# esw0116/DynaVSR

Measured on AMD Instinct MI355X. Metric: inner-loop frames/sec/GPU (EDVR-M x4, 5x3x180x320): forward leg = BASELINE.json configs[1]; the inner MAML step and the per-frame pipeline are `inner_step` / `per_frame_pipeline`, higher is better.
Workload: dtype f32; 1 GPU; EDVR-M x4 forward (PCD deformable alignment + TSA fusion + reconstruction), clips of 1x5x3x180x320 -> 3x720x1280 (BASELINE.json configs[1]); one step = 2 clip(s) per GPU, one per HIP stream (adapt.super_resolve_video); clips_in_flight_per_gpu=2

## Files before the change

### dynavsr_amd/csrc/conv2d_v2.hip

```cpp
#include <algorithm>
#include <cmath>
#include <cstdlib>
#include <type_traits>

#include "common.h"
#include "kernels.h"
#include "small_grid.h"

namespace dvsr {

#ifdef DVSR_CONV_TRACE
#define DVSR_ABLATE(a) ((a).ablate)
#define DVSR_STAMP(i)                                                                              \
  do {                                                                                             \
    if (a.trace && threadIdx.x == 0) a.trace[(size_t)blockIdx.x * 64 + (i)] = __builtin_readcyclecounter(); \
  } while (0)
#else
#define DVSR_ABLATE(a) 0
#define DVSR_STAMP(i) \
  do {                \
  } while (0)
#endif

template <int KS, int S, int CC, int TH, int MT, int BF = 0>
// ... 750 lines not shown
  using Sh = KsShape<MT, NT>;
  auto kern = conv2d_ksplit_kernel<MT, NT>;
  static PerDeviceOnce attr_once;
  set_dyn_lds_once(attr_once, (const void*)kern, Sh::LDS_BYTES);
  hipLaunchKernelGGL(kern, dim3(k.nitems), dim3(256), Sh::LDS_BYTES, st, k);
  return check_launch("conv2d_ksplit_kernel");
}

namespace {
struct ConvShape { int ks, stride, N, Ho, Wo, Cout, Ctot; };
int int_or(const char* v, int dflt) { return v ? atoi(v) : dflt; }

double conv2_pipe_cost(int TH, int MT, int CC, const ConvShape& s) {
  const double wgs = (double)ceil_div(s.Wo, 32) * ceil_div(s.Ho, TH) * s.N * ceil_div(s.Cout, 32 * MT);
  return ceil(wgs / 256.0) * 64.0 * (s.ks * s.ks) * (CC / 2) * (TH / 4) * MT;
}
bool mt1_wins(int cc, const ConvShape& s) { return conv2_pipe_cost(4, 1, cc, s) < 0.97 * conv2_pipe_cost(4, 2, cc, s); }

ConvGeo choose_row_split(const ConvShape& s, ConvAllow allow) {
  ConvGeo g{8, 4, mt1_wins(8, s) ? 1 : 2};
  if ((allow & ALLOW_DMA_HALO) && s.stride == 1 && s.Wo % 4 == 0) g.kernel = ConvKernel::ROW_SPLIT;
  return g;
}

constexpr long long KSPLIT_BELOW_WGS = 700;
bool choose_ksplit(const ConvShape& s, ConvAllow allow, ConvGeo* g) {
  if (!(s.ks == 3 && s.stride == 1 && (allow & ALLOW_KSPLIT) && s.Ctot >= 32 && s.Cout >= 32)) return false;
  const long long wg41 = (long long)ceil_div(s.Wo, 32) * ceil_div(s.Ho, 4) * s.N * ceil_div(s.Cout, 32);
  if (wg41 >= KSPLIT_BELOW_WGS) return false;
  *g = (s.Cout % 64 != 0 && s.Ho % 2 == 0) ? ConvGeo{32, 2, 1} : ConvGeo{32, 1, 2};
  return true;
}

int chunk_channels(int ks) { return ks == 1 ? 32 : (ks == 2 ? 16 : 8); }
ConvGeo choose_direct_tile(const ConvShape& s) {
  const int cc = chunk_channels(s.ks);
  if (s.ks == 3 && s.stride == 2) {
    const double c82 = conv2_pipe_cost(8, 2, cc, s);
    if (c82 <= conv2_pipe_cost(4, 2, cc, s) && c82 <= conv2_pipe_cost(4, 1, cc, s)) return ConvGeo{cc, 8, 2};
  }
  return ConvGeo{cc, 4, mt1_wins(cc, s) ? 1 : 2};
}

struct WinoPick { int th; double cost; };
double wino_workgroups(const ConvShape& s, int oh, int ow) { return (double)ceil_div(s.Wo, ow) * ceil_div(s.Ho, oh) * s.N * ceil_div(s.Cout, 64); }
double wino_rounds_cost(const ConvShape& s, double cus, int oh, int ow, double chunk_cyc, double fixed_cyc) {
  return ceil(wino_workgroups(s, oh, ow) / cus) * ((s.Ctot / 8) * chunk_cyc + fixed_cyc) / 2.07;
}
double direct_cost(const ConvShape& s) {
  const double dcyc = std::min(conv2_pipe_cost(4, 2, 8, s), conv2_pipe_cost(4, 1, 8, s));
  const double drounds = dcyc / (64.0 * 9 * 4 * (mt1_wins(8, s) ? 1 : 2));
  return dcyc * (s.Ctot / 8) / (drounds <= 6.0 ? 0.60 : 0.78) / 2.4;
}
WinoPick wino_f2_cost(const ConvShape& s, double cus, bool tile16) {
  const double w4 = wino_rounds_cost(s, cus, 4, 64, 5100.0, 12500.0), w8 = wino_rounds_cost(s, cus, 8, 32, 5100.0, 12500.0);
  const double w16 = tile16 ? wino_rounds_cost(s, cus, 16, 16, 5100.0, 12500.0) : 1e300;
  return {(w16 < w4 && w16 < w8) ? 16 : (w8 < w4 ? 8 : 4), std::min(std::min(w4, w8), w16)};
}
constexpr double W5_CHUNK_CYC = 4300.0, W5_FIXED_CYC = 17500.0;
WinoPick wino_f4_cost(const ConvShape& s, double cus) {
  const double f8 = wino_rounds_cost(s, cus, 8, 64, W5_CHUNK_CYC, W5_FIXED_CYC), f16 = wino_rounds_cost(s, cus, 16, 32, W5_CHUNK_CYC, W5_FIXED_CYC);
  return {f16 < f8 ? 16 : 8, std::min(f8, f16)};
}
constexpr double SHARED_LATENCY_BOUND = 1.05;
bool f4_occupies_less(const ConvShape& s, double cus, const WinoPick& f2, const WinoPick& f4) {
  const int ow2 = f2.th == 16 ? 16 : (f2.th == 8 ? 32 : 64), ow4 = f4.th == 16 ? 32 : 64;
  const double g2 = wino_workgroups(s, f2.th, ow2), g4 = wino_workgroups(s, f4.th, ow4);
  if (g2 > cus || g4 > cus) return false;
  ConvShape one = s;
  one.N = 1;
  if (2.0 * wino_workgroups(one, f2.th, ow2) <= cus || 2.0 * wino_workgroups(one, f4.th, ow4) > cus) return false;
  return g4 * f4.cost < g2 * f2.cost && f4.cost <= SHARED_LATENCY_BOUND * f2.cost;
}
}

double conv2_f4_occupied_cycles(int N, int Ho, int Wo, int Cout, int Ctot, int th) {
  const ConvShape s{3, 1, N, Ho, Wo, Cout, Ctot};
  return wino_workgroups(s, th, th == 16 ? 32 : 64) * ((Ctot / 8) * W5_CHUNK_CYC + W5_FIXED_CYC);
}

ConvGeo conv2_choose(int ks, int stride, int N, int Ho, int Wo, int Cout, int Ctot, ConvAllow allow) {
  const ConvShape s{ks, stride, N, Ho, Wo, Cout, Ctot};
  if (ks == 7 || ks == 9) return choose_row_split(s, allow);
  ConvGeo g;
  if (choose_ksplit(s, allow, &g)) return g;
  g = choose_direct_tile(s);
  if ((allow & ALLOW_DMA_HALO) && ks == 3 && stride == 1 && Wo % 4 == 0 && Ctot % 8 == 0) g.kernel = ConvKernel::DMA_HALO;
  const int wino_on = int_or(getenv("DVSR_CONV_WINO"), 1);
  if (!(wino_on && g.kernel == ConvKernel::DMA_HALO && (allow & ALLOW_WINO) && Cout >= 32 && Ctot >= 16)) return g;
  const int wino3_on = int_or(getenv("DVSR_CONV_WINO3"), 1), wino5_on = int_or(getenv("DVSR_CONV_WINO5"), 1);
  const double direct = direct_cost(s), cus = (double)device_cus();
  const WinoPick f2 = wino_f2_cost(s, cus, wino3_on != 0);
  if (wino5_on && wino3_on && (allow & ALLOW_WINO_F4) && Wo % 4 == 0 && device_lds_optin() >= (size_t)156 * 1024) {
    const WinoPick f4 = wino_f4_cost(s, cus);
    const bool shared_pick = (allow & ALLOW_SHARED_DEVICE) && f2.cost < direct && f4_occupies_less(s, cus, f2, f4);
    if (wino5_on >= 2 || (allow & ALLOW_ONLY_F4) || ((1.15 * f4.cost < f2.cost || shared_pick) && f4.cost < direct))
      return ConvGeo{8, wino5_on == 3 ? 16 : f4.th, 2, 0, ConvKernel::WINO_F4};
  }
  if ((wino_on == 2 || f2.cost < direct) && device_lds_optin() >= (size_t)155 * 1024)
    return ConvGeo{8, f2.th, 2, 0, wino3_on ? ConvKernel::WINO_F2_BF16 : ConvKernel::WINO_F2};
  return g;
}

static int pack_chunk_floats(int ks, int cc, int bf, PackLayout layout) {
  switch (layout) {
    case PackLayout::WINO_F2: return 16 * 2 * 64 * 4;
    case PackLayout::WINO_F2_BF16: return 2 * 6144;
    case PackLayout::WINO_F4: return 18 * 2 * 3 * 256;
    case PackLayout::DCN_SPLIT: return mdcn_pack_floats();
    default: return (bf == 2 ? 3 : 1) * 2 * ks * ks * (bf ? cc / 16 : cc / 8) * 2 * 32 * 4;
  }
}
size_t conv2_pack_floats(int ks, int Cout, int Ctot, int cc, int bf, PackLayout layout) {
  return (size_t)ceil_div(Cout, 64) * ceil_div(Ctot, cc) * pack_chunk_floats(ks, cc, bf, layout);
}
PackEntry conv2_pack_entry(const float* w, float* P, int ks, int Cout, int Ctot, int cc, int bf, PackLayout layout, int wt, int w_ctot,
                           int w_coff) {
  PackEntry e{};
  e.w = w; e.P = P; e.Cout = Cout; e.Ctot = Ctot; e.KK = ks * ks; e.CC = cc; e.wt = wt; e.w_ctot = w_ctot; e.w_coff = w_coff;
  e.ncb = ceil_div(Cout, 64); e.nchunks = ceil_div(Ctot, cc); e.pch = pack_chunk_floats(ks, cc, bf, layout);
  e.bf = bf; e.layout = layout;
  return e;
}

#ifdef DVSR_CONV_TRACE
static long long* g_trace_buf = nullptr;
static int g_trace_countdown = -1;
extern "C" int dvsr_debug_conv_trace(void* buf, int launch_index) {
  g_trace_buf = (long long*)buf;
  g_trace_countdown = launch_index;
  return 0;
}
#endif

int conv2d_packed_prepare(const dvsr_conv2d_desc& d, const float* wp, const ConvExtra& ex, const ConvGeo& geo, ConvK2* out) {
  DVSR_REQUIRE(d.x0 && wp && d.y, DVSR_ERR_INVALID, "conv2d_packed: null x0/wp/y");
  DVSR_REQUIRE(((d.ks == 1 || d.ks == 2) && d.stride == 1) || (d.ks == 3 && (d.stride == 1 || d.stride == 2)) ||
                   ((d.ks == 7 || d.ks == 9) && d.stride == 1 && geo.kernel == ConvKernel::ROW_SPLIT),
               DVSR_ERR_UNSUPPORTED, "conv2d_packed: ks=%d stride=%d", d.ks, d.stride);
  DVSR_REQUIRE(d.c1 == 0 || (d.c0 % geo.cc == 0 && !ex.in_ps && !ex.in_dil), DVSR_ERR_UNSUPPORTED,
               "conv2d_packed: two inputs need c0 %% %d == 0 and a plain first input (c0=%d)", geo.cc, d.c0);
  ConvK2& k = *out;
  k.x0 = d.x0; k.x1 = d.x1; k.wp = wp; k.bias = d.bias; k.res = d.res; k.y = d.y;
  k.N = d.N; k.c0 = d.c0; k.c1 = d.c1; k.H = d.H; k.W = d.W; k.Cout = d.Cout;
  k.pad = d.pad; k.act = d.act; k.ps = d.pixel_shuffle; k.x1_bdiv = d.x1_bdiv > 0 ? d.x1_bdiv : 1;
  k.x0_bs = d.x0_bstride > 0 ? d.x0_bstride : (long long)d.c0 * d.H * d.W;
  k.x1_bs = d.x1_bstride > 0 ? d.x1_bstride : (long long)d.c1 * d.H * d.W;
  k.Ho = (d.H + 2 * d.pad - d.ks) / d.stride + 1;
  k.Wo = (d.W + 2 * d.pad - d.ks) / d.stride + 1;
  k.nchunks = ceil_div(d.c0 + d.c1, geo.cc);
  k.in_ps = ex.in_ps; k.in_dil = ex.in_dil; k.Hs = ex.Hs; k.Ws = ex.Ws; k.accum = ex.accum;
  k.gmask = ex.gmask; k.gmask_act = ex.gmask_act;
  k.wdiv = ex.wdiv > 0 ? ex.wdiv : 1; k.w_gs = ex.w_gs; k.b_gs = ex.b_gs;
  DVSR_REQUIRE(!d.pre || (geo.kernel == ConvKernel::WINO_F4 && !d.res && d.pixel_shuffle == 0 && ((uintptr_t)d.pre & 15) == 0),
               DVSR_ERR_UNSUPPORTED, "conv2d_packed: a pre-activation addend needs the F(4x4, 3x3) kernel, a 16-byte aligned tensor, "
               "no residual and no PixelShuffle");
  k.pre = d.pre; k.pre_bdiv = d.pre_bdiv > 0 ? d.pre_bdiv : 1; k.pre_bs = (long long)d.Cout * k.Ho * k.Wo;
#ifdef DVSR_CONV_TRACE
  {
    static int ablate = -1;
    if (ablate < 0) {
      const char* v = getenv("DVSR_CONV_ABLATE");
      ablate = v ? atoi(v) : 0;
    }
    k.ablate = ablate;
  }
#endif
  if (k.in_ps) k.x0_bs = (long long)d.c0 * d.H * d.W;
  if (k.in_dil) k.x0_bs = (long long)d.c0 * ex.Hs * ex.Ws;
#ifdef DVSR_CONV_TRACE
  k.trace = (g_trace_countdown == 0) ? g_trace_buf : nullptr;
  if (g_trace_countdown >= 0) --g_trace_countdown;
#endif
  if (geo.kernel == ConvKernel::ROW_SPLIT) {
    DVSR_REQUIRE((d.ks == 7 || d.ks == 9) && d.stride == 1 && d.pad == d.ks / 2 && !ex.in_ps && !ex.in_dil && geo.cc == 8 &&
                     geo.th == 4 && d.W % 4 == 0 && (d.c1 == 0 || d.c0 % 8 == 0) && k.x0_bs % 4 == 0 && k.x1_bs % 4 == 0 &&
                     ((uintptr_t)d.x0 & 15) == 0 && ((uintptr_t)d.x1 & 15) == 0,
                 DVSR_ERR_UNSUPPORTED, "conv2d_packed: the row-split DMA kernel needs 7x7 / 9x9, stride 1, pad ks/2, plain "
                 "16-byte aligned inputs and W %% 4 == 0 (W=%d c0=%d c1=%d)", d.W, d.c0, d.c1);
  } else if (needs_dma_halo_inputs(geo.kernel)) {
    DVSR_REQUIRE(!is_winograd(geo.kernel) || d.c0 + d.c1 >= 16, DVSR_ERR_UNSUPPORTED, "conv2d_packed: the Winograd kernel needs two 8-channel chunks");
    DVSR_REQUIRE(geo.kernel != ConvKernel::WINO_F4 || (!ex.accum && !ex.gmask && d.W % 4 == 0 && (geo.th == 8 || geo.th == 16)), DVSR_ERR_UNSUPPORTED,
                 "conv2d_packed: the F(4x4, 3x3) kernel stores whole tile columns of forward launches (W=%d th=%d)", d.W, geo.th);
    DVSR_REQUIRE(!is_winograd(geo.kernel) || d.pixel_shuffle == 0 || (d.pixel_shuffle == 2 && d.Cout % 4 == 0 && !d.res && !ex.accum && !ex.gmask),
                 DVSR_ERR_UNSUPPORTED, "conv2d_packed: the Winograd kernel stores plain or PixelShuffle(2) tiles (ps=%d)", d.pixel_shuffle);
    DVSR_REQUIRE(d.ks == 3 && d.stride == 1 && d.pad == 1 && !ex.in_ps && !ex.in_dil && geo.cc == 8 && (geo.th == 4 || geo.th == 8 || (geo.th == 16 && on_bf16_split(geo.kernel))) &&
                     d.W % 4 == 0 && d.c0 % 8 == 0 && d.c1 % 8 == 0 && k.x0_bs % 4 == 0 && k.x1_bs % 4 == 0 &&
                     ((uintptr_t)d.x0 & 15) == 0 && ((uintptr_t)d.x1 & 15) == 0,
                 DVSR_ERR_UNSUPPORTED, "conv2d_packed: the DMA-halo kernel needs 3x3/s1/pad 1, plain 16-byte aligned inputs, "
                 "W %% 4 == 0 and channel counts %% 8 == 0 (W=%d c0=%d c1=%d)", d.W, d.c0, d.c1);
  }
  if (d.ks == 3 && geo.cc == 32) {
    DVSR_REQUIRE(d.stride == 1 && (d.c1 == 0 || d.c0 % 32 == 0) && !ex.in_ps && !ex.in_dil && d.pad == 1 &&
                     ((geo.th == 1 && geo.mt == 2) || (geo.th == 2 && geo.mt == 1)),
                 DVSR_ERR_UNSUPPORTED, "conv2d_packed: the K-split kernel needs 3x3/s1/pad 1, plain inputs, c0 %% 32 == 0 "
                 "with two inputs (th=%d mt=%d)", geo.th, geo.mt);
    k.tiles_x = ceil_div(k.Wo, 32); k.tiles_y = ceil_div(k.Ho, geo.th); k.ntiles = k.tiles_x * k.tiles_y * k.N;
    k.ncb = ceil_div(k.Cout, 32 * geo.mt);
    k.tiles_per_xcd = ceil_div(k.ntiles, 8);
    k.nitems = k.tiles_per_xcd * 8 * k.ncb;
  }
  return DVSR_OK;
}

template <int KS, int S, int CC, int TH, int BF>
static int launch_conv2_mt(int mt, const ConvK2& k, hipStream_t st) {
  return mt == 2 ? launch_conv2<KS, S, CC, TH, 2, BF>(k, st) : launch_conv2<KS, S, CC, TH, 1, BF>(k, st);
}

int conv2d_packed_run(const dvsr_conv2d_desc& d, const float* wp, const ConvExtra& ex, const ConvGeo& geo,
                      hipStream_t st) {
  ConvK2 k;
  int rc = conv2d_packed_prepare(d, wp, ex, geo, &k);
  if (rc) return rc;
  if (geo.bf) {
    DVSR_REQUIRE((d.ks == 3 || (d.ks == 2 && geo.bf == 2)) && d.stride == 1 && geo.cc == 16 && (geo.th == 4 || (geo.bf == 2 && geo.th == 8)),
                 DVSR_ERR_UNSUPPORTED,
                 "conv2d_packed: the bf16 kernel exists for 3x3 (split: also 2x2) stride-1 convs with 16-channel chunks");
    const bool th8 = geo.th == 8;
    if (geo.bf == 2 && d.ks == 2)
      return th8 ? launch_conv2_mt<2, 1, 16, 8, 2>(geo.mt, k, st) : launch_conv2_mt<2, 1, 16, 4, 2>(geo.mt, k, st);
    if (geo.bf == 2) return th8 ? launch_conv2_mt<3, 1, 16, 8, 2>(geo.mt, k, st) : launch_conv2_mt<3, 1, 16, 4, 2>(geo.mt, k, st);
    return launch_conv2_mt<3, 1, 16, 4, 1>(geo.mt, k, st);
  }
  switch (geo.kernel) {
    case ConvKernel::WINO_F2: return conv2d_wino_launch(k, geo.th, st);
    case ConvKernel::WINO_F2_BF16: return conv2d_wino3_launch(k, geo.th, st);
    case ConvKernel::WINO_F4: return conv2d_wino5_launch(k, geo.th, st);
    case ConvKernel::ROW_SPLIT:
      if (d.ks == 7) return geo.mt == 2 ? launch_dmarow<7, 4, 2>(k, st) : launch_dmarow<7, 4, 1>(k, st);
      return geo.mt == 2 ? launch_dmarow<9, 4, 2>(k, st) : launch_dmarow<9, 4, 1>(k, st);
    case ConvKernel::DMA_HALO:
      if (geo.th != 4) break;
      return geo.mt == 2 ? launch_dma<4, 2>(k, st) : launch_dma<4, 1>(k, st);
    case ConvKernel::REG:
      if (d.ks == 3 && geo.cc == 32) return geo.mt == 2 ? launch_ksplit<2, 1>(k, st) : launch_ksplit<1, 2>(k, st);
      switch (((d.ks * 10 + d.stride) * 100 + geo.cc) * 100 + geo.th * 10 + geo.mt) {
        case 320882: return launch_conv2<3, 2, 8, 8, 2>(k, st);
        case 320842: return launch_conv2<3, 2, 8, 4, 2>(k, st);
        case 320841: return launch_conv2<3, 2, 8, 4, 1>(k, st);
        case 310842: return launch_conv2<3, 1, 8, 4, 2>(k, st);
        case 310841: return launch_conv2<3, 1, 8, 4, 1>(k, st);
        case 211642: return launch_conv2<2, 1, 16, 4, 2>(k, st);
        case 211641: return launch_conv2<2, 1, 16, 4, 1>(k, st);
        case 113242: return launch_conv2<1, 1, 32, 4, 2>(k, st);
        case 113241: return launch_conv2<1, 1, 32, 4, 1>(k, st);
      }
      break;
  }
  DVSR_REQUIRE(false, DVSR_ERR_INVALID, "conv2d_packed: no kernel for ks=%d cc=%d th=%d mt=%d", d.ks, geo.cc, geo.th,
               geo.mt);
}

}

namespace {
struct OpPack {
  dvsr::ConvGeo geo;
  size_t floats;
};
OpPack op_pack(int ks, int stride, int pad, int N, int Ho, int Wo, int Cout, int Ctot, bool plain, bool aligned = false,
               bool only_f4 = false) {
  using namespace dvsr;
  OpPack o;
  const bool k3 = ks == 3 && stride == 1 && pad == 1, kbig = (ks == 7 || ks == 9) && stride == 1 && pad == ks / 2;
  o.geo = conv2_choose(ks, stride, N, Ho, Wo, Cout, Ctot, (k3 && plain && !only_f4 ? ALLOW_KSPLIT : ALLOW_NONE) | ((k3 || kbig) && aligned ? ALLOW_DMA_HALO : ALLOW_NONE) |
                                                              (k3 && aligned ? ALLOW_WINO | ALLOW_WINO_F4 : ALLOW_NONE) | (only_f4 ? ALLOW_ONLY_F4 : ALLOW_NONE));
  o.floats = conv2_pack_floats(ks, Cout, Ctot, o.geo);
  return o;
}
OpPack op_pack_for(const dvsr_conv2d_desc& d, int Cout, int Ctot) {
  const bool big = d.ks == 7 || d.ks == 9;
  const bool aligned = (((uintptr_t)d.x0 | (uintptr_t)d.x1) & 15) == 0 && (big ? (d.c1 == 0 || d.c0 % 8 == 0) : (d.c0 % 8 == 0 && d.c1 % 8 == 0)) &&
                       d.x0_bstride % 4 == 0 && d.x1_bstride % 4 == 0 && (d.H * d.W) % 4 == 0;
  return op_pack(d.ks, 1, d.pad, d.N, d.H, d.W, Cout, Ctot, d.c1 == 0 || d.c0 % 32 == 0, aligned, d.pre != nullptr);
}
int op_run(const dvsr_conv2d_desc& d, const dvsr::ConvExtra& ex, int Cout, int Ctot, void* ws, size_t bytes, hipStream_t st) {
  using namespace dvsr;
  DVSR_REQUIRE((d.ks == 1 || d.ks == 3 || d.ks == 7 || d.ks == 9) && d.stride == 1 && d.pad == d.ks / 2, DVSR_ERR_UNSUPPORTED,
               "conv2d (packed): ks=%d stride=%d pad=%d (1x1 / 3x3 / 7x7 / 9x9, stride 1, pad ks/2)", d.ks, d.stride, d.pad);
  const OpPack o = op_pack_for(d, Cout, Ctot);
  DVSR_REQUIRE(d.ks <= 3 || o.geo.kernel == ConvKernel::ROW_SPLIT, DVSR_ERR_UNSUPPORTED, "conv2d (packed): this %dx%d convolution is not eligible for the "
               "row-split kernel (dvsr_conv2d_packed_geometry): use dvsr_conv2d_forward / _backward", d.ks, d.ks);
  DVSR_REQUIRE(!d.pre || (o.geo.kernel == ConvKernel::WINO_F4 && !d.res && !d.pixel_shuffle), DVSR_ERR_UNSUPPORTED,
               "conv2d (packed): a pre-activation addend (pre) needs a launch the F(4x4, 3x3) kernel takes -- an aligned 3x3 / "
               "stride 1 / pad 1 convolution, W %% 4 == 0, whole 8-channel chunks, at least 32 outputs and 16 inputs -- without a "
               "residual or a PixelShuffle");
  DVSR_REQUIRE(ws && bytes >= o.floats * sizeof(float), DVSR_ERR_WORKSPACE, "conv2d (packed): workspace %zu < %zu bytes", bytes,
               o.floats * sizeof(float));
  PackTable t;
  t.n = 1;
  t.e[0] = conv2_pack_entry(d.w, (float*)ws, d.ks, Cout, Ctot, o.geo, ex.wt, ex.w_ctot, ex.w_coff);
  int rc = pack_weights_run(t, st);
  if (rc) return rc;
  return conv2d_packed_run(d, (const float*)ws, ex, o.geo, st);
}
}

extern "C" size_t dvsr_conv2d_packed_workspace_bytes(const dvsr_conv2d_desc* d) {
  if (!d || (d->ks != 1 && d->ks != 3 && d->ks != 7 && d->ks != 9)) return 0;
  const int ctot = d->c0 + d->c1;
  const size_t a = op_pack(d->ks, 1, d->ks / 2, d->N, d->H, d->W, d->Cout, ctot, true).floats;
  const size_t b = op_pack(d->ks, 1, d->ks / 2, d->N, d->H, d->W, ctot, d->Cout, true).floats;
  const size_t c = op_pack(d->ks, 1, d->ks / 2, d->N, d->H, d->W, d->Cout, ctot, false).floats;
  size_t w = 0;
  if (d->ks == 3)
    for (const dvsr::PackLayout l : {dvsr::PackLayout::WINO_F2_BF16, dvsr::PackLayout::WINO_F4})
      w = std::max(w, std::max(dvsr::conv2_pack_floats(3, d->Cout, ctot, 8, 0, l), dvsr::conv2_pack_floats(3, ctot, d->Cout, 8, 0, l)));
  return std::max(std::max(a, b), std::max(c, w)) * sizeof(float);
}

extern "C" int dvsr_conv2d_packed_geometry(const dvsr_conv2d_desc* d, int geo[4]) {
  DVSR_REQUIRE(d && geo && (d->ks == 1 || d->ks == 3 || d->ks == 7 || d->ks == 9) && d->stride == 1 && d->pad == d->ks / 2,
               DVSR_ERR_INVALID, "conv2d_packed_geometry: 1x1 / 3x3 / 7x7 / 9x9 stride-1 descriptors only");
  const OpPack o = op_pack_for(*d, d->Cout, d->c0 + d->c1);
  geo[0] = o.geo.cc; geo[1] = o.geo.th; geo[2] = o.geo.mt; geo[3] = static_cast<int>(o.geo.kernel);
  return DVSR_OK;
}

extern "C" int dvsr_conv2d_forward_packed(const dvsr_conv2d_desc* d, void* workspace, size_t workspace_bytes,
                                          dvsr_stream_t stream) {
  DVSR_REQUIRE(d && d->x0 && d->w && d->y, DVSR_ERR_INVALID, "conv2d_forward_packed: null argument");
  DVSR_REQUIRE(d->pixel_shuffle == 0 || (d->pixel_shuffle == 2 && d->Cout % 4 == 0 && !d->res), DVSR_ERR_INVALID,
               "conv2d_forward_packed: pixel_shuffle needs Cout %% 4 == 0 and no residual");
  return op_run(*d, dvsr::ConvExtra(), d->Cout, d->c0 + d->c1, workspace, workspace_bytes, (hipStream_t)stream);
}

extern "C" int dvsr_conv2d_dgrad_packed(const dvsr_conv2d_desc* d, const float* gy, float* gx0, void* workspace,
                                        size_t workspace_bytes, dvsr_stream_t stream) {
  using namespace dvsr;
  DVSR_REQUIRE(d && gy && gx0 && d->w, DVSR_ERR_INVALID, "conv2d_dgrad_packed: null argument");
  DVSR_REQUIRE(d->c1 == 0 && d->pixel_shuffle == 0, DVSR_ERR_UNSUPPORTED, "conv2d_dgrad_packed: single plain input only");
  dvsr_conv2d_desc g = {};
  g.x0 = gy; g.w = d->w; g.y = gx0; g.N = d->N; g.c0 = d->Cout; g.Cout = d->c0; g.H = d->H; g.W = d->W; g.ks = d->ks;
  g.stride = 1; g.pad = d->ks / 2; g.act = ACT_NONE; g.x1_bdiv = 1;
  ConvExtra ex;
  ex.wt = 1; ex.w_ctot = d->c0; ex.w_coff = 0;
  return op_run(g, ex, d->c0, d->Cout, workspace, workspace_bytes, (hipStream_t)stream);
}
```

### dynavsr_amd/csrc/conv2d_wino5.hip

```cpp
#include <type_traits>

#include "common.h"
#include "kernels.h"
#include "small_grid.h"

namespace dvsr {

#ifdef DVSR_CONV_TRACE
#define W5_STAMP(i)                                                                                       \
  do {                                                                                                    \
    if (a.trace && threadIdx.x == 0) a.trace[(size_t)blockIdx.x * 64 + (i)] = __builtin_readcyclecounter(); \
  } while (0)
#else
#define W5_STAMP(i) \
  do {              \
  } while (0)
#endif

typedef float w5f2 __attribute__((ext_vector_type(2)));
typedef __bf16 w5bf8 __attribute__((ext_vector_type(8)));
typedef __bf16 w5bf2 __attribute__((ext_vector_type(2)));
typedef unsigned w5u4 __attribute__((ext_vector_type(4)));

constexpr int W5_PCH = 18 * 2 * 3 * 256;

template <int TC>
struct Wino5Shape {
  static constexpr int CC = 8, NTILE = 32, TRW = NTILE / TC, NT = 768;
  static constexpr int OH = 4 * TRW, OW = 4 * TC;
  static constexpr int IH = OH + 2, RP = OW + 8, GR = RP / 4;
  static constexpr int NG = CC * IH * GR;
  static constexpr int NI = (NG + NT - 1) / NT;
  static constexpr int RAWPAD = NI * NT * 4;
  static constexpr int VIMG = 36 * 3 * 32 * 4;
  static constexpr int XCH = 6 * 16 * 64 * 4;
  static constexpr int LOOP = 2 * RAWPAD + 2 * VIMG;
  static constexpr size_t LDS_BYTES = (size_t)(LOOP > XCH ? LOOP : XCH) * sizeof(float);
};

constexpr int w5_waitcnt(int vm, int lgkm) { return (vm & 15) | (7 << 4) | ((lgkm & 15) << 8) | ((vm >> 4) << 14); }

__device__ __forceinline__ unsigned w5_cvt_pk(float a, float b) {
  return __builtin_bit_cast(unsigned, __builtin_convertvector(w5f2{a, b}, w5bf2));
}
__device__ __forceinline__ void w5_dma16(__amdgpu_buffer_rsrc_t rs, float* lds, unsigned voff, unsigned soff) {
  __builtin_amdgcn_raw_ptr_buffer_load_lds(rs, (__attribute__((address_space(3))) void*)lds, 16, voff, soff, 0, 0);
}
__device__ __forceinline__ __amdgpu_buffer_rsrc_t w5_rsrc(const float* base, int num_records) {
  return __builtin_amdgcn_make_buffer_rsrc(const_cast<float*>(base), 0, num_records, 0x00020000);
}

__global__ void pack_weights_wino5_kernel(PackTable t) {
  const PackEntry& e = t.e[blockIdx.y];
  if (e.layout != PackLayout::WINO_F4) return;
  __bf16* const P16 = reinterpret_cast<__bf16*>(e.P);
  const size_t total = (size_t)e.ncb * e.nchunks * 512;
  constexpr double G[6][3] = {{1.0 / 4, 0, 0},          {-1.0 / 6, -1.0 / 6, -1.0 / 6}, {-1.0 / 6, 1.0 / 6, -1.0 / 6},
                              {1.0 / 24, 1.0 / 12, 1.0 / 6}, {1.0 / 24, -1.0 / 12, 1.0 / 6}, {0, 0, 1}};
  for (size_t i = blockIdx.x * (size_t)blockDim.x + threadIdx.x; i < total; i += (size_t)gridDim.x * blockDim.x) {
    const int c8 = (int)(i & 7), col = (int)((i >> 3) & 63);
    const size_t ck = i >> 9;
    const int k = (int)(ck % e.nchunks), cb = (int)(ck / e.nchunks);
    const int co = cb * 64 + col, ci = k * 8 + c8;
    double g[3][3];
    const bool ok = co < e.Cout && ci < e.Ctot;
    const float* src = !e.wt ? e.w + ((size_t)co * (e.w_ctot ? e.w_ctot : e.Ctot) + (e.w_ctot ? e.w_coff : 0) + ci) * 9
                             : e.w + ((size_t)ci * e.w_ctot + e.w_coff + co) * 9;
#pragma unroll
    for (int tap = 0; tap < 9; ++tap) g[tap / 3][tap % 3] = ok ? (double)src[e.wt ? 8 - tap : tap] : 0.0;
    double c[6][3];
#pragma unroll
    for (int xi = 0; xi < 6; ++xi)
#pragma unroll
      for (int b = 0; b < 3; ++b) c[xi][b] = G[xi][0] * g[0][b] + G[xi][1] * g[1][b] + G[xi][2] * g[2][b];
    const int mh = col >> 5, c32 = col & 31;
    __bf16* dst = P16 + ck * (size_t)(2 * W5_PCH) + (size_t)mh * 1536 + (size_t)c32 * 8 + c8;
#pragma unroll
    for (int xi = 0; xi < 6; ++xi)
#pragma unroll
      for (int nu = 0; nu < 6; ++nu) {
        const float u = (float)(c[xi][0] * G[nu][0] + c[xi][1] * G[nu][1] + c[xi][2] * G[nu][2]);
        const __bf16 h = (__bf16)u;
        const float r1 = u - (float)h;
        const __bf16 m = (__bf16)r1;
        const __bf16 l = (__bf16)(r1 - (float)m);
        __bf16* d = dst + (size_t)(xi * 3 + (nu >> 1)) * 3072;
        if (nu & 1) { d[512] = m; d[768] = h; d[1024] = l; }
        else { d[0] = h; d[256] = m; d[1280] = l; }
      }
  }
}

int pack_weights_wino5_run(const PackTable& t, hipStream_t st) {
  hipLaunchKernelGGL(pack_weights_wino5_kernel, dim3(64, t.n), dim3(256), 0, st, t);
  return check_launch("pack_weights_wino5_kernel");
}

template <int TC, bool RES, bool R16, bool PRE>
__global__ __launch_bounds__(1024) void conv2d_wino5_kernel(ConvK2 a) {
  static_assert(!PRE || (R16 && !RES), "the addend is read by the sixteen-reader epilogue, never beside a residual");
  using Sh = Wino5Shape<TC>;
  constexpr int IH = Sh::IH, RP = Sh::RP, GR = Sh::GR;
  constexpr int CHF = IH * RP;
  constexpr int QF = 768 * 4;
  extern __shared__ __attribute__((aligned(16))) float smem[];
  float* const raw0 = smem;
  unsigned* const vimg0 = reinterpret_cast<unsigned*>(smem + 2 * Sh::RAWPAD);

  const int id = blockIdx.x;
  const int q_ = id >> 3;
  const int cbi = q_ % a.ncb;
  const int j_ = q_ / a.ncb;
  const int tile = (id & 7) * a.tiles_per_xcd + j_;
  if (j_ >= a.tiles_per_xcd || tile >= a.ntiles) return;
  const int tx_ = tile % a.tiles_x;
  const int t2 = tile / a.tiles_x;
  const int ty_ = t2 % a.tiles_y;
  const int n = t2 / a.tiles_y;
  const int oy0 = ty_ * Sh::OH, ox0 = tx_ * Sh::OW;

  const int tid = threadIdx.x, lane = tid & 63;
  const int wave = __builtin_amdgcn_readfirstlane(tid >> 6);
  const int lo = lane & 31, hi = lane >> 5;
  const size_t HW = (size_t)a.H * a.W;
  auto fence = [&]() __attribute__((always_inline)) { __builtin_amdgcn_sched_barrier(0); };
  auto lds_barrier = [&]() __attribute__((always_inline)) {
    asm volatile("s_waitcnt lgkmcnt(0)" ::: "memory");
    __builtin_amdgcn_s_barrier();
    asm volatile("" ::: "memory");
  };
  W5_STAMP(0);
#ifdef DVSR_CONV_TRACE
  if (a.trace && threadIdx.x == 0) a.trace[(size_t)blockIdx.x * 64 + 60] = __builtin_amdgcn_s_memrealtime();
#endif

  auto read16 = [&](int m) __attribute__((always_inline)) {
    int le = lane;
    asm volatile("" : "+v"(le));
    const int rq_r = wave & 3, cp_r = wave >> 2;
    const float* const xr = smem + (rq_r * 64 + le) * 4 + cp_r;
    const int lo_e = le & 31, hi_e = le >> 5;
    const int trow_e = lo_e / TC, tcol_e = lo_e - trow_e * TC;
    const int oy = oy0 + 4 * trow_e, ox = ox0 + 4 * tcol_e;
    const size_t HWo = (size_t)a.Ho * a.Wo;
    const float slope = a.act == ACT_LRELU ? 0.1f : (a.act == ACT_RELU ? 0.f : 1.f);
    const float* bias = wset_ptr(a.bias, a.b_gs, n, a.wdiv);
    const int co0 = cbi * 64 + m * 32 + 8 * rq_r + 4 * hi_e + cp_r;
    f32x4 pr[4];
    if constexpr (PRE) {
      const bool live = oy < a.Ho && ox < a.Wo && co0 < a.Cout;
      const float* pre = a.pre + (size_t)(n / a.pre_bdiv) * a.pre_bs + (size_t)co0 * HWo + (size_t)oy * a.Wo + ox;
#pragma unroll
      for (int i = 0; i < 4; ++i)
        pr[i] = (live && oy + i < a.Ho) ? *reinterpret_cast<const f32x4*>(pre + (size_t)i * a.Wo) : f32x4{0.f, 0.f, 0.f, 0.f};
    }
    float y[4][4];
#pragma unroll
    for (int j = 0; j < 4; ++j) {
      float z[6];
#pragma unroll
      for (int x = 0; x < 6; ++x) z[x] = xr[(x * 16 + j * 4) * 256];
      const float sa = z[1] + z[2], da = z[1] - z[2];
      const float sb = z[3] + z[4], db = z[3] - z[4];
      y[0][j] = z[0] + sa + sb;
      y[1][j] = __builtin_fmaf(2.f, db, da);
      y[2][j] = __builtin_fmaf(4.f, sb, sa);
      y[3][j] = __builtin_fmaf(8.f, db, da) + z[5];
    }
    const bool px_ok = oy < a.Ho && ox < a.Wo;
    const int nrow = a.Ho - oy < 4 ? a.Ho - oy : 4;
    if (px_ok && co0 < a.Cout) {
      const float b0 = bias ? bias[co0] : 0.f;
      const size_t base = ((size_t)n * a.Cout + co0) * HWo + (size_t)oy * a.Wo + ox;
      f32x4 rr[4];
      if constexpr (RES) {
#pragma unroll
        for (int i = 0; i < 4; ++i)
          rr[i] = i < nrow ? *reinterpret_cast<const f32x4*>(a.res + base + (size_t)i * a.Wo) : f32x4{0.f, 0.f, 0.f, 0.f};
      }
#pragma unroll
      for (int i = 0; i < 4; ++i) {
        if (i >= nrow) break;
        f32x4 v;
#pragma unroll
        for (int j = 0; j < 4; ++j) {
          float v0 = y[i][j] + b0;
          if constexpr (PRE) v0 += pr[i][j];
          v[j] = fmaxf(v0, v0 * slope);
        }
        if constexpr (RES) v += rr[i];
        *reinterpret_cast<f32x4*>(a.y + base + (size_t)i * a.Wo) = v;
      }
    }
  };

  if (wave >= 12) {
    const int pw = wave - 12, ptid = tid - 768;
    const float* x0n = a.x0 + (size_t)n * a.x0_bs;
    const float* x1n = a.c1 ? a.x1 + (size_t)(n / a.x1_bdiv) * a.x1_bs : x0n;
    static_assert(IH * GR * 4 == 720, "a channel quad is 720 groups");
    unsigned hoff[3];
#pragma unroll
    for (int jj = 0; jj < 3; ++jj) {
      const int L = jj * 256 + ptid;
      const int cq = L / (IH * GR), rr = L - cq * (IH * GR);
      const int iy = rr / GR, g = rr - iy * GR;
      const int gy = oy0 - 1 + iy, gx = ox0 - 4 + 4 * g;
      const bool live = L < 4 * IH * GR;
      const bool ok = live && (unsigned)gy < (unsigned)a.H && (unsigned)gx < (unsigned)a.W;
      hoff[jj] = ok ? (unsigned)(((size_t)cq * HW + (size_t)gy * a.W + gx) * 4) : 0x80000000u;
      if (live && !ok) {
#pragma unroll
        for (int bb = 0; bb < 4; ++bb) *reinterpret_cast<f32x4*>(raw0 + (bb >> 1) * Sh::RAWPAD + (bb & 1) * QF + L * 4) = f32x4{0.f, 0.f, 0.f, 0.f};
      }
    }
    const unsigned chunk_bytes = (unsigned)(Sh::CC * HW * 4), quad_bytes = (unsigned)(4 * HW * 4);
    auto issue_raw = [&](int k) __attribute__((always_inline)) {
      const bool live = k < a.nchunks;
      const bool second = k * Sh::CC >= a.c0;
      const unsigned soff = live ? (unsigned)(second ? k - a.c0 / Sh::CC : k) * chunk_bytes : 0u;
      const __amdgpu_buffer_rsrc_t rs = w5_rsrc(second ? x1n : x0n, live ? 0x7fffffff : 0);
      float* dst = raw0 + (k & 1) * Sh::RAWPAD + 256 * pw;
#pragma unroll
      for (int jj = 0; jj < 3; ++jj) {
        w5_dma16(rs, dst + jj * 1024, hoff[jj], soff);
        w5_dma16(rs, dst + QF + jj * 1024, hoff[jj], soff + quad_bytes);
      }
    };
    const int ptile = 8 * pw + (lane & 7), ppair = (lane >> 3) & 3;
    const int trow_t = ptile / TC, tcol_t = ptile - trow_t * TC;
    const int pch = 2 * ppair + hi;
    const float* prd = raw0 + (pch >> 2) * QF + (pch & 3) * CHF + 4 * trow_t * RP + 4 * tcol_t;
    unsigned* vw12 = vimg0 + (hi ? 2 : 1) * 6 * 384 + ptile * 4 + ppair;
    unsigned* vw34 = vimg0 + (hi ? 4 : 3) * 6 * 384 + ptile * 4 + ppair;
    unsigned* vw05 = vimg0 + (hi ? 5 : 0) * 6 * 384 + ptile * 4 + ppair;
    auto ld_row = [&](float (&d)[6], int row) __attribute__((always_inline)) {
      const float* p = prd + row * RP;
      const w5f2 l2 = *reinterpret_cast<const w5f2*>(p + 2);
      const f32x4 m4 = *reinterpret_cast<const f32x4*>(p + 4);
      const w5f2 h2 = *reinterpret_cast<const w5f2*>(p + 8);
      d[0] = l2[1]; d[1] = m4[0]; d[2] = m4[1]; d[3] = m4[2]; d[4] = m4[3]; d[5] = h2[0];
    };
    auto colpass = [&](const float (&r)[6], float (&v)[6]) __attribute__((always_inline)) {
      v[0] = __builtin_fmaf(4.f, r[0], __builtin_fmaf(-5.f, r[2], r[4]));
      v[5] = __builtin_fmaf(4.f, r[1], __builtin_fmaf(-5.f, r[3], r[5]));
      const float e1 = __builtin_fmaf(-4.f, r[2], r[4]), o1 = __builtin_fmaf(-4.f, r[1], r[3]);
      v[1] = e1 + o1; v[2] = e1 - o1;
      const float e2 = r[4] - r[2], o2 = r[3] - r[1];
      v[3] = __builtin_fmaf(2.f, o2, e2); v[4] = __builtin_fmaf(-2.f, o2, e2);
    };
    auto finish_pair = [&](const float (&ra)[6], const float (&rb)[6], unsigned* vw) __attribute__((always_inline)) {
      float va[6], vb[6];
      colpass(ra, va);
      colpass(rb, vb);
#pragma unroll
      for (int v = 0; v < 6; ++v) {
        const auto s0 = __builtin_amdgcn_permlane32_swap(__builtin_bit_cast(unsigned, va[v]), __builtin_bit_cast(unsigned, vb[v]), false, false);
        const unsigned u0 = s0[0], u1 = s0[1];
        const float v0 = __builtin_bit_cast(float, u0), v1 = __builtin_bit_cast(float, u1);
        const unsigned h = w5_cvt_pk(v0, v1);
        const float r0 = v0 - __builtin_bit_cast(float, h << 16), r1 = v1 - __builtin_bit_cast(float, h & 0xffff0000u);
        const unsigned m = w5_cvt_pk(r0, r1);
        const float q0 = r0 - __builtin_bit_cast(float, m << 16), q1 = r1 - __builtin_bit_cast(float, m & 0xffff0000u);
        unsigned* d = vw + v * 384;
#ifdef W5_NOVW
        d[0] = h ^ m ^ w5_cvt_pk(q0, q1);
#else
        d[0] = h; d[128] = m; d[256] = w5_cvt_pk(q0, q1);
#endif
      }
    };
    auto produce = [&]() __attribute__((always_inline)) {
      float d0[6], d1[6], d2[6], d3[6], d4[6], d5[6];
      ld_row(d1, 1); ld_row(d2, 2); ld_row(d3, 3); ld_row(d4, 4);
      ld_row(d0, 0); ld_row(d5, 5);
      float ra[6], rb[6];
#pragma unroll
      for (int j = 0; j < 6; ++j) {
        const float e = __builtin_fmaf(-4.f, d2[j], d4[j]), o = __builtin_fmaf(-4.f, d1[j], d3[j]);
        ra[j] = e + o; rb[j] = e - o;
      }
      finish_pair(ra, rb, vw12);
      fence();
#pragma unroll
      for (int j = 0; j < 6; ++j) {
        const float e = d4[j] - d2[j], o = d3[j] - d1[j];
        ra[j] = __builtin_fmaf(2.f, o, e); rb[j] = __builtin_fmaf(-2.f, o, e);
      }
      finish_pair(ra, rb, vw34);
      fence();
#pragma unroll
      for (int j = 0; j < 6; ++j) {
        ra[j] = __builtin_fmaf(4.f, d0[j], __builtin_fmaf(-5.f, d2[j], d4[j]));
        rb[j] = __builtin_fmaf(4.f, d1[j], __builtin_fmaf(-5.f, d3[j], d5[j]));
      }
      finish_pair(ra, rb, vw05);
    };
    issue_raw(0);
    issue_raw(1);
    __builtin_amdgcn_s_waitcnt(w5_waitcnt(6, 0));
    __builtin_amdgcn_s_barrier();
    asm volatile("" ::: "memory");
    produce();
    __builtin_amdgcn_s_waitcnt(w5_waitcnt(0, 0));
    __builtin_amdgcn_s_barrier();
    asm volatile("" ::: "memory");
    int vstep = Sh::VIMG, rstep = Sh::RAWPAD;
    vw12 += vstep; vw34 += vstep; vw05 += vstep; prd += rstep;
    __builtin_amdgcn_s_setprio(3);
    for (int k = 0; k < a.nchunks; ++k) {

#ifndef W5_NODMA
      issue_raw(k + 2);
#endif
#ifndef W5_NOPROD
      if (k + 1 < a.nchunks) produce();
#endif
      __builtin_amdgcn_s_waitcnt(w5_waitcnt(0, 0));
      __builtin_amdgcn_s_barrier();
      asm volatile("" ::: "memory");
      vw12 -= vstep; vw34 -= vstep; vw05 -= vstep; prd -= rstep;
      vstep = -vstep; rstep = -rstep;
    }
    if constexpr (R16) {
      __builtin_amdgcn_s_setprio(0);
      lds_barrier();
      lds_barrier(); read16(0);
      lds_barrier();
      lds_barrier(); read16(1);
    } else {
      lds_barrier(); lds_barrier(); lds_barrier(); lds_barrier();
    }
    return;
  }
  {
    const int cxi = wave % 6, cmh = wave / 6;
    f32x16 acc[6];
#pragma unroll
    for (int v = 0; v < 6; ++v)
#pragma unroll
      for (int r = 0; r < 16; ++r) acc[v][r] = 0.f;
    const float* wp_cb = wset_ptr(a.wp, a.w_gs, n, a.wdiv) + (size_t)cbi * a.nchunks * W5_PCH;
    const __amdgpu_buffer_rsrc_t wrsrc = w5_rsrc(wp_cb, -1);
    const unsigned avoff = (unsigned)(lane * 16);
    const int asb = (cxi * 3 * 2 + cmh) * 3072;
    f32x4 AF[3];
    auto gldA = [&](auto g_, int k) __attribute__((always_inline)) {
      constexpr int G = decltype(g_)::value;
#ifdef W5_NOA
      if (k > 0 || G > 2) return;
#endif
      const int soff = k * (W5_PCH * 4) + asb + (G / 3) * 6144 + (G % 3) * 1024;
      AF[G % 3] = __builtin_bit_cast(f32x4, __builtin_amdgcn_raw_buffer_load_b128(wrsrc, (int)avoff, soff, 0));
    };
    auto blend = [&](f32x4& x, const f32x4& l, bool keep) __attribute__((always_inline)) {
#pragma unroll
      for (int r = 0; r < 4; ++r) x[r] = keep ? x[r] : l[r];
    };
    const unsigned* vrd = vimg0 + cxi * 6 * 384 + lo * 4;
    const unsigned* vrd_lh = vrd + (hi ? 0 : 256);
    const unsigned* vrd_hl = vrd + (hi ? 256 : 0);
    w5u4 BF[2];
    auto ldB = [&](auto f_) __attribute__((always_inline)) {
      constexpr int F = decltype(f_)::value, NU = F / 3, W = F % 3;
      if constexpr (W == 0) BF[F & 1] = *reinterpret_cast<const w5u4*>(vrd + NU * 384);
      else if constexpr (W == 1) BF[F & 1] = *reinterpret_cast<const w5u4*>(vrd + NU * 384 + 128);
      else if constexpr (NU & 1) BF[F & 1] = *reinterpret_cast<const w5u4*>(vrd_hl + NU * 384);
      else BF[F & 1] = *reinterpret_cast<const w5u4*>(vrd_lh + NU * 384);
    };
    auto mma = [&](f32x16& c, const f32x4& av, const w5u4& bv) __attribute__((always_inline)) {
#ifdef W5_NOMMA
      c[0] += av[0] * __builtin_bit_cast(float, bv[0]);
      return;
#endif
      c = __builtin_amdgcn_mfma_f32_32x32x16_bf16(__builtin_bit_cast(w5bf8, av), __builtin_bit_cast(w5bf8, bv), c, 0, 0, 0);
    };
    static_for<0, 3>([&](auto g_) __attribute__((always_inline)) { gldA(g_, 0); });
    __builtin_amdgcn_s_barrier();
    asm volatile("" ::: "memory");
    __builtin_amdgcn_s_barrier();
    asm volatile("" ::: "memory");
    int vstep = Sh::VIMG;
    for (int k = 0; k < a.nchunks; ++k) {
      ldB(std::integral_constant<int, 0>{}); ldB(std::integral_constant<int, 1>{});
      const int knext = k + 1 < a.nchunks ? k + 1 : k;
      static_for<0, 18>([&](auto f_) __attribute__((always_inline)) {
        constexpr int F = decltype(f_)::value, NU = F / 3, I = F % 3;
        constexpr int XS = NU & 1;
        mma(acc[NU], AF[XS], BF[F & 1]);
#ifdef W5_NOBR
        if constexpr (false)
#else
        if constexpr (F + 2 < 18)
#endif
          ldB(std::integral_constant<int, (F + 2 < 18 ? F + 2 : 0)>{});
        if constexpr (I == 1) {
          blend(AF[XS], AF[2], (NU & 1) ? hi != 0 : hi == 0);
          if constexpr ((NU & 1) && NU < 5) gldA(std::integral_constant<int, 3 * ((NU < 5 ? NU : 1) / 2) + 5>{}, k);
          if constexpr (NU == 5) gldA(std::integral_constant<int, 2>{}, knext);
        }
        if constexpr (I == 2) {
          if constexpr (NU < 4) gldA(std::integral_constant<int, 3 * ((NU < 4 ? NU : 0) / 2) + 3 + (NU & 1)>{}, k);
          else gldA(std::integral_constant<int, (NU & 1)>{}, knext);
        }
        fence();
      });
      lds_barrier();
      if (k < 16) W5_STAMP(3 + k);
      vrd += vstep; vrd_lh += vstep; vrd_hl += vstep;
      vstep = -vstep;
    }
  W5_STAMP(40);

  int lane_e = lane;
  asm volatile("" : "+v"(lane_e));
  f32x16 Z[4];
#pragma unroll
  for (int r = 0; r < 16; ++r) {
    const float sa = acc[1][r] + acc[2][r], da = acc[1][r] - acc[2][r];
    const float sb = acc[3][r] + acc[4][r], db = acc[3][r] - acc[4][r];
    Z[0][r] = acc[0][r] + sa + sb;
    Z[1][r] = __builtin_fmaf(2.f, db, da);
    Z[2][r] = __builtin_fmaf(4.f, sb, sa);
    Z[3][r] = __builtin_fmaf(8.f, db, da) + acc[5][r];
  }
  float* const xw = smem + (cxi * 16 * 64 + lane_e) * 4;
  const int rq_r = wave & 3, cp_r = wave >> 2;
  const float* const xr = smem + (rq_r * 64 + lane_e) * 4 + cp_r * 2;
  const int lo_e = lane_e & 31, hi_e = lane_e >> 5;
  const int trow_e = lo_e / TC, tcol_e = lo_e - trow_e * TC;
  const int oy = oy0 + 4 * trow_e, ox = ox0 + 4 * tcol_e;
  const size_t HWo = (size_t)a.Ho * a.Wo;
  const float slope = a.act == ACT_LRELU ? 0.1f : (a.act == ACT_RELU ? 0.f : 1.f);
  const float* bias = wset_ptr(a.bias, a.b_gs, n, a.wdiv);
  W5_STAMP(50);
  lds_barrier();
  W5_STAMP(51);
#pragma unroll 1
  for (int m = 0; m < 2; ++m) {
    if (cmh == m) {
#pragma unroll
      for (int j = 0; j < 4; ++j)
#pragma unroll
        for (int rq = 0; rq < 4; ++rq)
          *reinterpret_cast<f32x4*>(xw + (j * 4 + rq) * 256) = f32x4{Z[j][4 * rq], Z[j][4 * rq + 1], Z[j][4 * rq + 2], Z[j][4 * rq + 3]};
    }
    W5_STAMP(52 + 4 * m);
    lds_barrier();
    W5_STAMP(53 + 4 * m);
    if constexpr (R16) read16(m);
    else if (wave < 8) {
      const int co0 = cbi * 64 + m * 32 + 8 * rq_r + 4 * hi_e + 2 * cp_r;
      float y[2][4][4];
#pragma unroll
      for (int j = 0; j < 4; ++j) {
        w5f2 z[6];
#pragma unroll
        for (int x = 0; x < 6; ++x) z[x] = *reinterpret_cast<const w5f2*>(xr + (x * 16 + j * 4) * 256);
#pragma unroll
        for (int c = 0; c < 2; ++c) {
          const float sa = z[1][c] + z[2][c], da = z[1][c] - z[2][c];
          const float sb = z[3][c] + z[4][c], db = z[3][c] - z[4][c];
          y[c][0][j] = z[0][c] + sa + sb;
          y[c][1][j] = __builtin_fmaf(2.f, db, da);
          y[c][2][j] = __builtin_fmaf(4.f, sb, sa);
          y[c][3][j] = __builtin_fmaf(8.f, db, da) + z[5][c];
        }
      }
      const bool px_ok = oy < a.Ho && ox < a.Wo;
      const int nrow = a.Ho - oy < 4 ? a.Ho - oy : 4;
      if (px_ok && co0 < a.Cout) {
        const bool two = co0 + 1 < a.Cout;
        const float b0 = bias ? bias[co0] : 0.f, b1 = (bias && two) ? bias[co0 + 1] : 0.f;
#pragma unroll
        for (int i = 0; i < 4; ++i)
#pragma unroll
          for (int j = 0; j < 4; ++j) {
            const float v0 = y[0][i][j] + b0, v1 = y[1][i][j] + b1;
            y[0][i][j] = fmaxf(v0, v0 * slope);
            y[1][i][j] = fmaxf(v1, v1 * slope);
          }
        if (a.ps == 0) {
#pragma unroll
          for (int c = 0; c < 2; ++c) {
            if (c == 1 && !two) break;
            const size_t base = ((size_t)n * a.Cout + co0 + c) * HWo + (size_t)oy * a.Wo + ox;
            if constexpr (RES) {
              f32x4 rr[4];
#pragma unroll
              for (int i = 0; i < 4; ++i)
                rr[i] = i < nrow ? *reinterpret_cast<const f32x4*>(a.res + base + (size_t)i * a.Wo) : f32x4{0.f, 0.f, 0.f, 0.f};
#pragma unroll
              for (int i = 0; i < 4; ++i) {
                if (i >= nrow) break;
                const f32x4 v = f32x4{y[c][i][0], y[c][i][1], y[c][i][2], y[c][i][3]} + rr[i];
                *reinterpret_cast<f32x4*>(a.y + base + (size_t)i * a.Wo) = v;
              }
            } else {
#pragma unroll
              for (int i = 0; i < 4; ++i) {
                if (i >= nrow) break;
                *reinterpret_cast<f32x4*>(a.y + base + (size_t)i * a.Wo) = f32x4{y[c][i][0], y[c][i][1], y[c][i][2], y[c][i][3]};
              }
            }
          }
        } else {
          const int cq = co0 >> 2, dy = (co0 >> 1) & 1;
          float* dst = a.y + (((size_t)n * (a.Cout >> 2) + cq) * (2 * a.Ho) + (2 * oy + dy)) * (size_t)(2 * a.Wo) + 2 * ox;
#pragma unroll
          for (int i = 0; i < 4; ++i) {
            if (i >= nrow) break;
            float* d = dst + (size_t)(2 * i) * (2 * a.Wo);
            *reinterpret_cast<f32x4*>(d) = f32x4{y[0][i][0], y[1][i][0], y[0][i][1], y[1][i][1]};
            *reinterpret_cast<f32x4*>(d + 4) = f32x4{y[0][i][2], y[1][i][2], y[0][i][3], y[1][i][3]};
          }
        }
      }
    }
    W5_STAMP(54 + 4 * m);
    if (m == 0) lds_barrier();
    W5_STAMP(55 + 4 * m);
  }
#ifdef DVSR_CONV_TRACE
  W5_STAMP(41);
  __builtin_amdgcn_s_waitcnt(0);
  W5_STAMP(42);
  if (a.trace && threadIdx.x == 0) {
    a.trace[(size_t)blockIdx.x * 64 + 61] = __builtin_amdgcn_s_memrealtime();
    a.trace[(size_t)blockIdx.x * 64 + 63] = __builtin_amdgcn_s_getreg((4) | (0 << 6) | (31 << 11));
    a.trace[(size_t)blockIdx.x * 64 + 62] = __builtin_amdgcn_s_getreg((20) | (0 << 6) | (31 << 11));
  }
#endif
  }
}

template <int TC>
static int launch_wino5(ConvK2 k, hipStream_t st) {
  using Sh = Wino5Shape<TC>;
  auto kern = k.pre ? conv2d_wino5_kernel<TC, false, true, true>
                    : (k.res ? conv2d_wino5_kernel<TC, true, true, false> : conv2d_wino5_kernel<TC, false, false, false>);
  static PerDeviceOnce attr_once, attr_once_r, attr_once_p;
  set_dyn_lds_once(attr_once, (const void*)conv2d_wino5_kernel<TC, false, false, false>, Sh::LDS_BYTES);
  set_dyn_lds_once(attr_once_r, (const void*)conv2d_wino5_kernel<TC, true, true, false>, Sh::LDS_BYTES);
  set_dyn_lds_once(attr_once_p, (const void*)conv2d_wino5_kernel<TC, false, true, true>, Sh::LDS_BYTES);
  k.tiles_x = ceil_div(k.Wo, Sh::OW); k.tiles_y = ceil_div(k.Ho, Sh::OH); k.ntiles = k.tiles_x * k.tiles_y * k.N;
  k.ncb = ceil_div(k.Cout, 64);
  k.tiles_per_xcd = ceil_div(k.ntiles, 8);
  k.nitems = k.tiles_per_xcd * 8 * k.ncb;
  hipLaunchKernelGGL(kern, dim3(k.nitems), dim3(1024), Sh::LDS_BYTES, st, k);
  return check_launch("conv2d_wino5_kernel");
}

int conv2d_wino5_launch(const ConvK2& k, int th, hipStream_t st) {
  return th == 16 ? launch_wino5<8>(k, st) : launch_wino5<16>(k, st);
}

}
```

### dynavsr_amd/csrc/engine.hip

```cpp
#include <algorithm>
#include <cstdlib>
#include <string>
#include <vector>

#include "common.h"
#include "kernels.h"
#include "small_grid.h"

namespace dvsr {

enum { SP_ARENA = 0, SP_INPUT = 1, SP_OUTPUT = 2, SP_NONE = 3 };
struct T {
  int space = SP_NONE;
  size_t off = 0, numel = 0;
  bool valid() const { return space != SP_NONE; }
};

enum OpType { OP_CONV, OP_DCN, OP_UP, OP_POOL, OP_GATE, OP_BLEND, OP_ADD, OP_PAD, OP_MEANSUB, OP_ADDMEAN };

struct Op {
  OpType type;
  const char* name = "";
  T x0, x1, res, y, y2;
  int pw = -1, pb = -1;
  int N = 0, c0 = 0, c1 = 0, H = 0, W = 0, Cout = 0, ks = 3, stride = 1, act = 0, ps = 0;
  int x1_bdiv = 1, dg = 8;
  int pad = -1;
  int pmode = 0, T = 1;
  int wmap = 0;
  size_t w2_off = 0;
  int no_dgrad = 0;
  int pad_out = 0;
  struct T ypad;
  int fused_into = -1;
  int dual = -1;
  long long x0_bs = 0, x1_bs = 0;
  int S = 1;
  float mul = 1.f;
  size_t planes = 0;
  int gB = 0, gN = 0, gC = 0;
  size_t gHW = 0;
  struct PackSlot { ConvGeo geo = {8, 8, 2}; size_t off = 0, floats = 0; };
  PackSlot dgrad[2], dcn_pack;
  enum LaunchRole { WHOLE, MAIN_PART, REF_PART };
  struct Launch { PackSlot pack; int c_off = 0, c = 0; LaunchRole role = WHOLE; };
  struct LaunchList {
    int n = 0; Launch l[2];
    const Launch* begin() const { return l; }
    const Launch* end() const { return l + n; }
    const Launch& primary() const { return l[n - 1]; }
  } launches[2];
  struct T pre;
};
enum FwdMode { FWD_GRAD = 0, FWD_NOGRAD = 1 };

enum { R_ACT = 0, R_GRAD = 1, R_X = 2, R_GX = 3, R_GOUT = 4, R_TMP = 5, R_NONE = 6 };
struct Ref {
  int space = R_NONE;
  size_t off = 0;
};
enum BType { B_MEMSET, B_COPYADD, B_ACT, B_WGRAD, B_DGRAD, B_REDUCE, B_DCN, B_UP, B_POOL, B_GATE, B_BLEND,
             B_PADFOLD, B_ADDMEAN, B_WUNMAP };
struct BOp {
  BType type;
  int fwd = -1;
  Ref a, b, c, d, e, f;
  size_t n = 0;
  int accum = 0, which = 0, cnt = 1, B = 0;
  int mask_op = -1;
  size_t ws_off = 0, ws_bytes = 0;
  long long bs = 0;
  size_t per = 0;
};

static inline int conv_pad(const Op& o) { return o.pad < 0 ? o.ks / 2 : o.pad; }
static inline int conv_out(const Op& o, int in) { return (in + 2 * conv_pad(o) - o.ks) / o.stride + 1; }

}

struct dvsr_edvr_plan {
  dvsr_edvr_config cfg;
  int B, H, W;
  int n_params = 0;
  size_t arena_floats = 0;
  std::vector<dvsr::Op> ops;
  std::vector<std::pair<std::string, dvsr::T>> named;
  std::vector<std::pair<size_t, size_t>> allocs;
  std::vector<dvsr::BOp> bops;
  size_t dpack_floats = 0;
  bool use_v1 = false;
  size_t tmp_floats = 0;
  size_t scratch_bytes = 0;
  size_t wscratch_bytes = 0;
  mutable hipStream_t side = nullptr;
  mutable hipEvent_t ev_fork = nullptr, ev_join = nullptr;
  int side_streams = 1;
  int fork_every = 3;
  const char* bwd_unsupported = nullptr;
  int wgroups = 1;
  int wsets = 1;
  bool split_any_pad = false;
};

namespace dvsr {

static T arena_alloc(dvsr_edvr_plan& p, const char* name, size_t numel) {
  T t;
  t.space = SP_ARENA;
  t.off = p.arena_floats;
  t.numel = numel;
  p.allocs.emplace_back(t.off, numel);
  p.arena_floats += (numel + 63) & ~(size_t)63;
  if (name && *name) p.named.emplace_back(name, t);
  return t;
}

static WgradDesc wgrad_shape(const dvsr_edvr_plan& p, const Op& o, int which) {
  WgradDesc d;
  d.x_bs = which ? o.x1_bs : o.x0_bs; d.x_bdiv = which ? o.x1_bdiv : 1; d.gy_ps = o.ps;
  d.N = o.N; d.Cin = which ? o.c1 : o.c0; d.H = o.H; d.W = o.W; d.Cout = o.Cout;
  d.Ctot = o.c0 + o.c1; d.c_off = which ? o.c0 : 0;
  d.ks = o.ks; d.stride = o.stride; d.pad = conv_pad(o);
  d.groups = p.wgroups; d.dW_gs = (long long)o.Cout * (o.c0 + o.c1) * o.ks * o.ks; d.db_gs = o.Cout;
  d.mode = (p.cfg.bf16_mfma == 1 && !o.wmap) ? 1 : (wgrad_split3_default() ? 2 : 0);
  return d;
}

static Op::LaunchList plan_hoist(const Op& o, const dvsr_edvr_plan& p, ConvAllow fwd_ok, const Op::Launch& whole) {
  Op::LaunchList pair;
  const char* hv = getenv("DVSR_PCD_HOIST");
  if ((hv && hv[0] == '0') || p.use_v1 || p.wsets != 1 || whole.pack.geo.kernel != ConvKernel::WINO_F4 || o.x1_bdiv <= 1 || o.c1 <= 0 ||
      o.N % o.x1_bdiv != 0 || o.res.valid() || o.ps)
    return pair;
  const int Ho = conv_out(o, o.H), Wo = conv_out(o, o.W), bd = o.x1_bdiv;
  const ConvAllow shared = fwd_ok | ALLOW_WINO_F4 | ALLOW_SHARED_DEVICE;
  const ConvAllow only_f4 = without(fwd_ok, ALLOW_KSPLIT) | ALLOW_WINO_F4 | ALLOW_ONLY_F4;
  auto choose = [&](int n, int c, ConvAllow allow) { return conv2_choose(o.ks, o.stride, n, Ho, Wo, o.Cout, c, allow); };
  auto f4 = [](const ConvGeo& g) { return g.kernel == ConvKernel::WINO_F4; };
  const ConvGeo gm = choose(o.N, o.c0, shared), gr = choose(o.N / bd, o.c1, only_f4);
  const ConvGeo u1 = choose(bd, o.c0 + o.c1, shared), m1 = choose(bd, o.c0, shared), r1 = choose(1, o.c1, only_f4);
  if (f4(gm) && f4(gr) && f4(u1) && f4(m1) && f4(r1) &&
      conv2_f4_occupied_cycles(bd, Ho, Wo, o.Cout, o.c0, m1.th) + conv2_f4_occupied_cycles(1, Ho, Wo, o.Cout, o.c1, r1.th) <
          conv2_f4_occupied_cycles(bd, Ho, Wo, o.Cout, o.c0 + o.c1, u1.th)) {
    const size_t mf = conv2_pack_floats(o.ks, o.Cout, o.c0, gm), rf = conv2_pack_floats(o.ks, o.Cout, o.c1, gr);
    if (mf + rf <= whole.pack.floats)
      pair = {2, {{{gr, whole.pack.off + mf, rf}, o.c0, o.c1, Op::REF_PART}, {{gm, whole.pack.off, mf}, 0, o.c0, Op::MAIN_PART}}};
  }
  return pair;
}

static void plan_conv_launches(Op& o, dvsr_edvr_plan& p) {
  const int ks = o.ks, N = o.N, c0 = o.c0, c1 = o.c1, Cout = o.Cout, Ho = conv_out(o, o.H), Wo = conv_out(o, o.W);
  const char* s2 = getenv("DVSR_EST_SPLIT2");
  const int split2 = s2 ? atoi(s2) : 1;
  const bool bf = p.cfg.bf16_mfma && (ks == 3 || (ks == 2 && p.split_any_pad && p.cfg.bf16_mfma == 2 && split2 && c0 % 16 == 0)) &&
                  o.stride == 1 && (o.pad < 0 || p.split_any_pad) && (c1 == 0 || c0 % 16 == 0);
  static const int split_th8_from = getenv("DVSR_SPLIT_TH8_FROM") ? atoi(getenv("DVSR_SPLIT_TH8_FROM")) : 200;
  auto as_bf = [&](ConvGeo g, int ho, int wo, int cout, bool dgrad = false) {
    if (!bf || (ks == 2 && split2 == 2 && dgrad)) return g;
    if (ks == 2 && (long long)ceil_div(wo, 32) * ceil_div(ho, 4) * N * ceil_div(cout, 64) < 256) return g;
    g.cc = 16; g.th = 4; g.bf = p.cfg.bf16_mfma == 2 ? 2 : 1;
    if (g.bf == 2 && (long long)ceil_div(wo, 32) * ceil_div(ho, 8) * N * ceil_div(cout, 32 * g.mt) >= split_th8_from)
      g.th = 8;
    return g;
  };
  const bool plain = o.pad < 0 && !o.wmap && !p.cfg.bf16_mfma;
  const ConvAllow ks_ok = (plain && (c1 == 0 || c0 % 32 == 0) ? ALLOW_KSPLIT : ALLOW_NONE) |
                          (plain && c0 % 8 == 0 && c1 % 8 == 0 ? ALLOW_DMA_HALO | ALLOW_WINO : ALLOW_NONE);
  const ConvAllow fwd_ok = (o.ps == 0 || (o.ps == 2 && !o.res.valid())) ? ks_ok : without(ks_ok, ALLOW_WINO);
  auto whole = [&](const ConvGeo& g) {
    const size_t floats = conv2_pack_floats(ks, Cout, c0 + c1, g);
    return Op::Launch{{g, arena_alloc(p, "", floats * p.wsets).off, floats}, 0, c0 + c1, Op::WHOLE};
  };
  o.launches[FWD_GRAD] = {1, {whole(as_bf(conv2_choose(ks, o.stride, N, Ho, Wo, Cout, c0 + c1, fwd_ok), Ho, Wo, Cout))}};
  Op::LaunchList& nograd = o.launches[FWD_NOGRAD] = o.launches[FWD_GRAD];
  if ((fwd_ok & ALLOW_WINO) && !nograd.l[0].pack.geo.bf) {
    const ConvGeo g5 = conv2_choose(ks, o.stride, N, Ho, Wo, Cout, c0 + c1, fwd_ok | ALLOW_WINO_F4 | ALLOW_SHARED_DEVICE);
    if (g5.kernel == ConvKernel::WINO_F4) nograd.l[0] = whole(g5);
  }
  const Op::LaunchList pair = plan_hoist(o, p, fwd_ok, nograd.l[0]);
  if (pair.n) {
    o.pre = arena_alloc(p, "", (size_t)(N / o.x1_bdiv) * Cout * Ho * Wo);
    nograd = pair;
  }
  for (int which = 0; which < 2; ++which) {
    const int ci = which ? c1 : c0;
    if (!ci) continue;
    Op::PackSlot& dg = o.dgrad[which];
    dg.geo = as_bf(conv2_choose(ks, 1, N, o.H, o.W, ci, Cout, (!o.ps && o.stride == 1) ? ks_ok : ALLOW_NONE), o.H, o.W, ci, true);
    dg.floats = conv2_pack_floats(ks, ci, Cout, dg.geo);
    dg.off = p.dpack_floats;
    p.dpack_floats += dg.floats * p.wsets;
  }
}

struct Builder {
  dvsr_edvr_plan& p;
  int pcur = 0;
  explicit Builder(dvsr_edvr_plan& plan) : p(plan) {}

  T alloc(const char* name, size_t numel) { return arena_alloc(p, name, numel); }
  static T view(const T& base, size_t off, size_t numel) {
    T t = base;
    t.off += off;
    t.numel = numel;
    return t;
  }
  struct CP { int w, b; };
  CP take() { CP c{pcur, pcur + 1}; pcur += 2; return c; }

  T conv(const char* name, CP cp, T x0, int c0, T x1, int c1, int N, int H, int W, int Cout, int ks,
         int stride, int act, T res = T(), int ps = 0, int x1_bdiv = 1, long long x0_bs = 0,
         long long x1_bs = 0, T y_override = T(), int pad = -1, int wmap = 0) {
    Op o;
    o.type = OP_CONV; o.name = name; o.pw = cp.w; o.pb = cp.b; o.pad = pad; o.wmap = wmap;
    o.x0 = x0; o.x1 = x1; o.res = res;
    o.N = N; o.c0 = c0; o.c1 = c1; o.H = H; o.W = W; o.Cout = Cout; o.ks = ks; o.stride = stride;
    o.act = act; o.ps = ps; o.x1_bdiv = x1_bdiv; o.x0_bs = x0_bs; o.x1_bs = x1_bs;
    o.y = y_override.valid() ? y_override : alloc(name, (size_t)N * Cout * conv_out(o, H) * conv_out(o, W));
    if (wmap) o.w2_off = alloc("", (size_t)std::max(p.wgroups, p.wsets) * Cout * (c0 + c1) * ks * ks).off;
    plan_conv_launches(o, p);
    p.ops.push_back(o);
    return o.y;
  }
  T dcn(const char* name, int pw, int pb, T x, T om, int N, int C, int H, int W, int dg, int act) {
    Op o;
    o.type = OP_DCN; o.name = name; o.pw = pw; o.pb = pb; o.x0 = x; o.x1 = om;
    o.N = N; o.c0 = C; o.H = H; o.W = W; o.Cout = C; o.dg = dg; o.act = act;
    o.y = alloc(name, (size_t)N * C * H * W);
    if (C % (dg * 8) == 0) {
      o.dcn_pack.floats = conv2_pack_floats(3, C, C, 8, 0, PackLayout::DCN_SPLIT);
      o.dcn_pack.off = alloc("", o.dcn_pack.floats * p.wsets).off;
    }
    p.ops.push_back(o);
    return o.y;
  }
  T up(const char* name, T x, size_t planes, int H, int W, int S, float mul) {
    Op o;
    o.type = OP_UP; o.name = name; o.x0 = x; o.planes = planes; o.H = H; o.W = W; o.S = S; o.mul = mul;
    o.y = alloc(name, planes * H * W * S * S);
    p.ops.push_back(o);
    return o.y;
  }
  T padop(const char* name, T x, int mode, int N, int C, int H, int W, int Tn) {
    Op o;
    o.type = OP_PAD; o.name = name; o.x0 = x; o.pmode = mode; o.N = N; o.c0 = C; o.H = H; o.W = W; o.T = Tn;
    o.y = alloc(name, pad_out_numel(mode, (size_t)N, C, H, W));
    p.ops.push_back(o);
    return o.y;
  }
  void pool(const char* name, T x, size_t planes, int H, int W, T& ymax, T& yavg) {
    Op o;
    o.type = OP_POOL; o.name = name; o.x0 = x; o.planes = planes; o.H = H; o.W = W;
    const size_t n = planes * (size_t)((H - 1) / 2 + 1) * ((W - 1) / 2 + 1);
    o.y = ymax = alloc((std::string(name) + "_max").c_str(), n);
    o.y2 = yavg = alloc((std::string(name) + "_avg").c_str(), n);
    p.ops.push_back(o);
  }
};

enum PlanPart { PART_WHOLE = 0, PART_EXTRACT = 1, PART_FUSE = 2 };

struct SlotLayout { size_t off[3], numel[3], raw, floats; };
static SlotLayout slot_layout(int C, int H, int W) {
  auto up = [](size_t n) { return (n + 63) & ~(size_t)63; };
  SlotLayout s;
  s.numel[0] = (size_t)C * H * W; s.numel[1] = (size_t)C * (H / 2) * (W / 2); s.numel[2] = (size_t)C * (H / 4) * (W / 4);
  s.off[0] = 0; s.off[1] = up(s.numel[0]); s.off[2] = s.off[1] + up(s.numel[1]);
  s.raw = s.off[2] + up(s.numel[2]);
  s.floats = s.raw + up((size_t)3 * H * W);
  return s;
}

static int build_plan(dvsr_edvr_plan& p, PlanPart part = PART_WHOLE) {
  const dvsr_edvr_config& c = p.cfg;
  const int B = p.B, Nf = c.nframes, C = c.nf, H = p.H, W = p.W, BN = B * Nf, dg = c.groups;
  const int H2 = H / 2, W2 = W / 2, H4 = H / 4, W4 = W / 4;
  const size_t HW = (size_t)H * W, HW2 = (size_t)H2 * W2, HW4 = (size_t)H4 * W4;
  Builder b(p);
  const int L = ACT_LRELU, R = ACT_RELU, NO = ACT_NONE;
  T none;
  const int EN = part == PART_EXTRACT ? 1 : BN;
  T xin; xin.space = SP_INPUT; xin.off = 0; xin.numel = (size_t)EN * 3 * HW;

  T f1, f2, f3;
  if (part == PART_FUSE) {
    f1 = b.alloc("L1_fea", (size_t)BN * C * HW);
    f2 = b.alloc("L2_fea", (size_t)BN * C * HW2);
    f3 = b.alloc("L3_fea", (size_t)BN * C * HW4);
    b.pcur += 2 * (1 + 2 * c.front_RBs + 4);
  } else {
    const SlotLayout sl = slot_layout(C, H, W);
    auto dst = [&](int l, bool final_of_level) {
      T t;
      if (part == PART_EXTRACT && final_of_level) { t.space = SP_OUTPUT; t.off = sl.off[l]; t.numel = sl.numel[l]; }
      return t;
    };
    f1 = b.conv("conv_first", b.take(), xin, 3, none, 0, EN, H, W, C, 3, 1, L, none, 0, 1, 0, 0, dst(0, c.front_RBs == 0));
    for (int i = 0; i < c.front_RBs; ++i) {
      auto p1 = b.take(); auto p2 = b.take();
      T t = b.conv("fe_rb_a", p1, f1, C, none, 0, EN, H, W, C, 3, 1, R);
      f1 = b.conv("fe_rb_b", p2, t, C, none, 0, EN, H, W, C, 3, 1, NO, f1, 0, 1, 0, 0, dst(0, i == c.front_RBs - 1));
    }
    p.named.emplace_back("L1_fea", f1);
    f2 = b.conv("fea_L2_conv1", b.take(), f1, C, none, 0, EN, H, W, C, 3, 2, L);
    f2 = b.conv("L2_fea", b.take(), f2, C, none, 0, EN, H2, W2, C, 3, 1, L, none, 0, 1, 0, 0, dst(1, true));
    f3 = b.conv("fea_L3_conv1", b.take(), f2, C, none, 0, EN, H2, W2, C, 3, 2, L);
    f3 = b.conv("L3_fea", b.take(), f3, C, none, 0, EN, H4, W4, C, 3, 1, L, none, 0, 1, 0, 0, dst(2, true));
  }
  if (part == PART_EXTRACT) {
    p.n_params = b.pcur;
    return DVSR_OK;
  }

  struct DP { int w, b; Builder::CP com; };
  auto take_dcn = [&]() { DP d; d.w = b.pcur; d.b = b.pcur + 1; b.pcur += 2; d.com = b.take(); return d; };
  auto L3o1 = b.take(); auto L3o2 = b.take(); DP L3d = take_dcn();
  auto L2o1 = b.take(); auto L2o2 = b.take(); auto L2o3 = b.take(); DP L2d = take_dcn(); auto L2f = b.take();
  auto L1o1 = b.take(); auto L1o2 = b.take(); auto L1o3 = b.take(); DP L1d = take_dcn(); auto L1f = b.take();
  auto cso1 = b.take(); auto cso2 = b.take(); DP csd = take_dcn();
  const int ctr = c.center;
  T ref1 = Builder::view(f1, (size_t)ctr * C * HW, 0), ref2 = Builder::view(f2, (size_t)ctr * C * HW2, 0),
    ref3 = Builder::view(f3, (size_t)ctr * C * HW4, 0);
  const long long rs1 = (long long)Nf * C * HW, rs2 = (long long)Nf * C * HW2, rs3 = (long long)Nf * C * HW4;
  T o3 = b.conv("L3_offset_conv1", L3o1, f3, C, ref3, C, BN, H4, W4, C, 3, 1, L, none, 0, Nf, 0, rs3);
  o3 = b.conv("L3_offset", L3o2, o3, C, none, 0, BN, H4, W4, C, 3, 1, L);
  T om3 = b.conv("L3_om", L3d.com, o3, C, none, 0, BN, H4, W4, dg * 27, 3, 1, NO);
  T fe3 = b.dcn("L3_aligned", L3d.w, L3d.b, f3, om3, BN, C, H4, W4, dg, L);
  T o2 = b.conv("L2_offset_conv1", L2o1, f2, C, ref2, C, BN, H2, W2, C, 3, 1, L, none, 0, Nf, 0, rs2);
  T u3 = b.up("L3_offset_up", o3, (size_t)BN * C, H4, W4, 2, 2.f);
  o2 = b.conv("L2_offset_conv2", L2o2, o2, C, u3, C, BN, H2, W2, C, 3, 1, L);
  o2 = b.conv("L2_offset", L2o3, o2, C, none, 0, BN, H2, W2, C, 3, 1, L);
  T om2 = b.conv("L2_om", L2d.com, o2, C, none, 0, BN, H2, W2, dg * 27, 3, 1, NO);
  T d2 = b.dcn("L2_dcn", L2d.w, L2d.b, f2, om2, BN, C, H2, W2, dg, NO);
  T uf3 = b.up("L3_aligned_up", fe3, (size_t)BN * C, H4, W4, 2, 1.f);
  T fe2 = b.conv("L2_aligned", L2f, d2, C, uf3, C, BN, H2, W2, C, 3, 1, L);
  T o1 = b.conv("L1_offset_conv1", L1o1, f1, C, ref1, C, BN, H, W, C, 3, 1, L, none, 0, Nf, 0, rs1);
  T u2 = b.up("L2_offset_up", o2, (size_t)BN * C, H2, W2, 2, 2.f);
  o1 = b.conv("L1_offset_conv2", L1o2, o1, C, u2, C, BN, H, W, C, 3, 1, L);
  o1 = b.conv("L1_offset", L1o3, o1, C, none, 0, BN, H, W, C, 3, 1, L);
  T om1 = b.conv("L1_om", L1d.com, o1, C, none, 0, BN, H, W, dg * 27, 3, 1, NO);
  T d1 = b.dcn("L1_dcn", L1d.w, L1d.b, f1, om1, BN, C, H, W, dg, NO);
  T uf2 = b.up("L2_aligned_up", fe2, (size_t)BN * C, H2, W2, 2, 1.f);
  T fe1 = b.conv("L1_aligned", L1f, d1, C, uf2, C, BN, H, W, C, 3, 1, NO);
  T oc = b.conv("cas_offset_conv1", cso1, fe1, C, ref1, C, BN, H, W, C, 3, 1, L, none, 0, Nf, 0, rs1);
  oc = b.conv("cas_offset", cso2, oc, C, none, 0, BN, H, W, C, 3, 1, L);
  T omc = b.conv("cas_om", csd.com, oc, C, none, 0, BN, H, W, dg * 27, 3, 1, NO);
  T aligned = b.dcn("aligned", csd.w, csd.b, fe1, omc, BN, C, H, W, dg, L);

  auto tA1 = b.take(); auto tA2 = b.take(); auto ffu = b.take(); auto s1 = b.take(); auto s2 = b.take();
  auto s3 = b.take(); auto s4 = b.take(); auto s5 = b.take(); auto sL1 = b.take(); auto sL2 = b.take();
  auto sL3 = b.take(); auto sa1 = b.take(); auto sa2 = b.take();
  T emb_ref = b.conv("tsa_emb_ref", tA2, Builder::view(aligned, (size_t)ctr * C * HW, 0), C, none, 0, B, H,
                     W, C, 3, 1, NO, none, 0, 1, (long long)Nf * C * HW);
  T emb = b.conv("tsa_emb", tA1, aligned, C, none, 0, BN, H, W, C, 3, 1, NO);
  T cor = b.alloc("tsa_cor", (size_t)BN * HW);
  T gated = b.alloc("tsa_gated", (size_t)BN * C * HW);
  {
    Op o; o.type = OP_GATE; o.name = "tsa_gate"; o.x0 = emb; o.x1 = emb_ref; o.res = aligned;
    o.y = cor; o.y2 = gated; o.gB = B; o.gN = Nf; o.gC = C; o.gHW = HW;
    p.ops.push_back(o);
  }
  T fea = b.conv("tsa_fea", ffu, gated, Nf * C, none, 0, B, H, W, C, 1, 1, L);
  T att = b.conv("tsa_att1", s1, gated, Nf * C, none, 0, B, H, W, C, 1, 1, L);
  {
    static const bool dual_on = [] { const char* v = getenv("DVSR_TSA_DUAL"); return !(v && v[0] == '0'); }();
    const int ia = (int)p.ops.size() - 2, ib = ia + 1;
    if (dual_on && C == 64 && !p.cfg.bf16_mfma) { p.ops[ia].dual = ib; p.ops[ib].fused_into = ia; }
  }
  T pmx, pav;
  b.pool("tsa_pool1", att, (size_t)B * C, H, W, pmx, pav);
  att = b.conv("tsa_att2", s2, pmx, C, pav, C, B, H2, W2, C, 1, 1, L);
  T attL = b.conv("tsa_attL1", sL1, att, C, none, 0, B, H2, W2, C, 1, 1, L);
  T qmx, qav;
  b.pool("tsa_pool2", attL, (size_t)B * C, H2, W2, qmx, qav);
  attL = b.conv("tsa_attL2", sL2, qmx, C, qav, C, B, H4, W4, C, 3, 1, L);
  attL = b.conv("tsa_attL3", sL3, attL, C, none, 0, B, H4, W4, C, 3, 1, L);
  T attLu = b.up("tsa_attL_up", attL, (size_t)B * C, H4, W4, 2, 1.f);
  T a3 = b.conv("tsa_att3", s3, att, C, none, 0, B, H2, W2, C, 3, 1, L);
  T att3 = b.alloc("tsa_att3_sum", (size_t)B * C * HW2);
  {
    Op o; o.type = OP_ADD; o.name = "tsa_att3_add"; o.x0 = a3; o.x1 = attLu; o.y = att3;
    p.ops.push_back(o);
  }
  T a4 = b.conv("tsa_att4", s4, att3, C, none, 0, B, H2, W2, C, 1, 1, L);
  T a4u = b.up("tsa_att4_up", a4, (size_t)B * C, H2, W2, 2, 1.f);
  T a5 = b.conv("tsa_att", s5, a4u, C, none, 0, B, H, W, C, 3, 1, NO);
  T ad = b.conv("tsa_add1", sa1, a5, C, none, 0, B, H, W, C, 1, 1, L);
  ad = b.conv("tsa_add2", sa2, ad, C, none, 0, B, H, W, C, 1, 1, NO);
  T out = b.alloc("tsa_out", (size_t)B * C * HW);
  {
    Op o; o.type = OP_BLEND; o.name = "tsa_blend"; o.x0 = fea; o.x1 = a5; o.res = ad; o.y = out;
    p.ops.push_back(o);
  }

  for (int i = 0; i < c.back_RBs; ++i) {
    auto p1 = b.take(); auto p2 = b.take();
    T t = b.conv("rc_rb_a", p1, out, C, none, 0, B, H, W, C, 3, 1, R);
    out = b.conv("rc_rb_b", p2, t, C, none, 0, B, H, W, C, 3, 1, NO, out);
  }
  p.named.emplace_back("recon", out);
  int h = H, w = W;
  if (c.scale == 4) {
    out = b.conv("upconv1", b.take(), out, C, none, 0, B, h, w, C * 4, 3, 1, L, none, 2);
    h *= 2; w *= 2;
    out = b.conv("upconv2", b.take(), out, C, none, 0, B, h, w, 256, 3, 1, L, none, 2);
  } else {
    out = b.conv("upconv2", b.take(), out, C, none, 0, B, h, w, 256, 3, 1, L, none, 2);
  }
  h *= 2; w *= 2;
  out = b.conv("HRconv", b.take(), out, 64, none, 0, B, h, w, 64, 3, 1, L);
  T base = b.alloc("base", (size_t)B * 3 * h * w);
  for (int bi = 0; bi < B; ++bi) {
    Op o; o.type = OP_UP; o.name = "base_up";
    o.x0 = Builder::view(xin, part == PART_FUSE ? 0 : ((size_t)bi * Nf + ctr) * 3 * HW, 3 * HW);
    o.planes = 3; o.H = H; o.W = W; o.S = c.scale; o.mul = 1.f;
    o.y = Builder::view(base, (size_t)bi * 3 * h * w, (size_t)3 * h * w);
    p.ops.push_back(o);
  }
  T yout; yout.space = SP_OUTPUT; yout.off = 0; yout.numel = (size_t)B * 3 * h * w;
  b.conv("conv_last", b.take(), out, 64, none, 0, B, h, w, 3, 3, 1, NO, base, 0, 1, 0, 0, yout);
  p.n_params = b.pcur;
  return DVSR_OK;
}


struct BackBuilder {
  dvsr_edvr_plan& p;
  std::vector<char> written;
  struct Pending { Ref src; size_t n; int fwd; };
  std::vector<Pending> pending;
  bool gx_zeroed = false;
  explicit BackBuilder(dvsr_edvr_plan& plan) : p(plan), written(plan.allocs.size(), 0), pending(plan.allocs.size()) {}

  int alloc_index(size_t off) const {
    int lo = 0, hi = (int)p.allocs.size() - 1, ans = -1;
    while (lo <= hi) {
      const int mid = (lo + hi) / 2;
      if (p.allocs[mid].first <= off) { ans = mid; lo = mid + 1; } else hi = mid - 1;
    }
    return ans;
  }
  static Ref act(const T& t) {
    Ref r;
    r.space = t.space == SP_ARENA ? R_ACT : (t.space == SP_INPUT ? R_X : R_NONE);
    r.off = t.off;
    return r;
  }
  static Ref grad(const T& t) {
    Ref r;
    r.space = t.space == SP_ARENA ? R_GRAD : (t.space == SP_INPUT ? R_GX : (t.space == SP_OUTPUT ? R_GOUT : R_NONE));
    r.off = t.off;
    return r;
  }
  void materialize(int ai) {
    if (ai < 0 || written[ai] != 2) return;
    BOp o;
    o.type = B_COPYADD; o.fwd = pending[ai].fwd; o.a.space = R_GRAD; o.a.off = p.allocs[ai].first; o.b = pending[ai].src;
    o.n = pending[ai].n; o.accum = 0;
    p.bops.push_back(o);
    written[ai] = 1;
  }
  void materialize(const T& t) { if (t.space == SP_ARENA) materialize(alloc_index(t.off)); }
  bool take_pending_as_residual(const T& t, Ref* src) {
    if (t.space != SP_ARENA) return false;
    const int ai = alloc_index(t.off);
    if (written[ai] != 2 || t.off != p.allocs[ai].first || t.numel != p.allocs[ai].second || pending[ai].n != t.numel)
      return false;
    *src = pending[ai].src;
    written[ai] = 1;
    return true;
  }
  int contribute(const T& t, bool full, int fwd) {
    if (t.space == SP_INPUT) return 1;
    const int ai = alloc_index(t.off);
    const bool whole = full && t.off == p.allocs[ai].first && t.numel == p.allocs[ai].second;
    materialize(ai);
    if (written[ai]) return 1;
    written[ai] = 1;
    if (whole) return 0;
    BOp m;
    m.type = B_MEMSET; m.fwd = fwd; m.a.space = R_GRAD; m.a.off = p.allocs[ai].first; m.n = p.allocs[ai].second;
    p.bops.push_back(m);
    return 1;
  }
  void copyadd(const T& dst, const Ref& src, size_t n, int fwd) {
    if (dst.space == SP_ARENA) {
      const int ai = alloc_index(dst.off);
      static const bool defer = [] { const char* v = getenv("DVSR_FUSE_RES_BWD"); return !(v && v[0] == '0'); }();
      if (defer && !written[ai] && dst.off == p.allocs[ai].first && dst.numel == p.allocs[ai].second && n == dst.numel) {
        written[ai] = 2;
        pending[ai] = Pending{src, n, fwd};
        return;
      }
    }
    BOp o;
    o.type = B_COPYADD; o.fwd = fwd; o.a = grad(dst); o.b = src; o.n = n;
    o.accum = contribute(dst, true, fwd);
    p.bops.push_back(o);
  }
};

static int sole_producer_with_act(const dvsr_edvr_plan& p, const T& t, int consumer) {
  if (t.space != SP_ARENA) return -1;
  int prod = -1;
  for (int j = 0; j < consumer; ++j) {
    const Op& q = p.ops[j];
    if (q.type == OP_CONV && q.act != ACT_NONE && q.y.space == SP_ARENA && q.y.off == t.off && q.y.numel == t.numel &&
        !q.ps)
      prod = j;
  }
  if (prod < 0) return -1;
  const Op& q = p.ops[prod];
  int readers = 0;
  for (size_t j = 0; j < p.ops.size(); ++j) {
    const Op& r = p.ops[j];
    for (const T* in : {&r.x0, &r.x1, &r.res})
      if (in->space == SP_ARENA && in->off < q.y.off + q.y.numel && in->off + in->numel > q.y.off) ++readers;
  }
  return readers == 1 ? prod : -1;
}

static void build_backward(dvsr_edvr_plan& p) {
  BackBuilder bb(p);
  size_t tmp = 0, scratch = 0, wscratch = 0;
  std::vector<char> act_fused(p.ops.size(), 0);
  const bool fuse_act = !p.use_v1 && [] { const char* v = getenv("DVSR_FUSE_ACT_BWD"); return !(v && v[0] == '0'); }();
  for (int i = (int)p.ops.size() - 1; i >= 0; --i) {
    const Op& o = p.ops[i];
    const Ref gy = BackBuilder::grad(o.y);
    bb.materialize(o.y);
    bb.materialize(o.y2);
    if (o.type == OP_GATE) bb.materialize(o.res);
    switch (o.type) {
      case OP_CONV: {
        if (o.res.valid() && o.act != ACT_NONE) p.bwd_unsupported = "a convolution with both a residual input and an activation";
        if (o.res.valid()) bb.copyadd(o.res, gy, o.y.numel, i);
        if (o.act != ACT_NONE && !act_fused[i]) {
          BOp a; a.type = B_ACT; a.fwd = i; a.a = gy; a.b = BackBuilder::act(o.y); a.n = o.y.numel;
          p.bops.push_back(a);
        }
        for (int which = 0; which < 2; ++which) {
          if (which == 1 && !o.c1) break;
          BOp w; w.type = B_WGRAD; w.fwd = i; w.which = which; w.a = BackBuilder::act(which ? o.x1 : o.x0); w.b = gy;
          p.bops.push_back(w);
          BOp& wr = p.bops.back();
          wr.ws_bytes = (conv2d_wgrad_workspace_bytes(wgrad_shape(p, o, which)) + 255) & ~(size_t)255;
          wr.ws_off = wscratch;
          wscratch += wr.ws_bytes;
          if (o.wmap) {
            BOp u; u.type = B_WUNMAP; u.fwd = i;
            p.bops.push_back(u);
          }
        }
        for (int which = 0; which < 2; ++which) {
          if ((which == 1 && !o.c1) || o.no_dgrad) break;
          const T& xin = which ? o.x1 : o.x0;
          const int ci = which ? o.c1 : o.c0;
          const bool strided = which ? (o.x1_bdiv > 1 || o.x1_bs != 0) : (o.x0_bs != 0);
          BOp d; d.type = B_DGRAD; d.fwd = i; d.which = which; d.b = gy;
          if (!strided) {
            T full = xin; full.numel = (size_t)o.N * ci * o.H * o.W;
            if (!p.use_v1 && bb.take_pending_as_residual(full, &d.e)) d.accum = 0;
            else d.accum = bb.contribute(full, true, i);
            d.a = BackBuilder::grad(xin);
            if (!d.accum && !o.c1 && fuse_act && d.e.space == R_NONE) {
              const int prod = sole_producer_with_act(p, full, i);
              if (prod >= 0) { d.mask_op = prod; act_fused[prod] = 1; }
            }
            p.bops.push_back(d);
          } else {
            d.accum = 0; d.a.space = R_TMP; d.a.off = 0;
            p.bops.push_back(d);
            const int bdiv = which ? o.x1_bdiv : 1;
            const size_t per = (size_t)ci * o.H * o.W;
// ... 162 lines not shown
      const bool mpad = b.mask_op >= 0 && p.ops[b.mask_op].pad_out;
      return pad_bwd(bs.at(b.b), gx, o->pmode, o->N, o->c0, o->H, o->W, o->T, b.accum, st,
                     b.mask_op >= 0 ? bs.arena + (mpad ? o->y.off : p.ops[b.mask_op].y.off) : nullptr,
                     b.mask_op >= 0 ? p.ops[b.mask_op].act : 0, mpad ? 1 : 0);
    }
    case B_ADDMEAN:
      return addmean_bwd(bs.at(b.b), bs.at(b.a), o->N / o->T, o->c0, o->T, (size_t)o->H * o->W, st);
    case B_DGRAD: {
      if (!bs.at(b.a)) return DVSR_OK;
      dvsr_conv2d_desc g;
      ConvExtra ex;
      dgrad_desc(p, b, P, bs, &g, &ex);
      if (p.use_v1) return conv2d_run(g, ex, st);
      return conv2d_packed_run(g, bs.dpack + o->dgrad[b.which].off, ex, o->dgrad[b.which].geo, st);
    }
    case B_REDUCE: {
      float* dst = bs.at(b.a);
      if (!dst) return DVSR_OK;
      return reduce_frames(dst, b.bs, bs.at(b.b), b.B, b.cnt, b.per, b.accum, st);
    }
    case B_DCN: {
      const size_t P_ = (size_t)o->H * o->W;
      const long long bstride = (long long)o->dg * 27 * P_;
      const float* om = bs.arena + o->x1.off;
      float* gom = bs.at(b.c);
      return mdcn_backward_run(bs.arena + o->x0.off, om, bstride, om + (size_t)o->dg * 18 * P_, bstride, 1, P[o->pw],
                               bs.at(b.b), bs.at(b.a), gom, bstride, gom + (size_t)o->dg * 18 * P_, bstride,
                               GP[o->pw], GP[o->pb], o->N, o->c0, o->H, o->W, o->Cout, 1, 1, 1, o->dg, scratch,
                               scratch_bytes, st, p.wgroups, (long long)o->Cout * o->c0 * 9, o->Cout,
                               p.wsets > 1 ? (long long)o->Cout * o->c0 * 9 : 0);
    }
    case B_UP: {
      float* gx = bs.at(b.a);
      if (!gx) return DVSR_OK;
      return upsample_bilinear_bwd(bs.at(b.b), gx, o->planes, o->H, o->W, o->S, o->mul, b.accum, st);
    }
    case B_POOL:
      return pool3s2_bwd(bs.arena + o->x0.off, bs.at(b.b), bs.at(b.c), bs.at(b.a), o->planes, o->H, o->W, b.accum, st);
    case B_GATE:
      return tsa_gate_bwd(bs.arena + o->x0.off, bs.arena + o->x1.off, bs.arena + o->res.off, bs.arena + o->y.off,
                          bs.at(b.b), bs.at(b.a), bs.at(b.c), bs.at(b.d), o->gB, o->gN, o->gC, o->gHW, st,
                          bs.garena + o->y.off);
    case B_BLEND:
      return tsa_blend_bwd(bs.arena + o->x0.off, bs.arena + o->x1.off, bs.at(b.b), bs.at(b.a), bs.at(b.c),
                           o->y.numel, b.accum, st);
    case B_WGRAD: break;
  }
  return DVSR_ERR_INVALID;
}

struct Bases {
  float* arena; const float* x; float* out;
  FwdMode mode;
  float* at(const T& t) const {
    if (t.space == SP_ARENA) return arena + t.off;
    if (t.space == SP_INPUT) return const_cast<float*>(x) + t.off;
    if (t.space == SP_OUTPUT) return out + t.off;
    return nullptr;
  }
};

static int pack_all(const dvsr_edvr_plan& p, const float* const* P, float* arena_base, float* fwd_base,
                    float* bwd_base, hipStream_t st, FwdMode mode = FWD_GRAD) {
  PackTable t;
  t.n = 0;
  auto flush = [&]() { int rc = pack_weights_run(t, st); t.n = 0; return rc; };
  const int S = p.wsets;
  for (const Op& o : p.ops) {
    if (o.type == OP_DCN && fwd_base && o.dcn_pack.floats) {
      for (int ws = 0; ws < S; ++ws) {
        t.e[t.n++] = conv2_pack_entry(P[o.pw] + (size_t)ws * o.Cout * o.c0 * 9, fwd_base + o.dcn_pack.off + (size_t)ws * o.dcn_pack.floats,
                                      3, o.Cout, o.c0, 8, 0, mdcn_pack_layout(o.W));
        if (t.n == 48) { int rc = flush(); if (rc) return rc; }
      }
    }
    if (o.type != OP_CONV) continue;
    const int ctot = o.c0 + o.c1, KK = o.ks * o.ks;
    const size_t wnum = (size_t)o.Cout * ctot * KK;
    const float* wsrc = P[o.pw];
    if (o.wmap) {
      wsrc = arena_base + o.w2_off;
      if (fwd_base) {
        int rc = w4_to_s2d(P[o.pw], arena_base + o.w2_off, S * o.Cout, ctot / 4, 0, st);
        if (rc) return rc;
      }
    }
    for (int ws = 0; ws < S; ++ws) {
      if (fwd_base) {
        for (const Op::Launch& l : o.launches[mode]) {
          const bool sliced = l.c != ctot;
          t.e[t.n++] = conv2_pack_entry(wsrc + ws * wnum, fwd_base + l.pack.off + (size_t)ws * l.pack.floats, o.ks, o.Cout, l.c, l.pack.geo,
                                        0, sliced ? ctot : 0, sliced ? l.c_off : 0);
          if (t.n == 48) { int rc = flush(); if (rc) return rc; }
        }
      }
      if (bwd_base) {
        for (int which = 0; which < 2; ++which) {
          const int ci = which ? o.c1 : o.c0;
          if (!ci) continue;
          const Op::PackSlot& dg = o.dgrad[which];
          t.e[t.n++] = conv2_pack_entry(wsrc + ws * wnum, bwd_base + dg.off + (size_t)ws * dg.floats, o.ks, ci, o.Cout, dg.geo, 1, ctot,
                                        which ? o.c0 : 0);
          if (t.n == 48) { int rc = flush(); if (rc) return rc; }
        }
      }
    }
  }
  return flush();
}

static dvsr_conv2d_desc launch_desc(dvsr_conv2d_desc d, const Op& o, Op::LaunchRole role, float* pre) {
  if (role == Op::WHOLE) return d;
  if (role == Op::REF_PART) { d.x0 = d.x1; d.c0 = o.c1; d.x0_bstride = o.x1_bs; d.N = o.N / o.x1_bdiv; d.act = ACT_NONE; d.y = pre; }
  else { d.bias = nullptr; d.pre = pre; d.pre_bdiv = o.x1_bdiv; }
  d.x1 = nullptr; d.c1 = 0; d.x1_bdiv = 1; d.x1_bstride = 0;
  return d;
}

static int run_forward_op(const dvsr_edvr_plan& p, const Op& o, const float* const* P, const Bases& bs, hipStream_t st) {
  switch (o.type) {
    case OP_CONV: {
      dvsr_conv2d_desc d = {};
      d.x0 = bs.at(o.x0); d.x1 = bs.at(o.x1); d.w = P[o.pw]; d.bias = P[o.pb]; d.res = bs.at(o.res);
      d.y = bs.at(o.y);
      d.N = o.N; d.c0 = o.c0; d.c1 = o.c1; d.H = o.H; d.W = o.W; d.Cout = o.Cout; d.ks = o.ks;
      d.stride = o.stride; d.pad = conv_pad(o); d.act = o.act; d.pixel_shuffle = o.ps;
      if (o.pad_out) { d.y = bs.at(o.ypad); d.pixel_shuffle = o.pad_out; }
      if (!p.use_v1 && (o.dual >= 0 || o.fused_into >= 0)) {
        const Op& oa = o.dual >= 0 ? o : p.ops[o.fused_into];
        const Op& ob = p.ops[oa.dual];
        const long long HW = (long long)oa.H * oa.W;
        auto plain1x1 = [](const Op& q) {
          return q.type == OP_CONV && q.ks == 1 && q.stride == 1 && q.c1 == 0 && q.Cout == 64 && !q.res.valid() && !q.ps && !q.wmap && !q.pad_out;
        };
        const bool pair_ok = plain1x1(oa) && plain1x1(ob) && oa.act == ob.act && oa.c0 == ob.c0 && oa.N == ob.N && oa.H == ob.H &&
                             oa.W == ob.W && oa.x0.space == ob.x0.space && oa.x0.off == ob.x0.off;
        if (pair_ok && conv1x1_dual_ok(bs.at(oa.x0), P[oa.pw], P[ob.pw], bs.at(oa.y), bs.at(ob.y), oa.c0, HW)) {
          if (o.fused_into >= 0) return DVSR_OK;
          return conv1x1_dual_run(bs.at(oa.x0), P[oa.pw], P[oa.pb], P[ob.pw], P[ob.pb], bs.at(oa.y), bs.at(ob.y), oa.N, oa.c0,
                                  (int)HW, oa.act, st, p.wsets > 1 ? oa.N / p.wsets : 1,
                                  p.wsets > 1 ? (long long)oa.Cout * oa.c0 : 0, p.wsets > 1 ? oa.Cout : 0);
        }
      }
      if (o.wmap) d.w = bs.arena + o.w2_off;
      d.x1_bdiv = o.x1_bdiv; d.x0_bstride = o.x0_bs; d.x1_bstride = o.x1_bs;
      if (p.use_v1) return conv2d_run(d, ConvExtra(), st);
      if (o.Cout <= 4 && o.ks == 3 && o.stride == 1 && !o.c1 && !o.ps && !o.x0_bs && o.pad < 0)
        return conv3x3_small_cout_run(d.x0, d.w, d.bias, d.res, d.y, o.N, o.c0, o.H, o.W, o.Cout, o.act, st,
                                      p.wsets > 1 ? o.N / p.wsets : 1, p.wsets > 1 ? (long long)o.Cout * o.c0 * 9 : 0,
                                      p.wsets > 1 ? o.Cout : 0);
      for (const Op::Launch& l : o.launches[bs.mode]) {
        ConvExtra ex;
        set_wsets(p, o.N, l.pack.floats, o.Cout, &ex);
        int rc = conv2d_packed_run(launch_desc(d, o, l.role, bs.at(o.pre)), bs.arena + l.pack.off, ex, l.pack.geo, st);
        if (rc != DVSR_OK) return rc;
      }
      return DVSR_OK;
    }
    case OP_DCN: {
      const float* om = bs.at(o.x1);
      const long long bstride = (long long)o.dg * 27 * o.H * o.W;
      if (!p.use_v1 && o.dcn_pack.floats)
        return mdcn_forward_packed_run(bs.at(o.x0), om, bstride, om + (size_t)o.dg * 18 * o.H * o.W, bstride, 1,
                                       bs.arena + o.dcn_pack.off, P[o.pb], bs.at(o.y), o.N, o.c0, o.H, o.W, o.Cout,
                                       o.dg, o.act, st, p.wsets > 1 ? o.N / p.wsets : 1,
                                       p.wsets > 1 ? (long long)o.dcn_pack.floats : 0, p.wsets > 1 ? o.Cout : 0, mdcn_pack_layout(o.W));
      return mdcn_forward_run(bs.at(o.x0), om, bstride, om + (size_t)o.dg * 18 * o.H * o.W, bstride, 1,
                              P[o.pw], P[o.pb], bs.at(o.y), o.N, o.c0, o.H, o.W, o.Cout, 3, 3, 1, 1,
                              1, 1, o.dg, o.act, st);
    }
    case OP_UP:
      return upsample_bilinear_fwd(bs.at(o.x0), bs.at(o.y), o.planes, o.H, o.W, o.S, o.mul, st);
    case OP_POOL:
      return pool3s2_fwd(bs.at(o.x0), bs.at(o.y), bs.at(o.y2), o.planes, o.H, o.W, st);
    case OP_GATE:
      return tsa_gate_fwd(bs.at(o.x0), bs.at(o.x1), bs.at(o.res), bs.at(o.y), bs.at(o.y2), o.gB, o.gN,
                          o.gC, o.gHW, st);
    case OP_BLEND:
      return tsa_blend_fwd(bs.at(o.x0), bs.at(o.x1), bs.at(o.res), bs.at(o.y), o.y.numel, st);
    case OP_PAD:
      if (o.fused_into >= 0) return DVSR_OK;
      return pad_fwd(bs.at(o.x0), bs.at(o.y), o.pmode, o.N, o.c0, o.H, o.W, o.T, st);
    case OP_MEANSUB:
      return meansub_fwd(bs.at(o.x0), bs.at(o.y), bs.at(o.y2), bs.at(o.res), o.N / o.T, o.c0, o.T, o.H, o.W, st);
    case OP_ADDMEAN:
      return addmean_fwd(bs.at(o.x0), bs.at(o.x1), bs.at(o.y), o.N / o.T, o.c0, o.T, (size_t)o.H * o.W, st);
    case OP_ADD:
      return add_out(bs.at(o.y), bs.at(o.x0), bs.at(o.x1), o.y.numel, st);
  }
  return DVSR_ERR_INVALID;
}

}

using namespace dvsr;

extern "C" int dvsr_edvr_plan_create(const dvsr_edvr_config* cfg, int B, int H, int W,
                                     dvsr_edvr_plan** out) {
  return dvsr_edvr_plan_create_grouped(cfg, B, H, W, 1, out);
}

extern "C" int dvsr_edvr_plan_create_grouped(const dvsr_edvr_config* cfg, int B, int H, int W, int grad_groups,
                                             dvsr_edvr_plan** out) {
  return dvsr_edvr_plan_create_ex(cfg, B, H, W, grad_groups, 1, out);
}

extern "C" int dvsr_edvr_plan_create_ex(const dvsr_edvr_config* cfg, int B, int H, int W, int grad_groups,
                                        int weight_sets, dvsr_edvr_plan** out) {
  DVSR_REQUIRE(cfg && out, DVSR_ERR_INVALID, "edvr_plan_create: null argument");
  DVSR_REQUIRE(weight_sets == 1 || weight_sets == grad_groups, DVSR_ERR_INVALID,
               "edvr_plan_create: weight_sets=%d must be 1 or grad_groups=%d", weight_sets, grad_groups);
  DVSR_REQUIRE(B > 0 && H > 0 && W > 0 && H % 4 == 0 && W % 4 == 0, DVSR_ERR_INVALID,
               "edvr_plan_create: B=%d H=%d W=%d (H, W must be positive multiples of 4)", B, H, W);
  DVSR_REQUIRE(grad_groups >= 1 && B % grad_groups == 0, DVSR_ERR_INVALID,
               "edvr_plan_create: grad_groups=%d must divide the batch B=%d", grad_groups, B);
  DVSR_REQUIRE(cfg->nf > 0 && cfg->nf % cfg->groups == 0 && cfg->nframes > 0 && cfg->front_RBs >= 0 &&
                   cfg->back_RBs >= 0, DVSR_ERR_INVALID, "edvr_plan_create: bad network config");
  DVSR_REQUIRE(cfg->scale == 4 || cfg->scale == 2, DVSR_ERR_UNSUPPORTED,
               "edvr_plan_create: scale=%d (2 or 4)", cfg->scale);
  DVSR_REQUIRE(cfg->center >= 0 && cfg->center < cfg->nframes, DVSR_ERR_INVALID,
               "edvr_plan_create: center=%d out of range", cfg->center);
  const int cpg = cfg->nf / cfg->groups;
  DVSR_REQUIRE(cpg == 4 || cpg == 8 || cpg == 16, DVSR_ERR_UNSUPPORTED,
               "edvr_plan_create: nf/groups=%d (supported: 4, 8, 16)", cpg);
  dvsr_edvr_plan* p = new dvsr_edvr_plan();
  p->cfg = *cfg; p->B = B; p->H = H; p->W = W; p->wgroups = grad_groups; p->wsets = weight_sets;
  { const char* v = getenv("DVSR_CONV_V1"); p->use_v1 = v && v[0] == '1'; }
  if (weight_sets > 1 && (p->use_v1 || cpg % 8 != 0)) {
    delete p;
    DVSR_REQUIRE(false, DVSR_ERR_UNSUPPORTED, "edvr_plan_create: per-sample weight sets need the packed kernels (no "
                 "DVSR_CONV_V1) and nf/groups a multiple of 8");
  }
  { const char* v = getenv("DVSR_BWD_STREAMS"); p->side_streams = (v && v[0] == '0') ? 0 : 1; }
  int rc = build_plan(*p);
  if (rc != DVSR_OK) { delete p; return rc; }
  build_backward(*p);
  *out = p;
  return DVSR_OK;
}

extern "C" void dvsr_edvr_plan_destroy(dvsr_edvr_plan* p) {
  if (!p) return;
  if (p->side) (void)hipStreamSynchronize(p->side);
  if (p->ev_fork) {
    (void)hipEventDestroy(p->ev_fork);
    (void)hipEventDestroy(p->ev_join);
  }
  delete p;
}

extern "C" int dvsr_edvr_num_params(const dvsr_edvr_plan* p) { return p ? p->n_params : -1; }

extern "C" int dvsr_edvr_num_launches(const dvsr_edvr_plan* p) { return p ? (int)p->ops.size() : -1; }

extern "C" size_t dvsr_edvr_workspace_bytes(const dvsr_edvr_plan* p, int need_grad) {
  if (!p) return 0;
  size_t b = p->arena_floats * sizeof(float);
  if (need_grad)
    b += (p->arena_floats + p->tmp_floats + p->dpack_floats) * sizeof(float) + p->scratch_bytes + p->wscratch_bytes;
  return b;
}

extern "C" int dvsr_edvr_backward(const dvsr_edvr_plan* p, const float* const* params, const float* x,
                                  const float* grad_out, float* const* grad_params, float* grad_x, void* ws,
                                  size_t ws_bytes, dvsr_stream_t stream) {
  DVSR_REQUIRE(p && params && x && grad_out && grad_params && ws, DVSR_ERR_INVALID, "edvr_backward: null argument");
  DVSR_REQUIRE(!p->bwd_unsupported, DVSR_ERR_UNSUPPORTED, "edvr_backward: the tape holds %s", p->bwd_unsupported);
  DVSR_REQUIRE(ws_bytes >= dvsr_edvr_workspace_bytes(p, 1), DVSR_ERR_WORKSPACE,
               "edvr_backward: workspace %zu < %zu bytes (allocate with need_grad=1 BEFORE the forward)", ws_bytes,
               dvsr_edvr_workspace_bytes(p, 1));
  hipStream_t st = (hipStream_t)stream;
  BBases bs;
  bs.arena = (float*)ws; bs.garena = bs.arena + p->arena_floats; bs.x = x; bs.gx = grad_x; bs.gout = grad_out;
  bs.tmp = bs.garena + p->arena_floats;
  bs.dpack = bs.tmp + p->tmp_floats;
  void* scratch = bs.dpack + p->dpack_floats;
  if (!p->use_v1) {
    int rc = pack_all(*p, params, bs.arena, nullptr, bs.dpack, st);
    if (rc != DVSR_OK) return rc;
  }
  if (grad_x) {
    const size_t n = (size_t)p->B * p->cfg.nframes * 3 * p->H * p->W;
    DVSR_REQUIRE(hipMemsetAsync(grad_x, 0, n * sizeof(float), st) == hipSuccess, DVSR_ERR_HIP,
                 "edvr_backward: memset of grad_x failed");
  }
  bool use_side = p->side_streams != 0;
  if (use_side && !p->ev_fork) {
    if (hipEventCreateWithFlags(&p->ev_fork, hipEventDisableTiming) != hipSuccess ||
        hipEventCreateWithFlags(&p->ev_join, hipEventDisableTiming) != hipSuccess) {
      (void)hipGetLastError();
      p->ev_fork = nullptr;
      use_side = false;
    }
  }
  if (use_side) {
    p->side = side_stream_for(st);
    if (!p->side) use_side = false;
  }
  void* wscratch = (char*)scratch + p->scratch_bytes;
  DVSR_REQUIRE(hipMemsetAsync(wscratch, 0, p->wscratch_bytes, st) == hipSuccess, DVSR_ERR_HIP,
               "edvr_backward: memset of the wgrad scratch failed");
  bool forked = false;
  int last_fork_fwd = -1;
  std::vector<WgradReduceEntry> reduces;
  std::vector<const BOp*> unmaps;
  reduces.reserve(p->bops.size());
  static const int fork_env = [] { const char* v = getenv("DVSR_BWD_FORK_EVERY"); return v ? atoi(v) : 0; }();
  const int fork_every = fork_env > 0 ? fork_env : p->fork_every;
  std::vector<WgradLaunch> waiting;
  int waiting_layers = 0;
  auto flush_waiting = [&]() -> int {
    if (waiting.empty()) return DVSR_OK;
    hipStream_t ws = st;
    if (use_side) {
      DVSR_REQUIRE(hipEventRecord(p->ev_fork, st) == hipSuccess && hipStreamWaitEvent(p->side, p->ev_fork, 0) == hipSuccess,
                   DVSR_ERR_HIP, "edvr_backward: fork to the wgrad stream failed");
      ws = p->side;
      forked = true;
    }
    for (const WgradLaunch& l : waiting) {
      int rc = conv2d_wgrad_launch(l, ws);
      if (rc != DVSR_OK) return rc;
    }
    waiting.clear();
    waiting_layers = 0;
    return DVSR_OK;
  };
  for (const BOp& b : p->bops) {
    int rc = DVSR_OK;
    if (b.type == B_WGRAD) {
      reduces.emplace_back();
      WgradLaunch l;
      rc = prep_wgrad(*p, b, grad_params, bs, (char*)wscratch + b.ws_off, b.ws_bytes, st, &reduces.back(), &l);
      if (rc != DVSR_OK) return rc;
      if (b.fwd != last_fork_fwd) {
        if (waiting_layers >= fork_every) rc = flush_waiting();
        last_fork_fwd = b.fwd;
        ++waiting_layers;
      }
      waiting.push_back(l);
      if (rc == DVSR_OK && (!use_side || !l.geo.row_split)) rc = flush_waiting();
    } else if (b.type == B_WUNMAP) {
      unmaps.push_back(&b);
    } else {
      rc = run_backward_op(*p, b, params, grad_params, bs, scratch, p->scratch_bytes, st);
    }
    if (rc != DVSR_OK) return rc;
  }
  {
    int rc = flush_waiting();
    if (rc != DVSR_OK) return rc;
    hipStream_t ws = use_side && forked ? p->side : st;
    rc = wgrad_reduce_batch(reduces.data(), (int)reduces.size(), ws);
    if (rc != DVSR_OK) return rc;
    for (const BOp* b : unmaps) {
      rc = run_backward_op(*p, *b, params, grad_params, bs, nullptr, 0, ws);
      if (rc != DVSR_OK) return rc;
    }
  }
  if (forked)
    DVSR_REQUIRE(hipEventRecord(p->ev_join, p->side) == hipSuccess &&
                     hipStreamWaitEvent(st, p->ev_join, 0) == hipSuccess,
                 DVSR_ERR_HIP, "edvr_backward: join of the wgrad stream failed");
  return DVSR_OK;
}

extern "C" int dvsr_edvr_num_backward_launches(const dvsr_edvr_plan* p) { return p ? (int)p->bops.size() : -1; }

static FwdMode forward_mode(const dvsr_edvr_plan* p, size_t ws_bytes) {
  return ws_bytes < dvsr_edvr_workspace_bytes(p, 1) ? FWD_NOGRAD : FWD_GRAD;
}

static int run_forward_tape(const dvsr_edvr_plan& p, const float* const* params, const Bases& bs, bool packs_valid, hipStream_t st) {
  if (!p.use_v1 && !packs_valid) {
    int rc = pack_all(p, params, bs.arena, bs.arena, nullptr, st, bs.mode);
    if (rc != DVSR_OK) return rc;
  }
  for (const Op& o : p.ops) {
    int rc = run_forward_op(p, o, params, bs, st);
    if (rc != DVSR_OK) return rc;
  }
  return DVSR_OK;
}

static int edvr_forward_impl(const dvsr_edvr_plan* p, const float* const* params, const float* x, float* out, void* ws,
                             size_t ws_bytes, dvsr_stream_t stream, bool packs_valid);

extern "C" int dvsr_edvr_forward(const dvsr_edvr_plan* p, const float* const* params, const float* x,
                                 float* out, void* ws, size_t ws_bytes, dvsr_stream_t stream) {
  return edvr_forward_impl(p, params, x, out, ws, ws_bytes, stream, false);
}

extern "C" int dvsr_edvr_forward_packed(const dvsr_edvr_plan* p, const float* const* params, const float* x,
                                        float* out, void* ws, size_t ws_bytes, dvsr_stream_t stream) {
  return edvr_forward_impl(p, params, x, out, ws, ws_bytes, stream, true);
}

static int edvr_forward_impl(const dvsr_edvr_plan* p, const float* const* params, const float* x, float* out, void* ws,
                             size_t ws_bytes, dvsr_stream_t stream, bool packs_valid) {
  DVSR_REQUIRE(p && params && x && out && ws, DVSR_ERR_INVALID, "edvr_forward: null argument");
  DVSR_REQUIRE(ws_bytes >= p->arena_floats * sizeof(float), DVSR_ERR_WORKSPACE,
               "edvr_forward: workspace %zu < %zu bytes", ws_bytes, p->arena_floats * sizeof(float));
  return run_forward_tape(*p, params, Bases{(float*)ws, x, out, forward_mode(p, ws_bytes)}, packs_valid, (hipStream_t)stream);
}

static void op_work(const Op& o, const char** kind, double* flops, double* bytes) {
  *flops = 0; *bytes = 0; *kind = "other";
  switch (o.type) {
    case OP_CONV: {
      const int Ho = conv_out(o, o.H), Wo = conv_out(o, o.W);
      const double ctot = o.c0 + o.c1, px = (double)o.N * Ho * Wo;
      *flops = 2.0 * px * o.Cout * ctot * o.ks * o.ks;
      *bytes = 4.0 * ((double)o.N * o.c0 * o.H * o.W + (double)(o.N / o.x1_bdiv) * o.c1 * o.H * o.W +
                      px * o.Cout * (o.res.valid() ? 2 : 1) + (double)o.Cout * ctot * o.ks * o.ks);
      *kind = o.ks == 1 ? "conv1x1" : (o.ks == 2 ? "conv2x2" : (o.stride == 2 ? "conv3x3s2" : "conv3x3s1"));
      break;
    }
    case OP_DCN: {
      const double px = (double)o.N * o.H * o.W;
      *flops = 2.0 * px * o.Cout * o.c0 * 9 + px * o.c0 * 9 * 8.0;
      *bytes = 4.0 * (px * o.c0 + px * o.dg * 27 + px * o.Cout + (double)o.Cout * o.c0 * 9);
      *kind = "mdcn";
      break;
    }
    case OP_UP: *bytes = 4.0 * o.planes * o.H * o.W * (1.0 + o.S * o.S); *kind = "upsample"; break;
    case OP_POOL: *bytes = 4.0 * o.planes * o.H * o.W * 1.5; *kind = "pool"; break;
    case OP_GATE: *bytes = 4.0 * ((double)o.gB * o.gN * o.gC * o.gHW * 3 + (double)o.gB * o.gC * o.gHW +
                                 (double)o.gB * o.gN * o.gHW); *kind = "tsa_gate"; break;
    case OP_BLEND: *bytes = 4.0 * o.y.numel * 4; *kind = "tsa_blend"; break;
    case OP_ADD: *bytes = 4.0 * o.y.numel * 3; *kind = "add"; break;
    case OP_PAD: *bytes = 4.0 * ((double)o.N * o.c0 * o.H * o.W + (double)o.y.numel); *kind = "pad"; break;
    case OP_MEANSUB: *bytes = 4.0 * o.y.numel * 3; *kind = "meansub"; break;
    case OP_ADDMEAN: *bytes = 4.0 * o.y.numel * 2; *kind = "addmean"; break;
  }
}

extern "C" int dvsr_edvr_op_info(const dvsr_edvr_plan* p, int index, char* kind, int kind_cap,
                                 char* name, int name_cap, double* flops, double* bytes) {
  DVSR_REQUIRE(p && kind && name && flops && bytes && index >= 0 && index < (int)p->ops.size(),
               DVSR_ERR_INVALID, "edvr_op_info: bad argument");
  const char* k;
  op_work(p->ops[index], &k, flops, bytes);
  snprintf(kind, kind_cap, "%s", k);
  if (p->ops[index].type == OP_CONV)
  {
    const ConvGeo& g = p->ops[index].launches[FWD_NOGRAD].primary().pack.geo;
    snprintf(name, name_cap, "%s[%d/%d/%d%s]", p->ops[index].name, g.cc, g.th, g.mt, kernel_tag(g.kernel));
  }
  else
    snprintf(name, name_cap, "%s", p->ops[index].name);
  return DVSR_OK;
}

extern "C" int dvsr_edvr_op_launch_count(const dvsr_edvr_plan* p, int index, int nograd) {
  if (!p || index < 0 || index >= (int)p->ops.size()) return -1;
  const Op& o = p->ops[index];
  return o.type == OP_CONV ? o.launches[nograd ? FWD_NOGRAD : FWD_GRAD].n : 1;
}

static int plan_work(const dvsr_edvr_plan* p, double* out9, FwdMode mode) {
  DVSR_REQUIRE(p && out9, DVSR_ERR_INVALID, "edvr_plan_work: null argument");
  double fa = 0, fe = 0, ba = 0, be = 0, fby = 0, f32p[2] = {0, 0}, bfp[2] = {0, 0};
  auto conv_part = [](const Op& o, int ci) {
    return 2.0 * (double)o.N * conv_out(o, o.H) * conv_out(o, o.W) * o.Cout * ci * o.ks * o.ks;
  };
  auto issue = [&](const ConvGeo& g, double f, double* ex, int pass) {
    const double shaped = f * multiplies_per_output_ratio(g.kernel);
    *ex += shaped;
    if (on_bf16_split(g.kernel) || g.bf == 2) bfp[pass] += 6.0 * shaped;
    else if (g.bf == 1) bfp[pass] += shaped;
    else f32p[pass] += shaped;
  };
  for (const Op& o : p->ops) {
    {
      const char* k; double fl, by;
      op_work(o, &k, &fl, &by);
      fby += by;
    }
    if (o.type == OP_CONV) {
      const double f = conv_part(o, o.c0 + o.c1);
      fa += f;
      for (const Op::Launch& l : o.launches[mode])
        issue(l.pack.geo, conv_part(o, l.c) / (l.role == Op::REF_PART ? o.x1_bdiv : 1), &fe, 0);
    } else if (o.type == OP_DCN) {
      const double f = 2.0 * (double)o.N * o.H * o.W * o.Cout * o.c0 * 9;
      fa += f; fe += f; f32p[0] += f;
    }
  }
  for (const BOp& b : p->bops) {
    if (b.fwd < 0) continue;
    const Op& o = p->ops[b.fwd];
    if (b.type == B_WGRAD) {
      const double f = conv_part(o, b.which ? o.c1 : o.c0);
      ba += f; be += f;
      const WgradKernel k = conv2d_wgrad_choose(wgrad_shape(*p, o, b.which)).kernel;
      if (on_bf16_split(k)) bfp[1] += 6.0 * f; else if (on_bf16_pipe(k)) bfp[1] += f; else f32p[1] += f;
    } else if (b.type == B_DGRAD) {
      const double f = conv_part(o, b.which ? o.c1 : o.c0);
      ba += f; issue(o.dgrad[b.which].geo, f, &be, 1);
    } else if (b.type == B_DCN) {
      const double f = 2.0 * 2.0 * (double)o.N * o.H * o.W * o.Cout * o.c0 * 9;
      ba += f; be += f; f32p[1] += f;
    }
  }
  out9[0] = fa; out9[1] = fe; out9[2] = ba; out9[3] = be;
  out9[4] = fby;
  out9[5] = f32p[0]; out9[6] = bfp[0]; out9[7] = f32p[1]; out9[8] = bfp[1];
  return DVSR_OK;
}
extern "C" int dvsr_edvr_plan_work(const dvsr_edvr_plan* p, double* out9) { return plan_work(p, out9, FWD_GRAD); }
extern "C" int dvsr_edvr_plan_work_nograd(const dvsr_edvr_plan* p, double* out9) { return plan_work(p, out9, FWD_NOGRAD); }

extern "C" int dvsr_edvr_forward_timed(const dvsr_edvr_plan* p, const float* const* params,
                                       const float* x, float* out, void* ws, size_t ws_bytes,
                                       dvsr_stream_t stream, float* op_ms) {
  DVSR_REQUIRE(p && params && x && out && ws && op_ms, DVSR_ERR_INVALID, "edvr_forward_timed: null argument");
  DVSR_REQUIRE(ws_bytes >= p->arena_floats * sizeof(float), DVSR_ERR_WORKSPACE,
               "edvr_forward_timed: workspace too small");
  hipStream_t st = (hipStream_t)stream;
  const size_t n = p->ops.size();
  std::vector<hipEvent_t> ev(n + 1);
  for (auto& e : ev) DVSR_REQUIRE(hipEventCreate(&e) == hipSuccess, DVSR_ERR_HIP, "hipEventCreate failed");
  const Bases bs{(float*)ws, x, out, forward_mode(p, ws_bytes)};
  int rc = p->use_v1 ? DVSR_OK : pack_all(*p, params, bs.arena, bs.arena, nullptr, st, bs.mode);
  hipEventRecord(ev[0], st);
  for (size_t i = 0; i < n && rc == DVSR_OK; ++i) {
    rc = run_forward_op(*p, p->ops[i], params, bs, st);
    hipEventRecord(ev[i + 1], st);
  }
  if (rc == DVSR_OK && hipStreamSynchronize(st) != hipSuccess) {
    set_error("edvr_forward_timed: stream synchronize failed");
    rc = DVSR_ERR_HIP;
  }
  if (rc == DVSR_OK)
    for (size_t i = 0; i < n; ++i) hipEventElapsedTime(&op_ms[i], ev[i], ev[i + 1]);
  for (auto& e : ev) hipEventDestroy(e);
  return rc;
}

extern "C" int dvsr_edvr_op_output(const dvsr_edvr_plan* p, int index, int which, int* in_arena, long long* offset_floats,
                                   long long* numel) {
  DVSR_REQUIRE(p && in_arena && offset_floats && numel && index >= 0 && index < (int)p->ops.size() && (which == 0 || which == 1),
               DVSR_ERR_INVALID, "edvr_op_output: bad argument");
  const T& t = which ? p->ops[index].y2 : p->ops[index].y;
  DVSR_REQUIRE(t.valid(), DVSR_ERR_INVALID, "edvr_op_output: launch %d has no output %d", index, which);
  *in_arena = t.space == SP_ARENA;
  *offset_floats = (long long)t.off;
  *numel = (long long)t.numel;
  return DVSR_OK;
}

extern "C" int dvsr_edvr_tensor_info(const dvsr_edvr_plan* p, const char* name, long long* offset_floats,
                                     long long* numel) {
  DVSR_REQUIRE(p && name && offset_floats && numel, DVSR_ERR_INVALID, "edvr_tensor_info: null argument");
  for (const auto& kv : p->named)
    if (kv.first == name && kv.second.space == SP_ARENA) {
      *offset_floats = (long long)kv.second.off;
      *numel = (long long)kv.second.numel;
      return DVSR_OK;
    }
  set_error("edvr_tensor_info: no tensor named '%s'", name);
  return DVSR_ERR_INVALID;
}


struct dvsr_edvr_stream {
  dvsr_edvr_plan extract, fuse;
  int slots = 0;
  dvsr::SlotLayout sl;
  size_t fea_off[3] = {0, 0, 0};
};

extern "C" int dvsr_edvr_stream_create(const dvsr_edvr_config* cfg, int H, int W, int slots, dvsr_edvr_stream** out) {
  DVSR_REQUIRE(cfg && out, DVSR_ERR_INVALID, "edvr_stream_create: null argument");
  DVSR_REQUIRE(H > 0 && W > 0 && H % 4 == 0 && W % 4 == 0, DVSR_ERR_INVALID,
               "edvr_stream_create: H=%d W=%d (H, W must be positive multiples of 4)", H, W);
  DVSR_REQUIRE(cfg->nf > 0 && cfg->groups > 0 && cfg->nf % cfg->groups == 0 && cfg->nframes > 0 && cfg->front_RBs >= 0 &&
                   cfg->back_RBs >= 0, DVSR_ERR_INVALID, "edvr_stream_create: bad network config");
  DVSR_REQUIRE(cfg->nframes <= DVSR_STREAM_MAX_FRAMES, DVSR_ERR_UNSUPPORTED, "edvr_stream_create: nframes=%d (at most %d)",
               cfg->nframes, DVSR_STREAM_MAX_FRAMES);
  DVSR_REQUIRE(slots >= cfg->nframes, DVSR_ERR_INVALID, "edvr_stream_create: slots=%d < nframes=%d", slots, cfg->nframes);
  DVSR_REQUIRE(cfg->scale == 4 || cfg->scale == 2, DVSR_ERR_UNSUPPORTED, "edvr_stream_create: scale=%d (2 or 4)", cfg->scale);
  DVSR_REQUIRE(cfg->center >= 0 && cfg->center < cfg->nframes, DVSR_ERR_INVALID, "edvr_stream_create: center=%d out of range",
               cfg->center);
  const int cpg = cfg->nf / cfg->groups;
  DVSR_REQUIRE(cpg == 4 || cpg == 8 || cpg == 16, DVSR_ERR_UNSUPPORTED, "edvr_stream_create: nf/groups=%d (supported: 4, 8, 16)", cpg);
  dvsr_edvr_stream* s = new dvsr_edvr_stream();
  const char* v1 = getenv("DVSR_CONV_V1");
  int k = 0;
  for (dvsr_edvr_plan* p : {&s->extract, &s->fuse}) {
    p->cfg = *cfg; p->B = 1; p->H = H; p->W = W;
    p->use_v1 = v1 && v1[0] == '1';
    int rc = build_plan(*p, k++ == 0 ? PART_EXTRACT : PART_FUSE);
    if (rc != DVSR_OK) { delete s; return rc; }
  }
  s->slots = slots;
  s->sl = slot_layout(cfg->nf, H, W);
  static const char* const names[3] = {"L1_fea", "L2_fea", "L3_fea"};
  for (int l = 0; l < 3; ++l)
    for (const auto& kv : s->fuse.named)
      if (kv.first == names[l]) s->fea_off[l] = kv.second.off;
  *out = s;
  return DVSR_OK;
}

extern "C" void dvsr_edvr_stream_destroy(dvsr_edvr_stream* s) { delete s; }

extern "C" int dvsr_edvr_stream_num_params(const dvsr_edvr_stream* s) { return s ? s->fuse.n_params : -1; }

extern "C" int dvsr_edvr_stream_num_launches(const dvsr_edvr_stream* s, int which) {
  if (!s) return -1;
  return which ? (int)s->fuse.ops.size() + 1 : (int)s->extract.ops.size();
}

extern "C" size_t dvsr_edvr_stream_cache_bytes(const dvsr_edvr_stream* s) {
  return s ? (size_t)s->slots * s->sl.floats * sizeof(float) : 0;
}

extern "C" size_t dvsr_edvr_stream_workspace_bytes(const dvsr_edvr_stream* s) {
  return s ? (s->fuse.arena_floats + s->extract.arena_floats) * sizeof(float) : 0;
}

static int stream_check(const dvsr_edvr_stream* s, const void* params, const void* cache, size_t cache_bytes, const void* ws,
                        size_t ws_bytes, const char* what) {
  DVSR_REQUIRE(s && params && cache && ws, DVSR_ERR_INVALID, "%s: null argument", what);
  DVSR_REQUIRE(cache_bytes >= dvsr_edvr_stream_cache_bytes(s), DVSR_ERR_INVALID, "%s: cache %zu < %zu bytes", what, cache_bytes,
               dvsr_edvr_stream_cache_bytes(s));
  DVSR_REQUIRE(ws_bytes >= dvsr_edvr_stream_workspace_bytes(s), DVSR_ERR_INVALID, "%s: workspace %zu < %zu bytes", what, ws_bytes,
               dvsr_edvr_stream_workspace_bytes(s));
  DVSR_REQUIRE((uintptr_t)cache % 16 == 0 && (uintptr_t)ws % 16 == 0, DVSR_ERR_INVALID, "%s: cache / workspace not 16-byte aligned", what);
  return DVSR_OK;
}

static int stream_extract_tape(const dvsr_edvr_stream* s, const float* const* params, const float* frame, float* dst, void* ws,
                               int packed, hipStream_t st) {
  return run_forward_tape(s->extract, params, Bases{(float*)ws + s->fuse.arena_floats, frame, dst, FWD_NOGRAD}, packed != 0, st);
}

extern "C" int dvsr_edvr_stream_extract(const dvsr_edvr_stream* s, const float* const* params, const float* frame, int slot,
                                        void* cache, size_t cache_bytes, void* ws, size_t ws_bytes, int packed,
                                        dvsr_stream_t stream) {
  int rc = stream_check(s, params, cache, cache_bytes, ws, ws_bytes, "edvr_stream_extract");
  if (rc != DVSR_OK) return rc;
  DVSR_REQUIRE(frame, DVSR_ERR_INVALID, "edvr_stream_extract: null argument");
  DVSR_REQUIRE(slot >= 0 && slot < s->slots, DVSR_ERR_INVALID, "edvr_stream_extract: slot %d outside [0, %d)", slot, s->slots);
  const dvsr_edvr_plan& p = s->extract;
  hipStream_t st = (hipStream_t)stream;
  float* dst = (float*)cache + (size_t)slot * s->sl.floats;
  rc = stream_extract_tape(s, params, frame, dst, ws, packed, st);
  if (rc != DVSR_OK) return rc;
  hipError_t e = hipMemcpyAsync(dst + s->sl.raw, frame, (size_t)3 * p.H * p.W * sizeof(float), hipMemcpyDeviceToDevice, st);
  DVSR_REQUIRE(e == hipSuccess, DVSR_ERR_HIP, "edvr_stream_extract: copy of the frame: %s", hipGetErrorString(e));
  return DVSR_OK;
}

template <class Ingest>
static int stream_extract_frame(const char* what, const dvsr_edvr_stream* s, const float* const* params, int slot, void* cache,
                                size_t cache_bytes, void* ws, size_t ws_bytes, int packed, dvsr_stream_t stream, Ingest ingest) {
  int rc = stream_check(s, params, cache, cache_bytes, ws, ws_bytes, what);
  if (rc != DVSR_OK) return rc;
  DVSR_REQUIRE(slot >= 0 && slot < s->slots, DVSR_ERR_INVALID, "%s: slot %d outside [0, %d)", what, slot, s->slots);
  const dvsr_edvr_plan& p = s->extract;
  hipStream_t st = (hipStream_t)stream;
  float* dst = (float*)cache + (size_t)slot * s->sl.floats;
  float* raw = dst + s->sl.raw;
  rc = ingest(what, raw, p.H, p.W, st);
  if (rc != DVSR_OK) return rc;
  return stream_extract_tape(s, params, raw, dst, ws, packed, st);
}

template <class Desc>
static auto yuv_ingest_step(const Desc* fd, int pad_mode) {
  return [=](const char* what, float* raw, int H, int W, hipStream_t st) {
    Yuv420 f;
    int rc = yuv420_from(what, fd, &f);
    if (rc == DVSR_OK) rc = frame_ingest_yuv_check(what, f, raw, H, W, pad_mode);
    return rc != DVSR_OK ? rc : frame_ingest_yuv_launch(f, raw, H, W, pad_mode, st);
  };
}

extern "C" int dvsr_edvr_stream_extract_frame(const dvsr_edvr_stream* s, const float* const* params, const void* frame,
                                              const dvsr_frame_desc* fd, int pad_mode, int slot, void* cache,
                                              size_t cache_bytes, void* ws, size_t ws_bytes, int packed, dvsr_stream_t stream) {
  return stream_extract_frame("edvr_stream_extract_frame", s, params, slot, cache, cache_bytes, ws, ws_bytes, packed, stream,
                              [=](const char* what, float* raw, int H, int W, hipStream_t st) {
                                int rc = frame_ingest_check(what, frame, fd, raw, H, W, pad_mode);
                                return rc != DVSR_OK ? rc : frame_ingest_launch(frame, *fd, raw, H, W, pad_mode, st);
                              });
}

extern "C" int dvsr_edvr_stream_extract_frame_yuv(const dvsr_edvr_stream* s, const float* const* params, const dvsr_yuv_desc* fd,
                                                  int pad_mode, int slot, void* cache, size_t cache_bytes, void* ws,
                                                  size_t ws_bytes, int packed, dvsr_stream_t stream) {
  return stream_extract_frame("edvr_stream_extract_frame_yuv", s, params, slot, cache, cache_bytes, ws, ws_bytes, packed, stream,
                              yuv_ingest_step(fd, pad_mode));
}

extern "C" int dvsr_edvr_stream_extract_frame_yuv16(const dvsr_edvr_stream* s, const float* const* params,
                                                    const dvsr_yuv16_desc* fd, int pad_mode, int slot, void* cache,
                                                    size_t cache_bytes, void* ws, size_t ws_bytes, int packed,
                                                    dvsr_stream_t stream) {
  return stream_extract_frame("edvr_stream_extract_frame_yuv16", s, params, slot, cache, cache_bytes, ws, ws_bytes, packed, stream,
                              yuv_ingest_step(fd, pad_mode));
}

extern "C" int dvsr_edvr_stream_fuse(const dvsr_edvr_stream* s, const float* const* params, const int* slots, const void* cache,
                                     size_t cache_bytes, float* out, void* ws, size_t ws_bytes, int packed,
                                     dvsr_stream_t stream) {
  int rc = stream_check(s, params, cache, cache_bytes, ws, ws_bytes, "edvr_stream_fuse");
  if (rc != DVSR_OK) return rc;
  DVSR_REQUIRE(slots && out, DVSR_ERR_INVALID, "edvr_stream_fuse: null argument");
  const dvsr_edvr_plan& p = s->fuse;
  const int Nf = p.cfg.nframes;
  for (int f = 0; f < Nf; ++f)
    DVSR_REQUIRE(slots[f] >= 0 && slots[f] < s->slots, DVSR_ERR_INVALID, "edvr_stream_fuse: slots[%d] = %d outside [0, %d)", f,
                 slots[f], s->slots);
  hipStream_t st = (hipStream_t)stream;
  const float* cf = (const float*)cache;
  const Bases bs{(float*)ws, cf + (size_t)slots[p.cfg.center] * s->sl.floats + s->sl.raw, out, FWD_NOGRAD};
  float* const dst[3] = {bs.arena + s->fea_off[0], bs.arena + s->fea_off[1], bs.arena + s->fea_off[2]};
  rc = stream_gather_run(cf, s->sl.floats, s->sl.off, dst, s->sl.numel, Nf, slots, st);
  if (rc != DVSR_OK) return rc;
  return run_forward_tape(p, params, bs, packed != 0, st);
}


struct dvsr_estimator_plan {
  dvsr_edvr_plan core;
  dvsr_estimator_config ecfg;
};

namespace dvsr {

static int build_estimator(dvsr_estimator_plan& ep) {
  dvsr_edvr_plan& p = ep.core;
  const dvsr_estimator_config& c = ep.ecfg;
  const int video = c.kind == DVSR_ESTIMATOR_MFDN;
  const int B = p.B, Tn = video ? c.nframes : 1, BT = B * Tn, nf = c.nf, ic = c.in_nc;
  int H = p.H, W = p.W;
  Builder b(p);
  const int L = ACT_LRELU, NO = ACT_NONE;
  T none;
  T xin; xin.space = SP_INPUT; xin.off = 0; xin.numel = (size_t)BT * ic * H * W;
  T xm = b.alloc("xm", xin.numel);
  T mean = b.alloc("mean", (size_t)BT * ic);
  {
    Op o; o.type = OP_MEANSUB; o.name = "meansub"; o.x0 = xin; o.y = xm; o.y2 = mean;
    o.res = b.alloc("", (size_t)BT * ic * meansub_slices());
    o.N = BT; o.c0 = ic; o.H = H; o.W = W; o.T = Tn;
    p.ops.push_back(o);
  }
  static const bool fuse_pad = [] { const char* v = getenv("DVSR_EST_FUSE_PAD"); return !(v && v[0] == '0'); }();
  auto fuse = [&](int mode) {
    const int pi = (int)p.ops.size() - 1;
    if (!fuse_pad || pi < 1 || (mode != PAD_REFLECT && mode != PAD_REFLECT_S2D)) return;
    Op& pad = p.ops[pi];
    Op& prod = p.ops[pi - 1];
    if (prod.type != OP_CONV || prod.y.space != SP_ARENA || prod.y.off != pad.x0.off || prod.ps || prod.res.valid()) return;
    prod.pad_out = mode == PAD_REFLECT ? PS_PAD_REFLECT : PS_PAD_REFLECT_S2D;
    prod.ypad = pad.y;
    pad.fused_into = pi - 1;
  };
  auto conv3 = [&](const char* pn, const char* cn, T x, int cin, int cout, int mode, bool first) {
    T xp = b.padop(pn, x, mode, BT, cin, H, W, Tn);
    fuse(mode);
    if (first) p.ops.back().no_dgrad = 1;
    const int cin_eff = mode == PAD_REPL_T3 ? 3 * cin : cin;
    T y = b.conv(cn, b.take(), xp, cin_eff, none, 0, BT, H + 2, W + 2, cout, 3, 1, L, none, 0, 1, 0, 0, T(), 0);
    if (first) p.ops.back().no_dgrad = 1;
    return y;
  };
  auto conv4s2 = [&](const char* pn, const char* cn, T x, int cin, int cout) {
    T xp = b.padop(pn, x, PAD_REFLECT_S2D, BT, cin, H, W, Tn);
    fuse(PAD_REFLECT_S2D);
    T y = b.conv(cn, b.take(), xp, 4 * cin, none, 0, BT, (H + 2) / 2, (W + 2) / 2, cout, 2, 1, L, none, 0, 1, 0, 0,
                 T(), 0, 1);
    H /= 2; W /= 2;
    return y;
  };
  T y;
  if (video) {
    y = conv3("pad0", "conv0", xm, ic, nf, PAD_REPL_T3, true);
    y = conv3("pad1", "conv1", y, nf, nf, PAD_REFLECT, false);
    y = conv4s2("pad2", "conv2", y, nf, 2 * nf);
    if (c.scale == 4) y = conv4s2("pad3", "conv3", y, 2 * nf, nf);
    else y = conv3("pad3", "conv3", y, 2 * nf, nf, PAD_REFLECT, false);
    y = conv3("pad4", "conv4", y, nf, nf, PAD_REFLECT, false);
    y = conv3("pad5", "conv5", y, nf, nf, PAD_REPL_T3, false);
  } else {
    y = conv3("pad0", "conv0", xm, ic, nf, PAD_REFLECT, true);
    y = conv3("pad1", "conv1", y, nf, nf, PAD_REFLECT, false);
    y = conv3("pad2", "conv2", y, nf, nf, PAD_REFLECT, false);
    y = conv4s2("pad3", "conv3", y, nf, 2 * nf);
    y = conv3("pad4", "conv4", y, 2 * nf, 2 * nf, PAD_REFLECT, false);
    y = conv3("pad5", "conv5", y, 2 * nf, nf, PAD_REFLECT, false);
  }
  y = b.conv("conv6", b.take(), y, nf, none, 0, BT, H, W, ic, 1, 1, NO, none, 0, 1, 0, 0, T(), 0);
  {
    Op o; o.type = OP_ADDMEAN; o.name = "addmean"; o.x0 = y; o.x1 = mean;
    o.y.space = SP_OUTPUT; o.y.off = 0; o.y.numel = (size_t)BT * ic * H * W;
    o.N = BT; o.c0 = ic; o.H = H; o.W = W; o.T = Tn;
    p.ops.push_back(o);
  }
  p.n_params = b.pcur;
  return DVSR_OK;
}

}

extern "C" int dvsr_estimator_plan_create(const dvsr_estimator_config* cfg, int B, int H, int W,
                                          dvsr_estimator_plan** out) {
  return dvsr_estimator_plan_create_grouped(cfg, B, H, W, 1, out);
}

extern "C" int dvsr_estimator_plan_create_grouped(const dvsr_estimator_config* cfg, int B, int H, int W, int grad_groups,
                                                  dvsr_estimator_plan** out) {
  return dvsr_estimator_plan_create_ex(cfg, B, H, W, grad_groups, 1, out);
}

extern "C" int dvsr_estimator_plan_create_ex(const dvsr_estimator_config* cfg, int B, int H, int W, int grad_groups,
                                             int weight_sets, dvsr_estimator_plan** out) {
  DVSR_REQUIRE(cfg && out, DVSR_ERR_INVALID, "estimator_plan_create: null argument");
  DVSR_REQUIRE(weight_sets == 1 || weight_sets == grad_groups, DVSR_ERR_INVALID,
               "estimator_plan_create: weight_sets=%d must be 1 or grad_groups=%d", weight_sets, grad_groups);
  DVSR_REQUIRE(grad_groups >= 1 && B > 0 && B % grad_groups == 0, DVSR_ERR_INVALID,
               "estimator_plan_create: grad_groups=%d must divide the batch B=%d", grad_groups, B);
  DVSR_REQUIRE(cfg->kind == DVSR_ESTIMATOR_MFDN || cfg->kind == DVSR_ESTIMATOR_SFDN, DVSR_ERR_INVALID,
               "estimator_plan_create: kind=%d", cfg->kind);
  DVSR_REQUIRE(cfg->nf > 0 && cfg->in_nc > 0, DVSR_ERR_INVALID, "estimator_plan_create: nf=%d in_nc=%d", cfg->nf,
               cfg->in_nc);
  if (cfg->kind == DVSR_ESTIMATOR_MFDN) {
    DVSR_REQUIRE(cfg->scale == 2 || cfg->scale == 4, DVSR_ERR_UNSUPPORTED,
                 "estimator_plan_create: MFDN scale=%d (2 or 4, LRimg_estimator.py:72)", cfg->scale);
    DVSR_REQUIRE(cfg->nframes > 0, DVSR_ERR_INVALID, "estimator_plan_create: nframes=%d", cfg->nframes);
  } else {
    DVSR_REQUIRE(cfg->scale == 2, DVSR_ERR_UNSUPPORTED, "estimator_plan_create: SFDN is x2 only (got %d)", cfg->scale);
  }
  const int s = cfg->scale;
  DVSR_REQUIRE(B > 0 && H >= 2 * s && W >= 2 * s && H % s == 0 && W % s == 0, DVSR_ERR_INVALID,
               "estimator_plan_create: B=%d H=%d W=%d (H, W must be multiples of the scale %d)", B, H, W, s);
  dvsr_estimator_plan* ep = new dvsr_estimator_plan();
  ep->ecfg = *cfg;
  dvsr_edvr_plan& p = ep->core;
  p.cfg = dvsr_edvr_config{cfg->nf, cfg->nframes, 1, 0, 0, cfg->scale, 0, 0};
  {
    const char* v = getenv("DVSR_EST_SPLIT");
    if (!v || atoi(v)) { p.cfg.bf16_mfma = 2; p.split_any_pad = true; }
  }
  p.B = B; p.H = H; p.W = W; p.wgroups = grad_groups; p.wsets = weight_sets;
  { const char* v = getenv("DVSR_BWD_STREAMS"); p.side_streams = (v && v[0] == '0') ? 0 : 1; }
  p.fork_every = 1;
  int rc = build_estimator(*ep);
  if (rc != DVSR_OK) { delete ep; return rc; }
  build_backward(p);
  *out = ep;
  return DVSR_OK;
}

extern "C" void dvsr_estimator_plan_destroy(dvsr_estimator_plan* ep) {
  if (!ep) return;
  dvsr_edvr_plan& p = ep->core;
  if (p.side) (void)hipStreamSynchronize(p.side);
  if (p.ev_fork) {
    (void)hipEventDestroy(p.ev_fork);
    (void)hipEventDestroy(p.ev_join);
  }
  delete ep;
}

extern "C" int dvsr_estimator_num_params(const dvsr_estimator_plan* ep) { return ep ? ep->core.n_params : -1; }

extern "C" int dvsr_estimator_num_launches(const dvsr_estimator_plan* ep, int backward) {
  if (!ep) return -1;
  return backward ? (int)ep->core.bops.size() : (int)ep->core.ops.size();
}

extern "C" int dvsr_estimator_plan_work(const dvsr_estimator_plan* ep, double* out9) {
  DVSR_REQUIRE(ep, DVSR_ERR_INVALID, "estimator_plan_work: null plan");
  return dvsr_edvr_plan_work(&ep->core, out9);
}

extern "C" size_t dvsr_estimator_workspace_bytes(const dvsr_estimator_plan* ep, int need_grad) {
  return ep ? dvsr_edvr_workspace_bytes(&ep->core, need_grad) : 0;
}

extern "C" int dvsr_estimator_forward(const dvsr_estimator_plan* ep, const float* const* params, const float* x,
                                      float* out, void* ws, size_t ws_bytes, dvsr_stream_t stream) {
  DVSR_REQUIRE(ep, DVSR_ERR_INVALID, "estimator_forward: null plan");
  return dvsr_edvr_forward(&ep->core, params, x, out, ws, ws_bytes, stream);
}

extern "C" int dvsr_estimator_backward(const dvsr_estimator_plan* ep, const float* const* params, const float* x,
                                       const float* grad_out, float* const* grad_params, void* ws, size_t ws_bytes,
                                       dvsr_stream_t stream) {
  DVSR_REQUIRE(ep, DVSR_ERR_INVALID, "estimator_backward: null plan");
  return dvsr_edvr_backward(&ep->core, params, x, grad_out, grad_params, nullptr, ws, ws_bytes, stream);
}
```

### dynavsr_amd/csrc/kernels.h

```cpp
#pragma once
#include "../../include/dynavsr_hip.h"
#include "common.h"

namespace dvsr {

struct ConvExtra {
  int wt = 0;
  int w_ctot = 0, w_coff = 0;
  int in_ps = 0;
  int in_dil = 0, Hs = 0, Ws = 0;
  int accum = 0;
  const float* gmask = nullptr;
  int gmask_act = 0;
  int wdiv = 1; long long w_gs = 0; int b_gs = 0;
};
int conv2d_run(const dvsr_conv2d_desc& d, const ConvExtra& ex, hipStream_t st);

int mdcn_forward_run(const float* x, const float* off, long long off_bs, const float* msk,
                     long long msk_bs, int mask_logit, const float* w, const float* b, float* out,
                     int N, int C, int H, int W, int Cout, int kh, int kw, int stride, int pad,
                     int dil, int groups, int dg, int act, hipStream_t st);

enum class ConvKernel : int {
  REG = 0,
  DMA_HALO = 1,
  ROW_SPLIT = 2,
  WINO_F2 = 3,
  WINO_F2_BF16 = 4,
  WINO_F4 = 5,
};
enum class PackLayout : int {
  INTERLEAVED = 0,
  DMA_ORDER = 1,
  ROW_SPLIT = 2,
  WINO_F2 = 3,
  WINO_F2_BF16 = 4,
  WINO_F4 = 5,
  DCN_SPLIT = 6,
};
constexpr PackLayout pack_layout(ConvKernel k) { return static_cast<PackLayout>(static_cast<int>(k)); }
constexpr bool is_winograd(ConvKernel k) { return k == ConvKernel::WINO_F2 || k == ConvKernel::WINO_F2_BF16 || k == ConvKernel::WINO_F4; }
constexpr bool on_bf16_split(ConvKernel k) { return k == ConvKernel::WINO_F2_BF16 || k == ConvKernel::WINO_F4; }
constexpr bool needs_dma_halo_inputs(ConvKernel k) { return k == ConvKernel::DMA_HALO || is_winograd(k); }
constexpr double multiplies_per_output_ratio(ConvKernel k) { return k == ConvKernel::WINO_F4 ? 0.25 : (is_winograd(k) ? 16.0 / 36.0 : 1.0); }
constexpr const char* kernel_tag(ConvKernel k) {
  return k == ConvKernel::WINO_F4 ? "w5" : (k == ConvKernel::WINO_F2_BF16 ? "w3" : (k == ConvKernel::WINO_F2 ? "w" : (k == ConvKernel::REG ? "" : "d")));
}
constexpr bool has_own_pack_kernel(PackLayout l) { return static_cast<int>(l) >= static_cast<int>(PackLayout::WINO_F2); }

struct PackEntry {
  const float* w; float* P;
  int Cout, Ctot, KK, CC, wt, w_ctot, w_coff, ncb, nchunks, pch;
  int bf = 0;
  PackLayout layout = PackLayout::INTERLEAVED;
};
struct PackTable {
  int n;
  PackEntry e[48];
};
int pack_weights_run(const PackTable& t, hipStream_t st);
struct ConvGeo { int cc, th, mt; int bf = 0; ConvKernel kernel = ConvKernel::REG; };
enum ConvAllow : int {
  ALLOW_NONE = 0,
  ALLOW_KSPLIT = 1,
  ALLOW_DMA_HALO = 2,
  ALLOW_WINO = 4,
  ALLOW_WINO_F4 = 8,
  ALLOW_SHARED_DEVICE = 16,
  ALLOW_ONLY_F4 = 32,
};
constexpr ConvAllow operator|(ConvAllow a, ConvAllow b) { return static_cast<ConvAllow>(static_cast<int>(a) | static_cast<int>(b)); }
constexpr ConvAllow without(ConvAllow a, ConvAllow b) { return static_cast<ConvAllow>(static_cast<int>(a) & ~static_cast<int>(b)); }
ConvGeo conv2_choose(int ks, int stride, int N, int Ho, int Wo, int Cout, int Ctot, ConvAllow allow = ALLOW_KSPLIT);
size_t conv2_pack_floats(int ks, int Cout, int Ctot, int cc, int bf, PackLayout layout);
PackEntry conv2_pack_entry(const float* w, float* P, int ks, int Cout, int Ctot, int cc, int bf, PackLayout layout, int wt = 0,
                           int w_ctot = 0, int w_coff = 0);
inline size_t conv2_pack_floats(int ks, int Cout, int Ctot, const ConvGeo& g) {
  return conv2_pack_floats(ks, Cout, Ctot, g.cc, g.bf, pack_layout(g.kernel));
}
inline PackEntry conv2_pack_entry(const float* w, float* P, int ks, int Cout, int Ctot, const ConvGeo& g, int wt = 0, int w_ctot = 0,
                                  int w_coff = 0) {
  return conv2_pack_entry(w, P, ks, Cout, Ctot, g.cc, g.bf, pack_layout(g.kernel), wt, w_ctot, w_coff);
}
double conv2_f4_occupied_cycles(int N, int Ho, int Wo, int Cout, int Ctot, int th);
int pack_weights_wino_run(const PackTable& t, hipStream_t st);
int pack_weights_wino3_run(const PackTable& t, hipStream_t st);
int pack_weights_wino5_run(const PackTable& t, hipStream_t st);
int conv2d_packed_run(const dvsr_conv2d_desc& d, const float* wp, const ConvExtra& ex, const ConvGeo& geo,
                      hipStream_t st);

bool conv1x1_dual_ok(const float* x, const float* w0, const float* w1, const float* y0, const float* y1, int Cin, long long HW);
int conv1x1_dual_run(const float* x, const float* w0, const float* b0, const float* w1, const float* b1, float* y0, float* y1,
                     int N, int Cin, int HW, int act, hipStream_t st, int wdiv = 1, long long w_gs = 0, int b_gs = 0);
int conv3x3_small_cout_run(const float* x, const float* w, const float* bias, const float* res, float* y, int N,
                           int C, int H, int W, int Cout, int act, hipStream_t st, int wdiv = 1, long long w_gs = 0,
                           int b_gs = 0);

struct WgradReduceEntry {
  float* partial; float* dbp; float* dW; float* db;
  int nslot, KK, OP, CP, Cout, Cin, Ctot, c_off;
  int ngroups = 1;
  long long dW_gs = 0, db_gs = 0;
};
constexpr int WGRAD_REDUCE_BATCH = 44;
struct WgradReduceTable {
  int n;
  WgradReduceEntry e[WGRAD_REDUCE_BATCH];
};
int wgrad_reduce_batch(const WgradReduceEntry* entries, int n, hipStream_t st, int blocks = 96);
struct WgradDesc {
  const float* x = nullptr; long long x_bs = 0; int x_bdiv = 1;
  const float* gy = nullptr; int gy_ps = 0;
  float* dW = nullptr; float* db = nullptr;
  int N = 0, Cin = 0, H = 0, W = 0, Cout = 0, Ctot = 0, c_off = 0, ks = 0, stride = 1, pad = -1;
  int groups = 1; long long dW_gs = 0, db_gs = 0;
  int mode = 0;
};
enum class WgradKernel : int {
  SIMPLE = 0,
  PIPE = 1,
  BF16 = 2,
  SPLIT_SCALAR = 3,
  SPLIT_VECTOR = 4,
  SPLIT_WAVE8 = 5,
};
constexpr bool on_bf16_pipe(WgradKernel k) { return k >= WgradKernel::BF16; }
constexpr bool on_bf16_split(WgradKernel k) { return k >= WgradKernel::SPLIT_SCALAR; }
struct WgradGeo {
  WgradKernel kernel = WgradKernel::PIPE;
  int row_split = 0;
  int vx = 0;
  int nsplit = 1, nslot = 1;
  dim3 grid; int block = 256;
};
WgradGeo conv2d_wgrad_choose(const WgradDesc& d);
bool wgrad_split3_default();
size_t conv2d_wgrad_workspace_bytes(const WgradDesc& d);
int conv2d_wgrad_run(const WgradDesc& d, void* ws, size_t ws_bytes, hipStream_t st, int scratch_is_zero = 0,
                     WgradReduceEntry* defer = nullptr);
size_t mdcn_backward_workspace_bytes(int N, int C, int H, int W, int Cout, int stride, int pad, int dil, int groups = 1);
int mdcn_backward_run(const float* x, const float* off, long long off_bs, const float* msk, long long msk_bs,
                      int mask_logit, const float* w, const float* gout, float* gx, float* goff,
                      long long goff_bs, float* gmsk, long long gmsk_bs, float* gw, float* gb, int N, int C,
                      int H, int W, int Cout, int stride, int pad, int dil, int dg, void* ws,
                      size_t ws_bytes, hipStream_t st, int groups = 1, long long gw_gs = 0, long long gb_gs = 0,
                      long long w_gs = 0);

int mdcn_forward_packed_run(const float* x, const float* off, long long off_bs, const float* msk,
                            long long msk_bs, int mask_logit, const float* wp, const float* b, float* out,
                            int N, int C, int H, int W, int Cout, int dg, int act, hipStream_t st, int wdiv = 1,
                            long long w_gs = 0, int b_gs = 0, PackLayout layout = PackLayout::INTERLEAVED);
int mdcn_fwd_variant();
int mdcn_pack_floats();
PackLayout mdcn_pack_layout(int W);
int pack_weights_dcn3_run(const PackTable& t, hipStream_t st);

struct DcnK2 {
  const float* x; const float* off; const float* msk; const float* wp; const float* bias; float* out;
  long long off_bstride, msk_bstride;
  int mask_logit;
  int N, C, H, W, Cout, dg, act;
  int tiles_x, tiles_y, ntiles, ncb, nchunks;
  int wdiv = 1; long long w_gs = 0; int b_gs = 0;
#ifdef DVSR_CONV_TRACE
  long long* trace;
#endif
};
// ... 87 lines not shown
```

### dynavsr_amd/csrc/small_grid.h

```cpp
#pragma once
#include <hip/amd_detail/amd_hip_unsafe_atomics.h>

#include <type_traits>

#include "common.h"
#include "kernels.h"

namespace dvsr {

struct ConvK2 {
  const float* x0; const float* x1; const float* wp; const float* bias; const float* res; float* y;
  int N, c0, c1, H, W, Cout, Ho, Wo, pad, act, ps, x1_bdiv;
  long long x0_bs, x1_bs;
  int tiles_x, tiles_y, ntiles, ncb, nchunks, nitems, tiles_per_xcd;
  int in_ps, in_dil, Hs, Ws, accum;
  const float* gmask; int gmask_act;
  int wdiv = 1; long long w_gs = 0; int b_gs = 0;
  const float* pre = nullptr; int pre_bdiv = 1; long long pre_bs = 0;
#ifdef DVSR_CONV_TRACE
  int ablate;
  long long* trace;
#endif
};

struct WgradK {
  const float* x; const float* gy; float* partial; float* dbp;
  long long x_bs;
  int x_bdiv;
  int N, Cin, H, W, Cout, Ho, Wo, pad, gy_ps;
  int tiles_x, tiles_y, ntiles, nsplit, nob, ncb, nslot;
  int ngroups = 1, gtiles = 0;
  int vx = 0;
#ifdef DVSR_CONV_TRACE
  int noflush = 0;
  long long* trace = nullptr;
#endif
};

struct WgSpan { int tile0, tile_end, slot; };
__device__ __forceinline__ WgSpan wg_span(const WgradK& a, int split) {
  int g = 0, s = split;
  if (a.ngroups > 1) { g = split / a.nsplit; s = split - g * a.nsplit; }
  return WgSpan{g * a.gtiles + s, (g + 1) * a.gtiles, g * a.nslot + s % a.nslot};
}

int conv2d_packed_prepare(const dvsr_conv2d_desc& d, const float* wp, const ConvExtra& ex, const ConvGeo& geo, ConvK2* k);
struct WgradLaunch { WgradK k; WgradGeo geo; int ks; };
int conv2d_wgrad_prepare(const WgradDesc& d, void* ws, size_t ws_bytes, hipStream_t st, int scratch_is_zero, WgradReduceEntry* entry,
                         WgradLaunch* out);
int conv2d_wgrad_launch(const WgradLaunch& l, hipStream_t st);
int conv2d_wino_launch(const ConvK2& k, int th, hipStream_t st);
int conv2d_wino3_launch(const ConvK2& k, int th, hipStream_t st);
int conv2d_wino4_launch(const ConvK2& k, int th, hipStream_t st);
int conv2d_wino5_launch(const ConvK2& k, int th, hipStream_t st);
int conv2d_wgrad_bf16_launch(const WgradLaunch& l, hipStream_t st);
int conv2d_wgrad_split3_launch(const WgradLaunch& l, hipStream_t st);

template <int MT, int NT>
struct KsShape {
  static constexpr int KK = 9, CC = 32, KQ4 = 4, TW = 32;
  static constexpr int IH = NT + 2, IW = TW + 2, PLANE = IH * IW;
  static constexpr int E = (PLANE + 127) / 128;
  static constexpr int IN_FLOATS = KQ4 * PLANE * 8;
  static constexpr int HALF = KK * KQ4 * 2 * 32 * 4;
  static constexpr int RED_FLOATS = 4 * MT * NT * 16 * 64;
  static constexpr int LDS_FLOATS = 2 * IN_FLOATS > RED_FLOATS ? 2 * IN_FLOATS : RED_FLOATS;
  static constexpr size_t LDS_BYTES = (size_t)LDS_FLOATS * sizeof(float);
};

template <int MT, int NT>
__device__ __forceinline__ void conv2d_ksplit_item(const ConvK2& a, const int id, float* const smem) {
  using Sh = KsShape<MT, NT>;
  constexpr int KK = Sh::KK, CC = Sh::CC, IH = Sh::IH, IW = Sh::IW, PLANE = Sh::PLANE;

  const int q_ = id >> 3;
  const int cbi = q_ % a.ncb;
  const int j_ = q_ / a.ncb;
  const int tile = (id & 7) * a.tiles_per_xcd + j_;
  if (j_ >= a.tiles_per_xcd || tile >= a.ntiles) return;
  const int tx_ = tile % a.tiles_x;
  const int t2 = tile / a.tiles_x;
  const int ty_ = t2 % a.tiles_y;
  const int n = t2 / a.tiles_y;
  const int oy0 = ty_ * NT, ox0 = tx_ * Sh::TW;
  const int iy0 = oy0 - a.pad, ix0 = ox0 - a.pad;

  const int tid = threadIdx.x, lane = tid & 63;
  const int wave = __builtin_amdgcn_readfirstlane(tid >> 6);
  const int lo = lane & 31, hi = lane >> 5;
  const int Ctot = a.c0 + a.c1;
  const size_t HW = (size_t)a.H * a.W;
  const float* x0n = a.x0 + (size_t)n * a.x0_bs;
  const float* x1n = a.c1 ? a.x1 + (size_t)(n / a.x1_bdiv) * a.x1_bs : x0n;

  constexpr int E = Sh::E;
  const int chalf = wave >> 1;
  unsigned eoffb[E];
  int elds[E];
  bool e_in[E], e_ok[E];
#pragma unroll
  for (int m = 0; m < E; ++m) {
    const int e_ = (tid & 127) + 128 * m;
    const int eiy = e_ / IW, eix = e_ - eiy * IW;
    const int gy_ = iy0 + eiy, gx_ = ix0 + eix;
    e_in[m] = e_ < PLANE;
    e_ok[m] = e_in[m] && (unsigned)gy_ < (unsigned)a.H && (unsigned)gx_ < (unsigned)a.W;
    eoffb[m] = e_ok[m] ? (unsigned)(gy_ * a.W + gx_) * 4u : 0u;
    elds[m] = (eiy * 2) * IW + eix;
  }

  float rin[16][E];
  auto issue_halo = [&](int k) {
    const int cbase = k * CC;
    const bool second = cbase >= a.c0;
    const float* b = second ? x1n : x0n;
    const int nci = second ? a.c1 : a.c0;
    const int ci = (second ? cbase - a.c0 : cbase) + 16 * chalf;
    const char* p = reinterpret_cast<const char*>(b + (size_t)(ci < nci ? ci : nci - 1) * HW);
#pragma unroll
    for (int c = 0; c < 16; ++c) {
#pragma unroll
      for (int m = 0; m < E; ++m) rin[c][m] = *reinterpret_cast<const float*>(p + eoffb[m]);
      p += (ci + c + 1 < nci) ? HW * 4 : 0;
    }
  };
  auto write_halo = [&](int buf) {
    float* s_in = smem + buf * Sh::IN_FLOATS;
#pragma unroll
    for (int m = 0; m < E; ++m) {
      if (!e_in[m]) continue;
#pragma unroll
      for (int qq = 0; qq < 2; ++qq)
#pragma unroll
        for (int h2 = 0; h2 < 2; ++h2) {
          const bool ok = e_ok[m];
          const f32x4 v = {ok ? rin[8 * qq + h2][m] : 0.f, ok ? rin[8 * qq + 2 + h2][m] : 0.f,
                           ok ? rin[8 * qq + 4 + h2][m] : 0.f, ok ? rin[8 * qq + 6 + h2][m] : 0.f};
          *reinterpret_cast<f32x4*>(s_in + ((size_t)((2 * chalf + qq) * IH * 2 * IW) + elds[m] + h2 * IW) * 4) = v;
        }
    }
  };

  const float* wp_cb = wset_ptr(a.wp, a.w_gs, n, a.wdiv) + ((size_t)((cbi * MT) >> 1) * a.nchunks * 2 + ((cbi * MT) & 1)) * Sh::HALF +
                       (size_t)(wave * 64 + lane) * 4;
  f32x4 Ag[3][MT];
  auto load_a = [&](int k, int tap, int slot) {
    const float* b = wp_cb + (size_t)k * (2 * Sh::HALF) + tap * (Sh::KQ4 * 64 * 4);
#pragma unroll
    for (int mt = 0; mt < MT; ++mt) Ag[slot][mt] = *reinterpret_cast<const f32x4*>(b + mt * Sh::HALF);
  };

  f32x16 acc[MT][NT];
#pragma unroll
  for (int i = 0; i < MT; ++i)
#pragma unroll
    for (int j = 0; j < NT; ++j)
#pragma unroll
      for (int r = 0; r < 16; ++r) acc[i][j][r] = 0.f;

  constexpr int AD = 2;
  load_a(0, 0, 0);
  load_a(0, 1, 1);
  issue_halo(0);
  write_halo(0);
  __syncthreads();

  auto chunk = [&](int k, auto has_next_tag) {
    constexpr bool HAS_NEXT = decltype(has_next_tag)::value;
    const float* s_in = smem + (k & 1) * Sh::IN_FLOATS + (size_t)(wave * IH * 2 * IW) * 4;
    if (HAS_NEXT) {
      issue_halo(k + 1);
// ... 396 lines not shown
```

### dynavsr_amd/engine.py

```python
import ctypes
import threading

import torch

from . import _lib as L

_plans = {}
_GEOMETRY_ENV = ("DVSR_CONV_WINO", "DVSR_CONV_WINO3", "DVSR_CONV_WINO5", "DVSR_CONV_V1", "DVSR_EST_SPLIT", "DVSR_EST_SPLIT2", "DVSR_FUSE_ACT_BWD",
                 "DVSR_BWD_STREAMS", "DVSR_PCD_HOIST")
_PROCESS_ENV = ("DVSR_CONV_LDS", "DVSR_CONV_LAST_MFMA", "DVSR_SPLIT_TH8_FROM", "DVSR_WGRAD_SPLIT3",
                "DVSR_WGRAD_WIDE", "DVSR_WGRAD_S3V", "DVSR_WGRAD_S3_KYS_BELOW", "DVSR_WGRAD_S3_WGS", "DVSR_WGRAD_S3W", "DVSR_DCN_FWD", "DVSR_DCN_BWD",
                "DVSR_EST_FUSE_PAD", "DVSR_FUSE_RES_BWD", "DVSR_BWD_FORK_EVERY", "DVSR_BWD_PROBE", "DVSR_TSA_DUAL", "DVSR_TSA_V",
                "DVSR_DEGRADE_GENERIC", "DVSR_UP2")
_process_env_seen = None


def _check_process_env():
    import os
    import warnings
    global _process_env_seen
    now = tuple(os.environ.get(k) for k in _PROCESS_ENV)
    if _process_env_seen is None:
        _process_env_seen = now
        return
    for k, a, b in zip(_PROCESS_ENV, _process_env_seen, now):
        if a != b:
            warnings.warn("dynavsr_amd: %s=%r now, but the native library read %r when the first plan of this process was built "
                          "and keeps that value (switches of this kind are read once per process: set them before the first "
                          "plan, one process per value)" % (k, b, a), RuntimeWarning, stacklevel=3)
    _process_env_seen = now


_WORK_KEYS = ("fwd_algorithmic", "fwd_executed", "bwd_algorithmic", "bwd_executed", "fwd_bytes",
              "fwd_f32_pipe", "fwd_bf16_pipe", "bwd_f32_pipe", "bwd_bf16_pipe")


def _env_key():
    import os
    return tuple(os.environ.get(k) for k in _GEOMETRY_ENV)


class Plan:

    def __init__(self, cfg, b, h, w, grad_groups=1, weight_sets=1):
        self.key = (cfg, b, h, w, grad_groups, weight_sets)
        cfg = tuple(cfg) + (0,) * (8 - len(cfg))
        self.cfg = dict(zip(("nf", "nframes", "groups", "front_RBs", "back_RBs", "scale", "center", "bf16_mfma"), cfg))
        self.b, self.h, self.w, self.grad_groups, self.weight_sets = b, h, w, grad_groups, weight_sets
        self._h = ctypes.c_void_p()
        L.check(L.lib().dvsr_edvr_plan_create_ex(L.EdvrConfig(*cfg), b, h, w, grad_groups, weight_sets,
                                                 ctypes.byref(self._h)), "dvsr_edvr_plan_create_ex")
        self.n_params = L.lib().dvsr_edvr_num_params(self._h)
        self.n_launches = L.lib().dvsr_edvr_num_launches(self._h)
        self.n_backward_launches = L.lib().dvsr_edvr_num_backward_launches(self._h)

    def workspace_bytes(self, need_grad):
        return int(L.lib().dvsr_edvr_workspace_bytes(self._h, int(need_grad)))

    def forward(self, params, x, out, ws, packed=False):
        arr = (ctypes.c_void_p * len(params))(*[L.ptr(p) for p in params])
        fn = L.lib().dvsr_edvr_forward_packed if packed else L.lib().dvsr_edvr_forward
        L.check(fn(self._h, arr, L.ptr(x), L.ptr(out), ws.data_ptr(), ws.numel() * ws.element_size(), L.stream()),
                "dvsr_edvr_forward_packed" if packed else "dvsr_edvr_forward")

    def backward(self, params, x, gout, gparams, gx, ws):
        arr = (ctypes.c_void_p * len(params))(*[L.ptr(p) for p in params])
        garr = (ctypes.c_void_p * len(gparams))(*[L.ptr(g) for g in gparams])
        L.check(L.lib().dvsr_edvr_backward(self._h, arr, L.ptr(x), L.ptr(gout), garr, L.ptr(gx),
                                           ws.data_ptr(), ws.numel() * ws.element_size(), L.stream()),
                "dvsr_edvr_backward")

    def forward_timed(self, params, x, out, ws):
        arr = (ctypes.c_void_p * len(params))(*[L.ptr(p) for p in params])
        ms = (ctypes.c_float * self.n_launches)()
        L.check(L.lib().dvsr_edvr_forward_timed(self._h, arr, L.ptr(x), L.ptr(out), ws.data_ptr(),
                                                ws.numel() * ws.element_size(), L.stream(), ms),
                "dvsr_edvr_forward_timed")
        return list(ms)

    def work(self, nograd=False):
        out = (ctypes.c_double * 9)()
        fn = L.lib().dvsr_edvr_plan_work_nograd if nograd else L.lib().dvsr_edvr_plan_work
        L.check(fn(self._h, ctypes.byref(out)), "dvsr_edvr_plan_work")
        return dict(zip(_WORK_KEYS, out))

    def op_output(self, ws, index, which=0):
        ia, off, n = ctypes.c_int(), ctypes.c_longlong(), ctypes.c_longlong()
        L.check(L.lib().dvsr_edvr_op_output(self._h, index, which, ctypes.byref(ia), ctypes.byref(off), ctypes.byref(n)),
                "dvsr_edvr_op_output")
        if not ia.value:
            return None
        return ws.view(torch.float32)[off.value:off.value + n.value]

    def op_info(self):
        out = []
        kind, name = ctypes.create_string_buffer(32), ctypes.create_string_buffer(64)
        fl, by = ctypes.c_double(), ctypes.c_double()
        for i in range(self.n_launches):
            L.check(L.lib().dvsr_edvr_op_info(self._h, i, kind, 32, name, 64, ctypes.byref(fl),
                                              ctypes.byref(by)), "dvsr_edvr_op_info")
            out.append((kind.value.decode(), name.value.decode(), fl.value, by.value))
        return out

    def tensor(self, ws, name, shape=None):
        off, n = ctypes.c_longlong(), ctypes.c_longlong()
        L.check(L.lib().dvsr_edvr_tensor_info(self._h, name.encode(), ctypes.byref(off),
                                              ctypes.byref(n)), "dvsr_edvr_tensor_info")
        t = ws.view(torch.float32)[off.value:off.value + n.value]
        return t.view(shape) if shape is not None else t

    def __del__(self):
        try:
            if self._h:
                L.lib().dvsr_edvr_plan_destroy(self._h)
        except Exception:
            pass


def get_plan(cfg, b, h, w, device=None, grad_groups=1, weight_sets=1):
    dev = torch.cuda.current_device() if device is None else torch.device(device).index
    key = (tuple(cfg), b, h, w, dev, torch.cuda.current_stream(dev).cuda_stream, grad_groups, weight_sets, _env_key())
    p = _plans.get(key)
    if p is None:
        _check_process_env()
        p = _plans[key] = Plan(tuple(cfg), b, h, w, grad_groups, weight_sets)
    return p


def _stash(ctx, plan, ws, x, params):
    ctx.plan, ctx.ws, ctx.x, ctx.params = plan, ws, x, params
    ctx.versions = [p._version for p in params]


def _check_stash(ctx, what):
    if ctx.ws is None:
        raise RuntimeError("%s: backward called a second time -- the activation arena was released after the "
                           "first one (the tape is first-order and single-use, like once_differentiable in "
                           "deform_conv.py:123)" % what)
    for i, (p, v) in enumerate(zip(ctx.params, ctx.versions)):
        if p._version != v:
            raise RuntimeError("%s: parameter %d was modified in place between forward and backward (version %d -> "
                               "%d); the gradient would be taken at the wrong weights" % (what, i, v, p._version))


def _prep(t):
    if t.dtype != torch.float32:
        t = t.float()
    return t.contiguous()


_grad_mode = threading.local()


class _TapeFunction(torch.autograd.Function):

    @classmethod
    def apply(cls, *args, **kwargs):
        _grad_mode.enabled = torch.is_grad_enabled()
        return super().apply(*args, **kwargs)


def _need_grad(ctx):
# ... 370 lines not shown
```

Measured before the change: 264.3 frames/s.

## Make the Winograd F4 conv kernel persistent with an atomic work queue and prefetch

```diff
diff --git a/dynavsr_amd/csrc/conv2d_v2.hip b/dynavsr_amd/csrc/conv2d_v2.hip
--- a/dynavsr_amd/csrc/conv2d_v2.hip
+++ b/dynavsr_amd/csrc/conv2d_v2.hip
@@ -926,6 +926,7 @@
   k.in_ps = ex.in_ps; k.in_dil = ex.in_dil; k.Hs = ex.Hs; k.Ws = ex.Ws; k.accum = ex.accum;
   k.gmask = ex.gmask; k.gmask_act = ex.gmask_act;
   k.wdiv = ex.wdiv > 0 ? ex.wdiv : 1; k.w_gs = ex.w_gs; k.b_gs = ex.b_gs;
+  k.queue = geo.kernel == ConvKernel::WINO_F4 ? ex.queue : nullptr;
   DVSR_REQUIRE(!d.pre || (geo.kernel == ConvKernel::WINO_F4 && !d.res && d.pixel_shuffle == 0 && ((uintptr_t)d.pre & 15) == 0),
                DVSR_ERR_UNSUPPORTED, "conv2d_packed: a pre-activation addend needs the F(4x4, 3x3) kernel, a 16-byte aligned tensor, "
                "no residual and no PixelShuffle");
@@ -1049,6 +1050,7 @@
                        d.x0_bstride % 4 == 0 && d.x1_bstride % 4 == 0 && (d.H * d.W) % 4 == 0;
   return op_pack(d.ks, 1, d.pad, d.N, d.H, d.W, Cout, Ctot, d.c1 == 0 || d.c0 % 32 == 0, aligned, d.pre != nullptr);
 }
+size_t op_queue_offset(size_t pack_floats) { return (pack_floats * sizeof(float) + 255) & ~(size_t)255; }
 int op_run(const dvsr_conv2d_desc& d, const dvsr::ConvExtra& ex, int Cout, int Ctot, void* ws, size_t bytes, hipStream_t st) {
   using namespace dvsr;
   DVSR_REQUIRE((d.ks == 1 || d.ks == 3 || d.ks == 7 || d.ks == 9) && d.stride == 1 && d.pad == d.ks / 2, DVSR_ERR_UNSUPPORTED,
@@ -1067,7 +1069,13 @@
   t.e[0] = conv2_pack_entry(d.w, (float*)ws, d.ks, Cout, Ctot, o.geo, ex.wt, ex.w_ctot, ex.w_coff);
   int rc = pack_weights_run(t, st);
   if (rc) return rc;
-  return conv2d_packed_run(d, (const float*)ws, ex, o.geo, st);
+  ConvExtra exq = ex;
+  const size_t qoff = op_queue_offset(o.floats);
+  if (o.geo.kernel == ConvKernel::WINO_F4 && bytes >= qoff + sizeof(int)) {
+    exq.queue = reinterpret_cast<int*>((char*)ws + qoff);
+    DVSR_REQUIRE(hipMemsetAsync(exq.queue, 0, sizeof(int), st) == hipSuccess, DVSR_ERR_HIP, "conv2d (packed): memset of the item counter failed");
+  }
+  return conv2d_packed_run(d, (const float*)ws, exq, o.geo, st);
 }
 }
 
@@ -1081,7 +1089,7 @@
   if (d->ks == 3)
     for (const dvsr::PackLayout l : {dvsr::PackLayout::WINO_F2_BF16, dvsr::PackLayout::WINO_F4})
       w = std::max(w, std::max(dvsr::conv2_pack_floats(3, d->Cout, ctot, 8, 0, l), dvsr::conv2_pack_floats(3, ctot, d->Cout, 8, 0, l)));
-  return std::max(std::max(a, b), std::max(c, w)) * sizeof(float);
+  return op_queue_offset(std::max(std::max(a, b), std::max(c, w))) + 256;
 }
 
 extern "C" int dvsr_conv2d_packed_geometry(const dvsr_conv2d_desc* d, int geo[4]) {
diff --git a/dynavsr_amd/csrc/conv2d_wino5.hip b/dynavsr_amd/csrc/conv2d_wino5.hip
--- a/dynavsr_amd/csrc/conv2d_wino5.hip
+++ b/dynavsr_amd/csrc/conv2d_wino5.hip
@@ -7,14 +7,16 @@
 namespace dvsr {
 
 #ifdef DVSR_CONV_TRACE
-#define W5_STAMP(i)                                                                                       \
-  do {                                                                                                    \
-    if (a.trace && threadIdx.x == 0) a.trace[(size_t)blockIdx.x * 64 + (i)] = __builtin_readcyclecounter(); \
+#define W5_STAMP_T(t, i)                                                                             \
+  do {                                                                                               \
+    if (a.trace && threadIdx.x == (t)) a.trace[(size_t)item * 64 + (i)] = __builtin_readcyclecounter(); \
   } while (0)
+#define W5_STAMP(i) W5_STAMP_T(0, i)
 #else
-#define W5_STAMP(i) \
-  do {              \
+#define W5_STAMP_T(t, i) \
+  do {                   \
   } while (0)
+#define W5_STAMP(i) W5_STAMP_T(0, i)
 #endif
 
 typedef float w5f2 __attribute__((ext_vector_type(2)));
@@ -35,7 +37,10 @@
   static constexpr int VIMG = 36 * 3 * 32 * 4;
   static constexpr int XCH = 6 * 16 * 64 * 4;
   static constexpr int LOOP = 2 * RAWPAD + 2 * VIMG;
-  static constexpr size_t LDS_BYTES = (size_t)(LOOP > XCH ? LOOP : XCH) * sizeof(float);
+  static constexpr int MAPF = LOOP > XCH ? LOOP : XCH;
+  static_assert(XCH <= 2 * VIMG && 2 * RAWPAD + XCH <= MAPF, "an exchange image and the next tile's raw chunks are disjoint");
+  static constexpr size_t LDS_BYTES = (size_t)MAPF * sizeof(float) + 16;
+
 };
 
 constexpr int w5_waitcnt(int vm, int lgkm) { return (vm & 15) | (7 << 4) | ((lgkm & 15) << 8) | ((vm >> 4) << 14); }
@@ -97,48 +102,98 @@
 }
 
 template <int TC, bool RES, bool R16, bool PRE>
-__global__ __launch_bounds__(1024) void conv2d_wino5_kernel(ConvK2 a) {
+__global__ __launch_bounds__(1024) void conv2d_wino5_kernel(ConvK2 a0) {
   static_assert(!PRE || (R16 && !RES), "the addend is read by the sixteen-reader epilogue, never beside a residual");
   using Sh = Wino5Shape<TC>;
   constexpr int IH = Sh::IH, RP = Sh::RP, GR = Sh::GR;
   constexpr int CHF = IH * RP;
   constexpr int QF = 768 * 4;
   extern __shared__ __attribute__((aligned(16))) float smem[];
-  float* const raw0 = smem;
-  unsigned* const vimg0 = reinterpret_cast<unsigned*>(smem + 2 * Sh::RAWPAD);
-
-  const int id = blockIdx.x;
-  const int q_ = id >> 3;
-  const int cbi = q_ % a.ncb;
-  const int j_ = q_ / a.ncb;
-  const int tile = (id & 7) * a.tiles_per_xcd + j_;
-  if (j_ >= a.tiles_per_xcd || tile >= a.ntiles) return;
-  const int tx_ = tile % a.tiles_x;
-  const int t2 = tile / a.tiles_x;
-  const int ty_ = t2 % a.tiles_y;
-  const int n = t2 / a.tiles_y;
-  const int oy0 = ty_ * Sh::OH, ox0 = tx_ * Sh::OW;
-
-  const int tid = threadIdx.x, lane = tid & 63;
-  const int wave = __builtin_amdgcn_readfirstlane(tid >> 6);
-  const int lo = lane & 31, hi = lane >> 5;
-  const size_t HW = (size_t)a.H * a.W;
+  int* const mail = reinterpret_cast<int*>(smem + Sh::MAPF);
+
+  const int wave = __builtin_amdgcn_readfirstlane(threadIdx.x >> 6);
   auto fence = [&]() __attribute__((always_inline)) { __builtin_amdgcn_sched_barrier(0); };
   auto lds_barrier = [&]() __attribute__((always_inline)) {
     asm volatile("s_waitcnt lgkmcnt(0)" ::: "memory");
     __builtin_amdgcn_s_barrier();
     asm volatile("" ::: "memory");
   };
+  struct Item { int cbi, n, oy0, ox0; bool ok; };
+  auto item_ok = [&](const auto& a, int id) __attribute__((always_inline)) {
+    const int j_ = (id >> 3) / a.ncb;
+    return j_ < a.tiles_per_xcd && (id & 7) * a.tiles_per_xcd + j_ < a.ntiles;
+  };
+  auto item_at = [&](const auto& a, int id) __attribute__((always_inline)) {
+    const int q_ = id >> 3;
+    const int j_ = q_ / a.ncb;
+    const int tile = (id & 7) * a.tiles_per_xcd + j_;
+    const int t2 = tile / a.tiles_x;
+    return Item{q_ - j_ * a.ncb, t2 / a.tiles_y, (t2 % a.tiles_y) * Sh::OH, (tile - t2 * a.tiles_x) * Sh::OW,
+                j_ < a.tiles_per_xcd && tile < a.ntiles};
+  };
+  auto take_item = [&](const auto& a) __attribute__((always_inline)) {
+    int nx = a.nitems;
+    int* const q = a.queue;
+    if (q) {
+      do nx = (int)gridDim.x + atomicAdd(q, 1);
+      while (nx < a.nitems && !item_ok(a, nx));
+    }
+    return nx;
+  };
+  int item = blockIdx.x;
+  auto lane_id = [&]() __attribute__((always_inline)) {
+    unsigned ones = ~0u;
+    asm volatile("" : "+s"(ones));
+    return (int)__builtin_amdgcn_mbcnt_hi(ones, __builtin_amdgcn_mbcnt_lo(ones, 0u));
+  };
+  typedef const ConvK2 __attribute__((address_space(4))) ArgsK;
+  ArgsK* ap = (ArgsK*)__builtin_amdgcn_kernarg_segment_ptr();
+  struct Pro {
+    const float *x0, *x1, *wp;
+    long long x0_bs, x1_bs, w_gs;
+    int c0, c1, H, W, x1_bdiv, nchunks, wdiv, ncb, tiles_x, tiles_y, tiles_per_xcd, ntiles, nitems;
+    int* queue;
+  };
+  Pro p{a0.x0, a0.x1, a0.wp, a0.x0_bs, a0.x1_bs, a0.w_gs, a0.c0, a0.c1, a0.H, a0.W, a0.x1_bdiv, a0.nchunks, a0.wdiv, a0.ncb, a0.tiles_x,
+        a0.tiles_y, a0.tiles_per_xcd, a0.ntiles, a0.nitems, a0.queue};
+#ifdef DVSR_CONV_TRACE
+  int item_prev = -1;
+#endif
+  for (int nth = 0;; ++nth) {
+  const int par = nth & 1;
+  const bool fetched = nth > 0;
+  asm volatile("" : "+s"(ap));
+  ArgsK& a = *ap;
+  if (nth) p = Pro{a.x0, a.x1, a.wp, a.x0_bs, a.x1_bs, a.w_gs, a.c0, a.c1, a.H, a.W, a.x1_bdiv, a.nchunks, a.wdiv, a.ncb, a.tiles_x,
+                   a.tiles_y, a.tiles_per_xcd, a.ntiles, a.nitems, a.queue};
+  Item it = item_at(p, item);
+  if (nth == 0 && !it.ok) {
+    if (!p.queue) return;
+    if (threadIdx.x == 0) *mail = take_item(p);
+    lds_barrier();
+    item = __builtin_amdgcn_readfirstlane(*mail);
+    lds_barrier();
+    if (item >= p.nitems) return;
+    it = item_at(p, item);
+  }
+  const int cbi = it.cbi, n = it.n, oy0 = it.oy0, ox0 = it.ox0;
+  float* const raw0 = smem + (par ? 2 * Sh::VIMG : 0);
+  float* const raw0_next = smem + (par ? 0 : 2 * Sh::VIMG);
+  unsigned* const vimg0 = reinterpret_cast<unsigned*>(smem + (par ? 0 : 2 * Sh::RAWPAD));
+  float* const xch0 = smem + (par ? 2 * Sh::RAWPAD : 0);
+  int next = p.nitems;
   W5_STAMP(0);
 #ifdef DVSR_CONV_TRACE
-  if (a.trace && threadIdx.x == 0) a.trace[(size_t)blockIdx.x * 64 + 60] = __builtin_amdgcn_s_memrealtime();
-#endif
-
-  auto read16 = [&](int m) __attribute__((always_inline)) {
-    int le = lane;
-    asm volatile("" : "+v"(le));
+  if (a.trace && threadIdx.x == 0) {
+    a.trace[(size_t)item * 64 + 60] = __builtin_amdgcn_s_memrealtime();
+    a.trace[(size_t)item * 64 + 1] = item_prev;
+  }
+#endif
+
+  auto read16 = [&](const auto& a, int m) __attribute__((always_inline)) {
+    const int le = lane_id();
     const int rq_r = wave & 3, cp_r = wave >> 2;
-    const float* const xr = smem + (rq_r * 64 + le) * 4 + cp_r;
+    const float* const xr = xch0 + (rq_r * 64 + le) * 4 + cp_r;
     const int lo_e = le & 31, hi_e = le >> 5;
     const int trow_e = lo_e / TC, tcol_e = lo_e - trow_e * TC;
     const int oy = oy0 + 4 * trow_e, ox = ox0 + 4 * tcol_e;
@@ -195,32 +250,37 @@
   };
 
   if (wave >= 12) {
-    const int pw = wave - 12, ptid = tid - 768;
-    const float* x0n = a.x0 + (size_t)n * a.x0_bs;
-    const float* x1n = a.c1 ? a.x1 + (size_t)(n / a.x1_bdiv) * a.x1_bs : x0n;
+    const int lane = lane_id(), hi = lane >> 5;
+    const int pw = wave - 12, ptid = pw * 64 + lane;
+    const float* x0n = p.x0 + (size_t)n * p.x0_bs;
+    const float* x1n = p.c1 ? p.x1 + (size_t)(n / p.x1_bdiv) * p.x1_bs : x0n;
     static_assert(IH * GR * 4 == 720, "a channel quad is 720 groups");
     unsigned hoff[3];
-#pragma unroll
-    for (int jj = 0; jj < 3; ++jj) {
-      const int L = jj * 256 + ptid;
-      const int cq = L / (IH * GR), rr = L - cq * (IH * GR);
-      const int iy = rr / GR, g = rr - iy * GR;
-      const int gy = oy0 - 1 + iy, gx = ox0 - 4 + 4 * g;
-      const bool live = L < 4 * IH * GR;
-      const bool ok = live && (unsigned)gy < (unsigned)a.H && (unsigned)gx < (unsigned)a.W;
-      hoff[jj] = ok ? (unsigned)(((size_t)cq * HW + (size_t)gy * a.W + gx) * 4) : 0x80000000u;
-      if (live && !ok) {
-#pragma unroll
-        for (int bb = 0; bb < 4; ++bb) *reinterpret_cast<f32x4*>(raw0 + (bb >> 1) * Sh::RAWPAD + (bb & 1) * QF + L * 4) = f32x4{0.f, 0.f, 0.f, 0.f};
-      }
-    }
-    const unsigned chunk_bytes = (unsigned)(Sh::CC * HW * 4), quad_bytes = (unsigned)(4 * HW * 4);
-    auto issue_raw = [&](int k) __attribute__((always_inline)) {
+    auto halo_of = [&](const auto& a, int ty0, int tx0, float* rb, bool fill) __attribute__((always_inline)) {
+      const size_t HW = (size_t)a.H * a.W;
+#pragma unroll
+      for (int jj = 0; jj < 3; ++jj) {
+        const int L = jj * 256 + ptid;
+        const int cq = L / (IH * GR), rr = L - cq * (IH * GR);
+        const int iy = rr / GR, g = rr - iy * GR;
+        const int gy = ty0 - 1 + iy, gx = tx0 - 4 + 4 * g;
+        const bool live = L < 4 * IH * GR;
+        const bool ok = live && (unsigned)gy < (unsigned)a.H && (unsigned)gx < (unsigned)a.W;
+        hoff[jj] = ok ? (unsigned)(((size_t)cq * HW + (size_t)gy * a.W + gx) * 4) : 0x80000000u;
+        if (fill && live && !ok) {
+#pragma unroll
+          for (int bb = 0; bb < 4; ++bb) *reinterpret_cast<f32x4*>(rb + (bb >> 1) * Sh::RAWPAD + (bb & 1) * QF + L * 4) = f32x4{0.f, 0.f, 0.f, 0.f};
+        }
+      }
+    };
+    auto issue_raw = [&](const auto& a, int k, const float* xa, const float* xb, float* rb) __attribute__((always_inline)) {
+      const size_t HW = (size_t)a.H * a.W;
+      const unsigned chunk_bytes = (unsigned)(Sh::CC * HW * 4), quad_bytes = (unsigned)(4 * HW * 4);
       const bool live = k < a.nchunks;
       const bool second = k * Sh::CC >= a.c0;
       const unsigned soff = live ? (unsigned)(second ? k - a.c0 / Sh::CC : k) * chunk_bytes : 0u;
-      const __amdgpu_buffer_rsrc_t rs = w5_rsrc(second ? x1n : x0n, live ? 0x7fffffff : 0);
-      float* dst = raw0 + (k & 1) * Sh::RAWPAD + 256 * pw;
+      const __amdgpu_buffer_rsrc_t rs = w5_rsrc(second ? xb : xa, live ? 0x7fffffff : 0);
+      float* dst = rb + (k & 1) * Sh::RAWPAD + 256 * pw;
 #pragma unroll
       for (int jj = 0; jj < 3; ++jj) {
         w5_dma16(rs, dst + jj * 1024, hoff[jj], soff);
@@ -296,25 +356,32 @@
       }
       finish_pair(ra, rb, vw05);
     };
-    issue_raw(0);
-    issue_raw(1);
-    __builtin_amdgcn_s_waitcnt(w5_waitcnt(6, 0));
+    halo_of(p, oy0, ox0, raw0, !fetched);
+    if (!fetched) {
+      issue_raw(p, 0, x0n, x1n, raw0);
+      issue_raw(p, 1, x0n, x1n, raw0);
+      __builtin_amdgcn_s_waitcnt(w5_waitcnt(6, 0));
+    } else {
+      __builtin_amdgcn_s_waitcnt(w5_waitcnt(0, 0));
+      W5_STAMP_T(768, 45);
+    }
     __builtin_amdgcn_s_barrier();
     asm volatile("" ::: "memory");
     produce();
     __builtin_amdgcn_s_waitcnt(w5_waitcnt(0, 0));
     __builtin_amdgcn_s_barrier();
     asm volatile("" ::: "memory");
+    next = __builtin_amdgcn_readfirstlane(*mail);
     int vstep = Sh::VIMG, rstep = Sh::RAWPAD;
     vw12 += vstep; vw34 += vstep; vw05 += vstep; prd += rstep;
     __builtin_amdgcn_s_setprio(3);
-    for (int k = 0; k < a.nchunks; ++k) {
+    for (int k = 0; k < p.nchunks; ++k) {
 
 #ifndef W5_NODMA
-      issue_raw(k + 2);
+      issue_raw(p, k + 2, x0n, x1n, raw0);
 #endif
 #ifndef W5_NOPROD
-      if (k + 1 < a.nchunks) produce();
+      if (k + 1 < p.nchunks) produce();
 #endif
       __builtin_amdgcn_s_waitcnt(w5_waitcnt(0, 0));
       __builtin_amdgcn_s_barrier();
@@ -322,25 +389,38 @@
       vw12 -= vstep; vw34 -= vstep; vw05 -= vstep; prd -= rstep;
       vstep = -vstep; rstep = -rstep;
     }
+    __builtin_amdgcn_s_setprio(0);
+    lds_barrier();
+    ArgsK* ape = ap;
+    asm volatile("" : "+s"(ape));
+    ArgsK& ae = *ape;
+    if (next < ae.nitems) {
+      W5_STAMP_T(768, 43);
+      const Item nt = item_at(ae, next);
+      const float* x0m = ae.x0 + (size_t)nt.n * ae.x0_bs;
+      const float* x1m = ae.c1 ? ae.x1 + (size_t)(nt.n / ae.x1_bdiv) * ae.x1_bs : x0m;
+      halo_of(ae, nt.oy0, nt.ox0, raw0_next, true);
+      fence();
+      issue_raw(ae, 0, x0m, x1m, raw0_next);
+      issue_raw(ae, 1, x0m, x1m, raw0_next);
+      W5_STAMP_T(768, 44);
+    }
     if constexpr (R16) {
-      __builtin_amdgcn_s_setprio(0);
+      lds_barrier(); read16(ae, 0);
       lds_barrier();
-      lds_barrier(); read16(0);
-      lds_barrier();
-      lds_barrier(); read16(1);
+      lds_barrier(); read16(ae, 1);
     } else {
-      lds_barrier(); lds_barrier(); lds_barrier(); lds_barrier();
-    }
-    return;
-  }
-  {
+      lds_barrier(); lds_barrier(); lds_barrier();
+    }
+  } else {
+    const int lane = lane_id(), lo = lane & 31, hi = lane >> 5;
     const int cxi = wave % 6, cmh = wave / 6;
     f32x16 acc[6];
 #pragma unroll
     for (int v = 0; v < 6; ++v)
 #pragma unroll
       for (int r = 0; r < 16; ++r) acc[v][r] = 0.f;
-    const float* wp_cb = wset_ptr(a.wp, a.w_gs, n, a.wdiv) + (size_t)cbi * a.nchunks * W5_PCH;
+    const float* wp_cb = wset_ptr(p.wp, p.w_gs, n, p.wdiv) + (size_t)cbi * p.nchunks * W5_PCH;
     const __amdgpu_buffer_rsrc_t wrsrc = w5_rsrc(wp_cb, -1);
     const unsigned avoff = (unsigned)(lane * 16);
     const int asb = (cxi * 3 * 2 + cmh) * 3072;
@@ -375,15 +455,27 @@
 #endif
       c = __builtin_amdgcn_mfma_f32_32x32x16_bf16(__builtin_bit_cast(w5bf8, av), __builtin_bit_cast(w5bf8, bv), c, 0, 0, 0);
     };
+    int taken = 0;
+    int zero = 0;
+    asm volatile("" : "+v"(zero));
+    if (wave == 0 && lane == 0 && p.queue) taken = atomicAdd(p.queue + zero, 1);
     static_for<0, 3>([&](auto g_) __attribute__((always_inline)) { gldA(g_, 0); });
+    lds_barrier();
+    if (wave == 0) {
+      if (lane == 0) {
+        int nx = p.queue ? (int)gridDim.x + taken : p.nitems;
+        if (nx < p.nitems && !item_ok(p, nx)) nx = take_item(p);
+        *mail = nx;
+      }
+      asm volatile("s_waitcnt lgkmcnt(0)" ::: "memory");
+    }
     __builtin_amdgcn_s_barrier();
     asm volatile("" ::: "memory");
-    __builtin_amdgcn_s_barrier();
-    asm volatile("" ::: "memory");
+    next = __builtin_amdgcn_readfirstlane(*mail);
     int vstep = Sh::VIMG;
-    for (int k = 0; k < a.nchunks; ++k) {
+    for (int k = 0; k < p.nchunks; ++k) {
       ldB(std::integral_constant<int, 0>{}); ldB(std::integral_constant<int, 1>{});
-      const int knext = k + 1 < a.nchunks ? k + 1 : k;
+      const int knext = k + 1 < p.nchunks ? k + 1 : k;
       static_for<0, 18>([&](auto f_) __attribute__((always_inline)) {
         constexpr int F = decltype(f_)::value, NU = F / 3, I = F % 3;
         constexpr int XS = NU & 1;
@@ -412,8 +504,10 @@
     }
   W5_STAMP(40);
 
-  int lane_e = lane;
-  asm volatile("" : "+v"(lane_e));
+  const int lane_e = lane_id();
+  ArgsK* ape = ap;
+  asm volatile("" : "+s"(ape));
+  ArgsK& a = *ape;
   f32x16 Z[4];
 #pragma unroll
   for (int r = 0; r < 16; ++r) {
@@ -424,12 +518,8 @@
     Z[2][r] = __builtin_fmaf(4.f, sb, sa);
     Z[3][r] = __builtin_fmaf(8.f, db, da) + acc[5][r];
   }
-  float* const xw = smem + (cxi * 16 * 64 + lane_e) * 4;
+  float* const xw = xch0 + (cxi * 16 * 64 + lane_e) * 4;
   const int rq_r = wave & 3, cp_r = wave >> 2;
-  const float* const xr = smem + (rq_r * 64 + lane_e) * 4 + cp_r * 2;
-  const int lo_e = lane_e & 31, hi_e = lane_e >> 5;
-  const int trow_e = lo_e / TC, tcol_e = lo_e - trow_e * TC;
-  const int oy = oy0 + 4 * trow_e, ox = ox0 + 4 * tcol_e;
   const size_t HWo = (size_t)a.Ho * a.Wo;
   const float slope = a.act == ACT_LRELU ? 0.1f : (a.act == ACT_RELU ? 0.f : 1.f);
   const float* bias = wset_ptr(a.bias, a.b_gs, n, a.wdiv);
@@ -448,8 +538,13 @@
     W5_STAMP(52 + 4 * m);
     lds_barrier();
     W5_STAMP(53 + 4 * m);
-    if constexpr (R16) read16(m);
+    if constexpr (R16) read16(a, m);
     else if (wave < 8) {
+      const int lane_r = lane_id();
+      const float* const xr = xch0 + (rq_r * 64 + lane_r) * 4 + cp_r * 2;
+      const int lo_e = lane_r & 31, hi_e = lane_r >> 5;
+      const int trow_e = lo_e / TC, tcol_e = lo_e - trow_e * TC;
+      const int oy = oy0 + 4 * trow_e, ox = ox0 + 4 * tcol_e;
       const int co0 = cbi * 64 + m * 32 + 8 * rq_r + 4 * hi_e + 2 * cp_r;
       float y[2][4][4];
 #pragma unroll
@@ -526,11 +621,17 @@
   __builtin_amdgcn_s_waitcnt(0);
   W5_STAMP(42);
   if (a.trace && threadIdx.x == 0) {
-    a.trace[(size_t)blockIdx.x * 64 + 61] = __builtin_amdgcn_s_memrealtime();
-    a.trace[(size_t)blockIdx.x * 64 + 63] = __builtin_amdgcn_s_getreg((4) | (0 << 6) | (31 << 11));
-    a.trace[(size_t)blockIdx.x * 64 + 62] = __builtin_amdgcn_s_getreg((20) | (0 << 6) | (31 << 11));
-  }
-#endif
+    a.trace[(size_t)item * 64 + 61] = __builtin_amdgcn_s_memrealtime();
+    a.trace[(size_t)item * 64 + 63] = __builtin_amdgcn_s_getreg((4) | (0 << 6) | (31 << 11));
+    a.trace[(size_t)item * 64 + 62] = __builtin_amdgcn_s_getreg((20) | (0 << 6) | (31 << 11));
+  }
+#endif
+  }
+  if (next >= p.nitems) break;
+#ifdef DVSR_CONV_TRACE
+  item_prev = item;
+#endif
+  item = next;
   }
 }
 
@@ -547,7 +648,11 @@
   k.ncb = ceil_div(k.Cout, 64);
   k.tiles_per_xcd = ceil_div(k.ntiles, 8);
   k.nitems = k.tiles_per_xcd * 8 * k.ncb;
-  hipLaunchKernelGGL(kern, dim3(k.nitems), dim3(1024), Sh::LDS_BYTES, st, k);
+  int grid = k.nitems;
+  const char* qv = getenv("DVSR_CONV_WINO5_QUEUE");
+  if (k.queue && !(qv && atoi(qv) == 0) && k.nitems > device_cus()) grid = device_cus();
+  else k.queue = nullptr;
+  hipLaunchKernelGGL(kern, dim3(grid), dim3(1024), Sh::LDS_BYTES, st, k);
   return check_launch("conv2d_wino5_kernel");
 }
 
diff --git a/dynavsr_amd/csrc/engine.hip b/dynavsr_amd/csrc/engine.hip
--- a/dynavsr_amd/csrc/engine.hip
+++ b/dynavsr_amd/csrc/engine.hip
@@ -43,7 +43,7 @@
   struct PackSlot { ConvGeo geo = {8, 8, 2}; size_t off = 0, floats = 0; };
   PackSlot dgrad[2], dcn_pack;
   enum LaunchRole { WHOLE, MAIN_PART, REF_PART };
-  struct Launch { PackSlot pack; int c_off = 0, c = 0; LaunchRole role = WHOLE; };
+  struct Launch { PackSlot pack; int c_off = 0, c = 0; LaunchRole role = WHOLE; int qslot = -1; };
   struct LaunchList {
     int n = 0; Launch l[2];
     const Launch* begin() const { return l; }
@@ -88,6 +88,8 @@
   std::vector<std::pair<size_t, size_t>> allocs;
   std::vector<dvsr::BOp> bops;
   size_t dpack_floats = 0;
+  int nqueue = 0;
+  size_t queue_off = 0;
   bool use_v1 = false;
   size_t tmp_floats = 0;
   size_t scratch_bytes = 0;
@@ -183,6 +185,9 @@
     o.pre = arena_alloc(p, "", (size_t)(N / o.x1_bdiv) * Cout * Ho * Wo);
     nograd = pair;
   }
+  for (int i = 0; i < nograd.n; ++i)
+    if (nograd.l[i].pack.geo.kernel == ConvKernel::WINO_F4) nograd.l[i].qslot = p.nqueue + i;
+  p.nqueue += 2;
   for (int which = 0; which < 2; ++which) {
     const int ci = which ? c1 : c0;
     if (!ci) continue;
@@ -310,6 +315,7 @@
   }
   if (part == PART_EXTRACT) {
     p.n_params = b.pcur;
+    p.queue_off = b.alloc("", (size_t)std::max(p.nqueue, 1)).off;
     return DVSR_OK;
   }
 
@@ -421,6 +427,7 @@
   T yout; yout.space = SP_OUTPUT; yout.off = 0; yout.numel = (size_t)B * 3 * h * w;
   b.conv("conv_last", b.take(), out, 64, none, 0, B, h, w, 3, 3, 1, NO, base, 0, 1, 0, 0, yout);
   p.n_params = b.pcur;
+  p.queue_off = b.alloc("", (size_t)std::max(p.nqueue, 1)).off;
   return DVSR_OK;
 }
 
@@ -889,6 +896,7 @@
       for (const Op::Launch& l : o.launches[bs.mode]) {
         ConvExtra ex;
         set_wsets(p, o.N, l.pack.floats, o.Cout, &ex);
+        if (l.qslot >= 0) ex.queue = reinterpret_cast<int*>(bs.arena + p.queue_off) + l.qslot;
         int rc = conv2d_packed_run(launch_desc(d, o, l.role, bs.at(o.pre)), bs.arena + l.pack.off, ex, l.pack.geo, st);
         if (rc != DVSR_OK) return rc;
       }
@@ -1108,7 +1116,18 @@
   return ws_bytes < dvsr_edvr_workspace_bytes(p, 1) ? FWD_NOGRAD : FWD_GRAD;
 }
 
+static int zero_queues(const dvsr_edvr_plan& p, const Bases& bs, hipStream_t st) {
+  if (!p.nqueue || bs.mode != FWD_NOGRAD) return DVSR_OK;
+  DVSR_REQUIRE(hipMemsetAsync(bs.arena + p.queue_off, 0, (size_t)p.nqueue * sizeof(int), st) == hipSuccess, DVSR_ERR_HIP,
+               "edvr_forward: memset of the item counters failed");
+  return DVSR_OK;
+}
+
 static int run_forward_tape(const dvsr_edvr_plan& p, const float* const* params, const Bases& bs, bool packs_valid, hipStream_t st) {
+  {
+    int rc = zero_queues(p, bs, st);
+    if (rc != DVSR_OK) return rc;
+  }
   if (!p.use_v1 && !packs_valid) {
     int rc = pack_all(p, params, bs.arena, bs.arena, nullptr, st, bs.mode);
     if (rc != DVSR_OK) return rc;
@@ -1259,7 +1278,8 @@
   std::vector<hipEvent_t> ev(n + 1);
   for (auto& e : ev) DVSR_REQUIRE(hipEventCreate(&e) == hipSuccess, DVSR_ERR_HIP, "hipEventCreate failed");
   const Bases bs{(float*)ws, x, out, forward_mode(p, ws_bytes)};
-  int rc = p->use_v1 ? DVSR_OK : pack_all(*p, params, bs.arena, bs.arena, nullptr, st, bs.mode);
+  int rc = zero_queues(*p, bs, st);
+  if (rc == DVSR_OK && !p->use_v1) rc = pack_all(*p, params, bs.arena, bs.arena, nullptr, st, bs.mode);
   hipEventRecord(ev[0], st);
   for (size_t i = 0; i < n && rc == DVSR_OK; ++i) {
     rc = run_forward_op(*p, p->ops[i], params, bs, st);
@@ -1540,6 +1560,7 @@
     p.ops.push_back(o);
   }
   p.n_params = b.pcur;
+  p.queue_off = b.alloc("", (size_t)std::max(p.nqueue, 1)).off;
   return DVSR_OK;
 }
 
diff --git a/dynavsr_amd/csrc/kernels.h b/dynavsr_amd/csrc/kernels.h
--- a/dynavsr_amd/csrc/kernels.h
+++ b/dynavsr_amd/csrc/kernels.h
@@ -13,6 +13,7 @@
   const float* gmask = nullptr;
   int gmask_act = 0;
   int wdiv = 1; long long w_gs = 0; int b_gs = 0;
+  int* queue = nullptr;
 };
 int conv2d_run(const dvsr_conv2d_desc& d, const ConvExtra& ex, hipStream_t st);
 
diff --git a/dynavsr_amd/csrc/small_grid.h b/dynavsr_amd/csrc/small_grid.h
--- a/dynavsr_amd/csrc/small_grid.h
+++ b/dynavsr_amd/csrc/small_grid.h
@@ -17,6 +17,7 @@
   const float* gmask; int gmask_act;
   int wdiv = 1; long long w_gs = 0; int b_gs = 0;
   const float* pre = nullptr; int pre_bdiv = 1; long long pre_bs = 0;
+  int* queue = nullptr;
 #ifdef DVSR_CONV_TRACE
   int ablate;
   long long* trace;
diff --git a/dynavsr_amd/engine.py b/dynavsr_amd/engine.py
--- a/dynavsr_amd/engine.py
+++ b/dynavsr_amd/engine.py
@@ -7,7 +7,7 @@
 
 _plans = {}
 _GEOMETRY_ENV = ("DVSR_CONV_WINO", "DVSR_CONV_WINO3", "DVSR_CONV_WINO5", "DVSR_CONV_V1", "DVSR_EST_SPLIT", "DVSR_EST_SPLIT2", "DVSR_FUSE_ACT_BWD",
-                 "DVSR_BWD_STREAMS", "DVSR_PCD_HOIST")
+                 "DVSR_BWD_STREAMS", "DVSR_PCD_HOIST", "DVSR_CONV_WINO5_QUEUE")
 _PROCESS_ENV = ("DVSR_CONV_LDS", "DVSR_CONV_LAST_MFMA", "DVSR_SPLIT_TH8_FROM", "DVSR_WGRAD_SPLIT3",
                 "DVSR_WGRAD_WIDE", "DVSR_WGRAD_S3V", "DVSR_WGRAD_S3_KYS_BELOW", "DVSR_WGRAD_S3_WGS", "DVSR_WGRAD_S3W", "DVSR_DCN_FWD", "DVSR_DCN_BWD",
                 "DVSR_EST_FUSE_PAD", "DVSR_FUSE_RES_BWD", "DVSR_BWD_FORK_EVERY", "DVSR_BWD_PROBE", "DVSR_TSA_DUAL", "DVSR_TSA_V",
```

New measurement: 262.9 frames/s. About the same (-0.5%).
